# neggles/neurosis

Hardware: AMD Instinct MI355X
Metric: train images/sec (node) SDXL 1024^2 (higher is better)
Workload: dtype bf16

## Files before the change

### include/neurosis_hip.h

```cpp
#ifndef NEUROSIS_HIP_H
#define NEUROSIS_HIP_H

#ifdef __cplusplus
extern "C" {
#endif

const char* nk_last_error(void);
int nk_abi_version(void);

int nk_linear_fwd(const void* x, const void* w, const float* bias, const void* residual, void* y,
                  int M, int N, int K, long ldx, long ldw, long ldr, long ldy, float alpha, void* stream);
int nk_linear_dgrad(const void* dy, const void* w, const void* dx_add, void* dx, int M, int N, int K,
                    long lddy, long ldw, long ldadd, long lddx, void* stream);
long nk_linear_fwd_geglu_ok(int M, int I, int K);
int nk_linear_fwd_geglu(const void* x, const void* w, const float* bias, void* u, void* h, int M, int I, int K, long ldx, long ldw, long ldu,
                        long ldh, void* stream);
int nk_linear_dgrad_geglu(const void* dy, const void* w, const void* u, void* du, int M, int N, int I, long lddy, long ldw, long ldu,
                          long lddu, void* stream);
int nk_linear_fwd_geglu_s(const void* x, const void* w, const float* bias, void* s, void* h, int M, int I, int K, long ldx, long ldw, long lds,
                          long ldh, void* stream);
int nk_linear_dgrad_geglu_s(const void* dy, const void* w, const void* s, void* du, int M, int N, int I, long lddy, long ldw, long lds,
                            long lddu, void* stream);
int nk_linear_wgrad(const void* dy, const void* x, float* dw, int M, int N, int K, long lddy, long ldx,
                    long lddw, int accumulate, void* stream);
int nk_linear_wgrad_bias(const void* dy, const void* x, float* dw, float* dbias, int M, int N, int K, long lddy, long ldx, long lddw,
                         int accumulate, void* stream);

int nk_gemm_sk_status(void);

int nk_health_status(void);
int nk_health_clear(void);
int nk_health_export(int* dst, void* stream);
int nk_health_import(const int* src, void* stream);
int nk_debug_raise_health(void* stream);
int nk_debug_stamp(unsigned long long* dst, void* stream);
int nk_debug_launch_log(int mode);
long nk_debug_launch_names(char* buf, long cap);

int nk_colsum_batched(const void* dy, float* out, float* ws, long M, int N, long ld, int nbatch, int accumulate, void* stream);

int nk_linear_fwd_batched(const void* const* x, const void* const* w, void* const* y, int count, int M, int N, int K,
                          long ldx, long ldw, long ldy, void* stream);

int nk_linear_wgrad_batched(const void* const* dy, const void* const* x, float* const* dw, float* const* dbias, int count, int M, int N,
                            int K, long lddy, long ldx, long lddw, int accumulate, void* stream);

typedef struct NkConvDesc {
  int N, H, W, Cin;
  int Cout, KH, KW;
  int stride;
  int pad_t, pad_l;
  int Ho, Wo;
  int upsample;
} NkConvDesc;
int nk_conv2d_fwd(const NkConvDesc* d, const void* x, const void* w, const float* bias, const void* rowvec,
                  const void* residual, void* y, void* stream);
long nk_conv2d_stats_tiles(const NkConvDesc* d, int stats_groups);
int nk_conv2d_fwd_stats(const NkConvDesc* d, const void* x, const void* w, const float* bias, const void* rowvec, const void* residual,
                        void* y, float* stats_part, int stats_groups, void* stream);
int nk_conv3x3_few_channels_fwd(const void* x, const void* w, const float* bias, void* y, int N, int H, int W, int Cout, int cin_real,
                                void* stream);
int nk_conv_weight_flip(const void* w, void* wt, int Cout, int Cin, int taps, void* stream);
long nk_conv2d_dgrad_flipped_ok(const NkConvDesc* d);
int nk_conv2d_dgrad_flipped(const NkConvDesc* d, const void* dy, const void* wt, void* dx, void* stream);
int nk_conv2d_dgrad(const NkConvDesc* d, const void* dy, const void* w, void* dx, void* stream);
int nk_conv2d_wgrad(const NkConvDesc* d, const void* dy, const void* x, float* dw, int accumulate, void* stream);
int nk_conv2d_wgrad_bias(const NkConvDesc* d, const void* dy, const void* x, float* dw, float* dbias, int accumulate, void* stream);

typedef struct NkAttnDesc {
  int B, H, Lq, Lk, D;
  long sq, sk, sv, so;
  long bq, bk, bv, bo;
  long sdq, sdk, sdv, sdo;
  long bdq, bdk, bdv, bdo;
  float scale;
  int causal;
} NkAttnDesc;
int nk_attention_fwd(const NkAttnDesc* d, const void* q, const void* k, const void* v, void* o, float* lse,
                     void* stream);
long nk_attention_bwd_ws_floats(const NkAttnDesc* d);
int nk_attention_bwd(const NkAttnDesc* d, const void* q, const void* k, const void* v, const void* o,
                     const float* lse, const void* d_o, void* dq, void* dk, void* dv, float* delta_ws, void* stream);
int nk_attention_bwd_causal(const NkAttnDesc* d, const void* q, const void* k, const void* v, const void* o,
                            const float* lse, const void* d_o, void* dq, void* dk, void* dv, void* stream);
int nk_attention_relbias_fwd(const NkAttnDesc* d, const void* q, const void* k, const void* v, void* o, const float* rel, void* stream);
int nk_softmax_rows(void* s, long M, int L, void* stream);

long nk_groupnorm_ws_floats(int N, int HW, int C, int G);
int nk_groupnorm_fwd(const void* x, const float* gamma, const float* beta, void* y, float* mean, float* rstd,
                     float* ws, int N, int HW, int C, int G, float eps, int silu, void* stream);
int nk_groupnorm_sums(const void* x, float* sums, float* ws, int N, int HW, int C, int G, void* stream);
long nk_groupnorm_sums_ws_floats(int N, int nparts, int G);
int nk_groupnorm_sums_from_parts(const float* part, float* sums, float* ws, int N, int nparts, int G, void* stream);
int nk_groupnorm_apply(const void* x, const float* sums, const float* gamma, const float* beta, void* y, float* mean, float* rstd,
                       int N, int HW, int C, int G, float eps, int silu, void* stream);
int nk_groupnorm_bwd(const void* dy, const void* x, const float* gamma, const float* beta, const float* mean,
                     const float* rstd, const void* dx_add, void* dx, float* dgamma, float* dbeta, float* ws,
                     int N, int HW, int C, int G, int silu, int accumulate, void* stream);
int nk_groupnorm_mod_fwd(const void* x, const float* gamma, const float* beta, const void* mod, void* y, float* mean, float* rstd,
                         float* ws, int N, int HW, int C, int G, float eps, int silu, void* stream);
int nk_groupnorm_mod_apply(const void* x, const float* sums, const float* gamma, const float* beta, const void* mod, void* y, float* mean,
                           float* rstd, int N, int HW, int C, int G, float eps, int silu, void* stream);
int nk_groupnorm_mod_bwd(const void* dy, const void* x, const float* gamma, const float* beta, const void* mod, const float* mean,
                         const float* rstd, const void* dx_add, void* dx, float* dgamma, float* dbeta, void* dmod, float* ws,
                         int N, int HW, int C, int G, int silu, int accumulate, void* stream);

int nk_layernorm_fwd(const void* x, const float* gamma, const float* beta, void* y, float* mean, float* rstd,
                     int M, int C, float eps, void* stream);
long nk_layernorm_ws_floats(int M, int C);
int nk_rmsnorm_fwd(const void* x, const float* gamma, void* y, int M, int C, float eps, void* stream);
int nk_layernorm_bwd(const void* dy, const void* x, const float* gamma, const float* mean, const float* rstd,
                     const void* dx_add, void* dx, float* dgamma, float* dbeta, float* ws, int M, int C, int accumulate, void* stream);
#define NK_COLPART_MAX 32
typedef struct NkColpartBatch {
  const float* part[NK_COLPART_MAX];
  float* dgamma[NK_COLPART_MAX];
  float* dbeta[NK_COLPART_MAX];
  int nrows[NK_COLPART_MAX];
  int C[NK_COLPART_MAX];
  int accumulate[NK_COLPART_MAX];
  int n;
} NkColpartBatch;
long nk_layernorm_part_rows(int M);
int nk_layernorm_bwd_rows(const void* dy, const void* x, const float* gamma, const float* mean, const float* rstd,
                          const void* dx_add, void* dx, float* part, int M, int C, void* stream);
int nk_colpart_reduce_batch(const NkColpartBatch* b, void* stream);
int nk_layernorm_bwd_dx(const void* dy, const void* x, const float* gamma, const float* mean, const float* rstd,
                        const void* dx_add, void* dx, int M, int C, void* stream);
int nk_layernorm_bwd_params(const void* dy, const void* x, const float* mean, const float* rstd, float* dgamma,
                            float* dbeta, float* ws, int M, int C, int accumulate, void* stream);

int nk_geglu_fwd(const void* u, void* y, long M, int I, void* stream);
int nk_geglu_bwd(const void* dy, const void* u, void* du, long M, int I, void* stream);
int nk_geglu_fwd_s(const void* u, void* y, void* s, long M, int I, void* stream);
int nk_geglu_bwd_s(const void* dy, const void* s, void* du, long M, int I, void* stream);

int nk_silu_fwd(const void* x, void* y, long n, void* stream);
int nk_silu_bwd(const void* dy, const void* x, void* dx, long n, void* stream);

int nk_dropout(const void* x, const void* residual, void* y, long rows, int cols, long ld_x, long ld_res, long ld_y, const void* token,
               int site, int thr, float scale, void* stream);
int nk_dropout_draw(void* state, void* token, void* stream);

int nk_add(const void* a, const void* b, void* out, long n, void* stream);

int nk_cat_channels(const void* a, const void* b, void* out, long rows, int Ca, int Cb, void* stream);
int nk_split_channels(const void* src, void* a, void* b, long rows, int Ca, int Cb, void* stream);

int nk_upsample2x_bwd(const void* dup, void* dx, int N, int H, int W, int C, void* stream);
int nk_upsample2x_fwd(const void* x, void* up, int N, int H, int W, int C, void* stream);
int nk_avgpool2x_fwd(const void* x, void* y, int N, int H, int W, int C, void* stream);
int nk_avgpool2x_bwd(const void* dy, void* dx, int N, int H, int W, int C, void* stream);

int nk_nchw_to_nhwc(const void* src, int src_is_f32, void* dst, int N, int C, int HW, int Cpad, float scale,
                    void* stream);
int nk_nhwc_to_nchw(const void* src, void* dst, int dst_is_f32, int N, int C, int HW, int Cpad, void* stream);
int nk_cast_f32_to_bf16(const float* src, void* dst, long n, void* stream);
int nk_cast_bf16_to_f32(const void* src, float* dst, long n, void* stream);

long nk_colsum_ws_floats(long M, int N);
int nk_colsum(const void* dy, float* out, float* ws, long M, int N, long ld, int accumulate, void* stream);

int nk_softmax_rows_bwd(const void* p, void* dp, long M, int L, float scale, void* stream);

int nk_leaky_relu_fwd(const void* x, void* y, long n, float slope, void* stream);
int nk_leaky_relu_bwd(const void* dy, const void* y, void* dx, long n, float slope, void* stream);
long nk_batchnorm_ws_floats(long M, int C);
int nk_batchnorm_fwd(const void* x, const float* gamma, const float* beta, void* y, float* mean, float* rstd, float* running_mean,
                     float* running_var, float* ws, long M, int C, float eps, float momentum, float slope, void* stream);
int nk_batchnorm_bwd(const void* dy, const void* x, const void* y, const float* gamma, const float* mean, const float* rstd, void* dx,
                     float* dgamma, float* dbeta, float* ws, long M, int C, float slope, int accumulate, void* stream);
int nk_batchnorm_eval(const void* x, const float* gamma, const float* beta, const float* running_mean, const float* running_var, void* y,
                      float* ws, long M, int C, float eps, float slope, void* stream);

int nk_maxpool2x2_fwd(const void* x, void* y, int N, int H, int W, int C, void* stream);
int nk_maxpool2x2_bwd(const void* dy, const void* x, void* dx, int N, int H, int W, int C, void* stream);
int nk_maxpool_fwd(const void* x, void* y, int N, int H, int W, int C, int k, int s, void* stream);
int nk_maxpool_bwd(const void* dy, const void* x, void* dx, int N, int H, int W, int C, int k, int s, void* stream);
long nk_lpips_layer_ws_floats(int N, int HW);
int nk_lpips_layer_fwd(const void* f0, const void* f1, const float* w, float* out, float* ws, int N, int HW, int C, float eps,
                       int accumulate, void* stream);
int nk_lpips_layer_bwd(const void* f0, const void* f1, const float* w, const float* upstream, void* df1, int N, int HW, int C,
                       float eps, void* stream);

int nk_gelu_fwd(const void* x, void* y, long n, int mode, void* stream);
int nk_gated_gelu_tanh_fwd(const void* u, void* y, long M, int I, void* stream);
int nk_gelu_bwd(const void* dy, const void* x, void* dx, long n, int mode, void* stream);
#define NK_EMBEDDING_BWD_MAX_TOKENS 8192
int nk_embedding_bwd(const long long* ids, const void* dx, long ldx, float* dtable, float* dpos, int B, int L, int V, int P, int C,
                     int accumulate, void* stream);
int nk_gather_rows_bwd(const void* dsel, long ldsel, const long long* idx, void* dx, int B, int L, int C, void* stream);
int nk_wgrad_few_rows(const void* x, long ldx, const void* dy, long lddy, float* dw, long lddw, int M, int K, int N, int accumulate, void* stream);

#define NK_VQ_MAX_D 256
#define NK_VQ_MAX_CODES 65536
long nk_vq_search_ws_floats(long N, int n_e);
int nk_vq_search(const float* z, long ldz, const float* codebook, float* ws, long long* idx, long N, int D, int n_e, void* stream);
int nk_vq_code_stats(const long long* idx, const float* z, long ldz, long long* count, float* sum, long N, int D, int n_e, void* stream);
long nk_vq_quantize_ws_floats(long N);
int nk_vq_quantize(const long long* idx, const float* codebook, const float* z, long ldz, float* zq, float* sumsq, float* ws, long N, int D,
                   int n_e, int HW, void* stream);

int nk_timestep_embedding(const float* t, void* out, int B, int dim, float max_period, void* stream);

int nk_edm_prepare(const float* x, const float* eps, const float* sigma, const float* c_in, float* zt, void* net_in,
                   int B, int C, int HW, int Cpad, void* stream);
int nk_edm_prepare_cat(const float* x, const float* eps, const float* sigma, const float* c_in, const float* extra, float* zt,
                       void* net_in, int B, int C, int Ce, int HW, int Cpad, void* stream);
int nk_edm_loss(const void* net_out, const float* zt, const float* target, const float* c_out, const float* c_skip,
                const float* w, float* loss, void* dnet, int B, int C, int HW, int Cpad, float upstream, void* stream);

int nk_sample_prepare(const float* x, const float* c_in, void* net_in, int B, int C, int HW, int Cpad, int rep, void* stream);
int nk_sample_prepare_cat(const float* x, const float* c_in, const float* extra_u, const float* extra_c, void* net_in, int B, int C,
                          int Ce, int HW, int Cpad, int rep, void* stream);
int nk_sample_denoise(const void* net_out, const float* x, const float* c_skip, const float* c_out, float scale,
                      float* denoised, int B, int C, int HW, int Cpad, int rep, void* stream);
int nk_sample_euler_step(const void* net_out, const float* x, const float* c_skip, const float* c_out, const float* sigma_hat,
                         const float* sigma_next, float scale, float* x_next, float* denoised, int B, int C, int HW, int Cpad,
                         int rep, void* stream);

int nk_adamw_flat(float* p, const float* g, float* m, float* v, void* shadow, long n, float lr, float beta1,
                  float beta2, float eps, float weight_decay, int step, float grad_scale, void* stream);

typedef struct NkAdafactorArgs {
  float* master; const float* grad; void* shadow; float* state; float* ws;
  const void* tensors; const void* items;
  float* u2_part; float* p2_part; float* mean_row; float* scale; float* lr_t;
  int item_lo, item_hi, tensor_lo, tensor_hi;
  float beta2t, eps1, eps2, clip_threshold, rel_step, weight_decay, grad_scale;
  int scale_parameter;
  unsigned* counters;
  int has_matrix;
  int reserved;
} NkAdafactorArgs;
long nk_adafactor_tensor_bytes(void);
int nk_adafactor_init(const NkAdafactorArgs* args, void* stream);
int nk_adafactor_chunk(const NkAdafactorArgs* args, void* stream);

typedef struct NkCameArgs {
  float* master; const float* grad; void* shadow; float* state; float* ws;
  const void* tensors; const void* items;
  float* u2_part;
  float* mean_row;
  float* denom;
  unsigned* counters;
  int item_lo, item_hi, tensor_lo, tensor_hi;
  float beta1, beta2, beta3;
  float one_minus_beta1, one_minus_beta2, one_minus_beta3;
  float eps1, eps2, clip_threshold, lr, decay, grad_scale;
  int has_matrix;
} NkCameArgs;
long nk_came_tensor_bytes(void);
int nk_came_chunk(const NkCameArgs* args, void* stream);

typedef struct NkAdamW8bitArgs {
  float* master; const float* grad; void* shadow;
  unsigned char* code1; unsigned char* code2; float* absmax1; float* absmax2;
  float* m32; float* v32;
  const float* qmap1; const float* qmap2;
  const void* tensors; const int* blk_start;
  int ntensors, nblocks;
  float beta1, beta2, one_minus_beta1, one_minus_beta2, eps, lr, decay, bc1, bc2, grad_scale;
} NkAdamW8bitArgs;
long nk_adamw8bit_tensor_bytes(void);
int nk_adamw8bit_step(const NkAdamW8bitArgs* args, void* stream);

int nk_ema_flat(float* ema, const float* p, long n, float one_minus_decay, void* stream);

#ifdef __cplusplus
}
#endif
#endif
```

### neurosis_amd/csrc/norm.hip

```cpp
#include "../../include/neurosis_hip.h"
#include "nk_common.h"

#define GN_THREADS 256
#define GN_MAXC 4096

__global__ __launch_bounds__(GN_THREADS) void gn_stats_kernel(const bf16_t* __restrict__ x, float* __restrict__ stats,
                                                              int HW, int C, int G, int rows_per) {
  __shared__ float ps[GN_THREADS * 8], pss[GN_THREADS * 8];
  const int n = blockIdx.y;
  const int cpr = (C >> 3) / gridDim.z;
  const int ch0 = blockIdx.z * cpr;
  const int rows_par = GN_THREADS / cpr;
  const int tid = threadIdx.x;
  const int cpg = C / G;
  const int row_lo = blockIdx.x * rows_per;
  const int row_hi = min(HW, row_lo + rows_per);
  float s[8], ss[8];
#pragma unroll
  for (int e = 0; e < 8; ++e) { s[e] = 0.f; ss[e] = 0.f; }
  const int chunk = tid % cpr, rsub = tid / cpr;
  if (rsub < rows_par) {
    const bf16_t* base = x + ((long)n * HW) * C + (ch0 + chunk) * 8;
    int r = row_lo + rsub;
    for (; r + 3 * rows_par < row_hi; r += 4 * rows_par) {
      uint4_t v[4];
#pragma unroll
      for (int u = 0; u < 4; ++u) v[u] = *(const uint4_t*)(base + (long)(r + u * rows_par) * C);
#pragma unroll
      for (int u = 0; u < 4; ++u) {
        float f[8];
        unpack8(v[u], f);
#pragma unroll
        for (int e = 0; e < 8; ++e) { s[e] += f[e]; ss[e] += f[e] * f[e]; }
      }
    }
    for (; r < row_hi; r += rows_par) {
      float f[8];
      unpack8(*(const uint4_t*)(base + (long)r * C), f);
#pragma unroll
      for (int e = 0; e < 8; ++e) { s[e] += f[e]; ss[e] += f[e] * f[e]; }
    }
#pragma unroll
    for (int e = 0; e < 8; ++e) {
      ps[(rsub * cpr + chunk) * 8 + e] = s[e];
      pss[(rsub * cpr + chunk) * 8 + e] = ss[e];
    }
  }
  __syncthreads();
  float* part = stats + (((long)n * gridDim.x + blockIdx.x) * gridDim.z + blockIdx.z) * 2 * G;
  for (int i = tid; i < 2 * G; i += GN_THREADS) {
    const int g = i >> 1;
    const float* src = (i & 1) ? pss : ps;
    const int c_lo = max(g * cpg, ch0 * 8), c_hi = min((g + 1) * cpg, (ch0 + cpr) * 8);
    float a = 0.f;
    for (int c = c_lo; c < c_hi; ++c)
      for (int r = 0; r < rows_par; ++r) a += src[r * cpr * 8 + (c - ch0 * 8)];
    part[i] = a;
  }
}

__global__ __launch_bounds__(1024) void gn_reduce_partials_kernel(const float* __restrict__ part, float* __restrict__ out,
                                                                 int nparts, int G2) {
  __shared__ float sm[8][128];
  const int n = blockIdx.x;
  const int tx = threadIdx.x & 127, ty = threadIdx.x >> 7;
  float a = 0.f;
  if (tx < G2)
    for (int p = ty; p < nparts; p += 8) a += part[((long)n * nparts + p) * G2 + tx];
  sm[ty][tx] = a;
  __syncthreads();
  if (ty == 0 && tx < G2) {
#pragma unroll
    for (int j = 1; j < 8; ++j) a += sm[j][tx];
    out[(long)n * G2 + tx] = a;
  }
}

__device__ __forceinline__ void gn_modulate(const bf16_t* __restrict__ mod, int n, int c, int C, float& ga, float& be) {
  const float s1 = 1.0f + bf2f(mod[(long)n * 2 * C + c]);
  const float t = bf2f(mod[(long)n * 2 * C + C + c]);
  ga = ga * s1;
  be = be * s1 + t;
}

template <bool MOD>
__global__ __launch_bounds__(GN_THREADS) void gn_apply_kernel(const bf16_t* __restrict__ x, const float* __restrict__ stats,
                                                              const float* __restrict__ gamma, const float* __restrict__ beta,
                                                              const bf16_t* __restrict__ mod,
                                                              bf16_t* __restrict__ y, float* __restrict__ mean_out,
                                                              float* __restrict__ rstd_out, int HW, int C, int G,
                                                              float eps, int silu, int rows_per) {
  extern __shared__ __attribute__((aligned(16))) char smem_raw[];
  float* sc = (float*)smem_raw;
  float* sh = sc + C;
  const int n = blockIdx.y;
  const int tid = threadIdx.x;
  const int cpg = C / G;
  const float inv_cnt = 1.0f / ((float)HW * (float)cpg);
  for (int c = tid; c < C; c += GN_THREADS) {
    int g = c / cpg;
    float m = stats[(long)n * 2 * G + 2 * g] * inv_cnt;
    float var = fmaxf(stats[(long)n * 2 * G + 2 * g + 1] * inv_cnt - m * m, 0.f);
    float rs = rsqrtf(var + eps);
    float ga = gamma[c], be = beta[c];
    if constexpr (MOD) gn_modulate(mod, n, c, C, ga, be);
    float a = rs * ga;
    sc[c] = a;
    sh[c] = be - m * a;
    if (blockIdx.x == 0 && (c % cpg) == 0) { mean_out[n * G + g] = m; rstd_out[n * G + g] = rs; }
  }
  __syncthreads();
  const int cpr = C >> 3;
  const int row_lo = blockIdx.x * rows_per;
  const int row_hi = min(HW, row_lo + rows_per);
  const unsigned total = (unsigned)(row_hi - row_lo) * (unsigned)cpr;
  const bf16_t* xb = x + ((long)n * HW + row_lo) * C;
  bf16_t* yb = y + ((long)n * HW + row_lo) * C;
  auto one = [&](unsigned i, const uint4_t& raw) {
    const unsigned chunk = i % (unsigned)cpr;
    float f[8];
    unpack8(raw, f);
    const float4_t a0 = *(const float4_t*)(sc + chunk * 8), a1 = *(const float4_t*)(sc + chunk * 8 + 4);
    const float4_t b0 = *(const float4_t*)(sh + chunk * 8), b1 = *(const float4_t*)(sh + chunk * 8 + 4);
    f[0] = f[0] * a0[0] + b0[0]; f[1] = f[1] * a0[1] + b0[1]; f[2] = f[2] * a0[2] + b0[2]; f[3] = f[3] * a0[3] + b0[3];
    f[4] = f[4] * a1[0] + b1[0]; f[5] = f[5] * a1[1] + b1[1]; f[6] = f[6] * a1[2] + b1[2]; f[7] = f[7] * a1[3] + b1[3];
    if (silu) {
#pragma unroll
      for (int e = 0; e < 8; ++e) f[e] = silu_f(f[e]);
    }
    *(uint4_t*)(yb + (size_t)i * 8) = pack8(f);
  };
  unsigned i = tid;
  for (; i + 3 * GN_THREADS < total; i += 4 * GN_THREADS) {
    uint4_t v[4];
#pragma unroll
    for (int u = 0; u < 4; ++u) v[u] = *(const uint4_t*)(xb + (size_t)(i + u * GN_THREADS) * 8);
#pragma unroll
    for (int u = 0; u < 4; ++u) one(i + u * GN_THREADS, v[u]);
  }
  for (; i < total; i += GN_THREADS) one(i, *(const uint4_t*)(xb + (size_t)i * 8));
}

template <bool MOD>
__global__ __launch_bounds__(GN_THREADS, 4) void gn_bwd_stats_kernel(const bf16_t* __restrict__ dy, const bf16_t* __restrict__ x,
                                                                  const float* __restrict__ gamma, const float* __restrict__ beta,
                                                                  const bf16_t* __restrict__ mod,
                                                                  const float* __restrict__ mean, const float* __restrict__ rstd,
                                                                  float* __restrict__ gsum, float* __restrict__ chan_part,
                                                                  int HW, int C, int G, int silu, int rows_per) {
  __shared__ float pa[GN_THREADS * 8], pb[GN_THREADS * 8];
  extern __shared__ __attribute__((aligned(16))) char smem_raw[];
  float* ca = (float*)smem_raw;
  float* cb = ca + C;
  const int n = blockIdx.y;
  const int tid = threadIdx.x;
  const int cpg = C / G;
  const int cpr = (C >> 3) / gridDim.z;
  const int ch0 = blockIdx.z * cpr;
  const int rows_par = GN_THREADS / cpr;
  const int row_lo = blockIdx.x * rows_per;
  const int row_hi = min(HW, row_lo + rows_per);
  const int chunk = tid % cpr, rsub = tid / cpr;
  if (rsub < rows_par) {
    float a[8], b[8], mu[8], rs[8], ga[8], be[8];
#pragma unroll
    for (int e = 0; e < 8; ++e) {
      int c = (ch0 + chunk) * 8 + e;
      int g = c / cpg;
      a[e] = 0.f; b[e] = 0.f;
      mu[e] = mean[n * G + g]; rs[e] = rstd[n * G + g];
      ga[e] = gamma[c]; be[e] = beta[c];
      if constexpr (MOD) gn_modulate(mod, n, c, C, ga[e], be[e]);
    }
    const long base = ((long)n * HW) * C + (ch0 + chunk) * 8;
    auto one = [&](const uint4_t& rx, const uint4_t& rd) {
      float fx[8], fd[8];
      unpack8(rx, fx);
      unpack8(rd, fd);
#pragma unroll
      for (int e = 0; e < 8; ++e) {
        float xh = (fx[e] - mu[e]) * rs[e];
        float dz = fd[e];
        if (silu) dz *= dsilu_f(xh * ga[e] + be[e]);
        a[e] += dz;
        b[e] += dz * xh;
      }
    };
    int r = row_lo + rsub;
    for (; r + 3 * rows_par < row_hi; r += 4 * rows_par) {
      uint4_t vx[4], vd[4];
#pragma unroll
      for (int u = 0; u < 4; ++u) {
        vx[u] = *(const uint4_t*)(x + base + (long)(r + u * rows_par) * C);
        vd[u] = *(const uint4_t*)(dy + base + (long)(r + u * rows_par) * C);
      }
#pragma unroll
      for (int u = 0; u < 4; ++u) one(vx[u], vd[u]);
    }
    for (; r < row_hi; r += rows_par) one(*(const uint4_t*)(x + base + (long)r * C), *(const uint4_t*)(dy + base + (long)r * C));
#pragma unroll
    for (int e = 0; e < 8; ++e) {
      pa[(rsub * cpr + chunk) * 8 + e] = a[e];
      pb[(rsub * cpr + chunk) * 8 + e] = b[e];
    }
  }
  __syncthreads();
  float* cp = chan_part + ((long)n * gridDim.x + blockIdx.x) * 2 * C;
  for (int cl = tid; cl < cpr * 8; cl += GN_THREADS) {
    float av = 0.f, bv = 0.f;
    for (int r = 0; r < rows_par; ++r) { av += pa[r * cpr * 8 + cl]; bv += pb[r * cpr * 8 + cl]; }
    const int c = ch0 * 8 + cl;
    ca[cl] = av;
    cb[cl] = bv;
    cp[c] = bv;
    cp[C + c] = av;
  }
  __syncthreads();
  float* part = gsum + (((long)n * gridDim.x + blockIdx.x) * gridDim.z + blockIdx.z) * 2 * G;
  for (int i = tid; i < 2 * G; i += GN_THREADS) {
    const int g = i >> 1;
    const float* src = (i & 1) ? cb : ca;
    const int c_lo = max(g * cpg, ch0 * 8), c_hi = min((g + 1) * cpg, (ch0 + cpr) * 8);
    float acc = 0.f;
    for (int c = c_lo; c < c_hi; ++c) {
      float gc = gamma[c];
      if constexpr (MOD) { float bc = 0.f; gn_modulate(mod, n, c, C, gc, bc); }
      acc += gc * src[c - ch0 * 8];
    }
    part[i] = acc;
  }
}

__global__ __launch_bounds__(1024) void colpart_reduce_kernel(const float* __restrict__ part, float* __restrict__ dgamma,
                                                              float* __restrict__ dbeta, int nrows, int C, int accumulate) {
  __shared__ float sa[16][64], sb[16][64];
  const int tx = threadIdx.x & 63, ty = threadIdx.x >> 6;
  const int c = blockIdx.x * 64 + tx;
  float a = 0.f, b = 0.f;
  if (c < C) {
#pragma unroll 4
    for (int r = ty; r < nrows; r += 16) {
      a += part[(long)r * 2 * C + c];
      b += part[(long)r * 2 * C + C + c];
    }
  }
  sa[ty][tx] = a;
  sb[ty][tx] = b;
  __syncthreads();
  if (ty == 0 && c < C) {
#pragma unroll
    for (int j = 1; j < 16; ++j) { a += sa[j][tx]; b += sb[j][tx]; }
    dgamma[c] = accumulate ? dgamma[c] + a : a;
    dbeta[c] = accumulate ? dbeta[c] + b : b;
  }
}

__global__ __launch_bounds__(1024) void colpart_reduce_mod_kernel(const float* __restrict__ part, const bf16_t* __restrict__ mod,
                                                                  float* __restrict__ dgamma, float* __restrict__ dbeta, int nrows, int nsplit,
                                                                  int C, int accumulate) {
  __shared__ float sa[16][64], sb[16][64];
  const int tx = threadIdx.x & 63, ty = threadIdx.x >> 6;
  const int c = blockIdx.x * 64 + tx;
  float a = 0.f, b = 0.f;
  if (c < C) {
#pragma unroll 4
    for (int r = ty; r < nrows; r += 16) {
      const float s1 = 1.0f + bf2f(mod[(long)(r / nsplit) * 2 * C + c]);
      a += s1 * part[(long)r * 2 * C + c];
      b += s1 * part[(long)r * 2 * C + C + c];
    }
  }
  sa[ty][tx] = a;
  sb[ty][tx] = b;
  __syncthreads();
  if (ty == 0 && c < C) {
#pragma unroll
    for (int j = 1; j < 16; ++j) { a += sa[j][tx]; b += sb[j][tx]; }
    dgamma[c] = accumulate ? dgamma[c] + a : a;
    dbeta[c] = accumulate ? dbeta[c] + b : b;
  }
}

__global__ __launch_bounds__(1024) void gn_dmod_kernel(const float* __restrict__ part, const float* __restrict__ gamma,
                                                       const float* __restrict__ beta, bf16_t* __restrict__ dmod, int nsplit, int C) {
  __shared__ float sa[16][64], sb[16][64];
  const int tx = threadIdx.x & 63, ty = threadIdx.x >> 6;
  const int c = blockIdx.x * 64 + tx, n = blockIdx.y;
  float a = 0.f, b = 0.f;
  if (c < C) {
    for (int r = ty; r < nsplit; r += 16) {
      b += part[((long)n * nsplit + r) * 2 * C + c];
      a += part[((long)n * nsplit + r) * 2 * C + C + c];
    }
  }
  sa[ty][tx] = a;
  sb[ty][tx] = b;
  __syncthreads();
  if (ty == 0 && c < C) {
#pragma unroll
    for (int j = 1; j < 16; ++j) { a += sa[j][tx]; b += sb[j][tx]; }
    dmod[(long)n * 2 * C + c] = f2bf(gamma[c] * b + beta[c] * a);
    dmod[(long)n * 2 * C + C + c] = f2bf(a);
  }
}

template <bool MOD>
__global__ __launch_bounds__(GN_THREADS) void gn_bwd_apply_kernel(const bf16_t* __restrict__ dy, const bf16_t* __restrict__ x,
                                                                  const float* __restrict__ gamma, const float* __restrict__ beta,
                                                                  const bf16_t* __restrict__ mod,
                                                                  const float* __restrict__ mean, const float* __restrict__ rstd,
                                                                  const float* __restrict__ gsum, const bf16_t* __restrict__ dx_add,
                                                                  bf16_t* __restrict__ dx, int HW, int C, int G, int silu,
                                                                  int rows_per) {
  extern __shared__ __attribute__((aligned(16))) char smem_raw[];
  float* p_a = (float*)smem_raw;
  float* p_b = p_a + C;
  float* p_c = p_b + C;
  float* p_d = p_c + C;
  const int n = blockIdx.y;
  const int tid = threadIdx.x;
  const int cpg = C / G;
  const float inv_cnt = 1.0f / ((float)HW * (float)cpg);
  for (int c = tid; c < C; c += GN_THREADS) {
    const int g = c / cpg;
    const float mu = mean[n * G + g], rs = rstd[n * G + g];
    const float s1 = gsum[(long)n * 2 * G + 2 * g] * inv_cnt, s2 = gsum[(long)n * 2 * G + 2 * g + 1] * inv_cnt;
    float ga = gamma[c], be = beta[c];
    if constexpr (MOD) gn_modulate(mod, n, c, C, ga, be);
    const float a = rs * ga;
    p_a[c] = a;
    p_b[c] = be - mu * a;
    p_c[c] = -rs * rs * s2;
    p_d[c] = -rs * s1 + mu * rs * rs * s2;
  }
  __syncthreads();
  const int cpr = C >> 3;
  const int row_lo = blockIdx.x * rows_per;
  const int row_hi = min(HW, row_lo + rows_per);
  const unsigned total = (unsigned)(row_hi - row_lo) * (unsigned)cpr;
  const long off0 = ((long)n * HW + row_lo) * C;
  auto one = [&](unsigned i, const uint4_t& rx, const uint4_t& rd, const uint4_t& ra) {
    const int c0 = (int)(i % (unsigned)cpr) * 8;
    float fx[8], fd[8], fa[8], ca[8], cb[8], cc[8], cd[8];
    unpack8(rx, fx);
    unpack8(rd, fd);
    unpack8(ra, fa);
    *(float4_t*)ca = *(const float4_t*)(p_a + c0); *(float4_t*)(ca + 4) = *(const float4_t*)(p_a + c0 + 4);
    *(float4_t*)cc = *(const float4_t*)(p_c + c0); *(float4_t*)(cc + 4) = *(const float4_t*)(p_c + c0 + 4);
    *(float4_t*)cd = *(const float4_t*)(p_d + c0); *(float4_t*)(cd + 4) = *(const float4_t*)(p_d + c0 + 4);
    if (silu) {
      *(float4_t*)cb = *(const float4_t*)(p_b + c0); *(float4_t*)(cb + 4) = *(const float4_t*)(p_b + c0 + 4);
#pragma unroll
      for (int e = 0; e < 8; ++e) fd[e] *= dsilu_f(fx[e] * ca[e] + cb[e]);
    }
#pragma unroll
    for (int e = 0; e < 8; ++e) fx[e] = ca[e] * fd[e] + (fx[e] * cc[e] + cd[e]) + fa[e];
    *(uint4_t*)(dx + off0 + (size_t)i * 8) = pack8(fx);
  };
  const uint4_t zero4 = {0u, 0u, 0u, 0u};
  unsigned i = tid;
  for (; i + GN_THREADS < total; i += 2 * GN_THREADS) {
    uint4_t vx[2], vd[2], va[2];
#pragma unroll
    for (int u = 0; u < 2; ++u) {
      const size_t o = off0 + (size_t)(i + u * GN_THREADS) * 8;
      vx[u] = *(const uint4_t*)(x + o);
      vd[u] = *(const uint4_t*)(dy + o);
      va[u] = dx_add ? *(const uint4_t*)(dx_add + o) : zero4;
    }
#pragma unroll
    for (int u = 0; u < 2; ++u) one(i + u * GN_THREADS, vx[u], vd[u], va[u]);
  }
  for (; i < total; i += GN_THREADS) {
    const size_t o = off0 + (size_t)i * 8;
    one(i, *(const uint4_t*)(x + o), *(const uint4_t*)(dy + o), dx_add ? *(const uint4_t*)(dx_add + o) : zero4);
  }
}

static int gn_nz(int C) {
  int cpr = C >> 3, nz = (cpr + GN_THREADS - 1) / GN_THREADS;
  while (cpr % nz) ++nz;
  return nz;
}

static int gn_rows_per(int N, int HW, int* nsplit) {
  int want = (1024 + N - 1) / N;
  int rows_per = (HW + want - 1) / want;
  if (rows_per < 32) rows_per = 32;
  *nsplit = (HW + rows_per - 1) / rows_per;
  return rows_per;
}

extern "C" long nk_groupnorm_ws_floats(int N, int HW, int C, int G) {
  int nsplit;
  gn_rows_per(N, HW, &nsplit);
  long parts = (long)N * nsplit * gn_nz(C) * 2 * G;
  long chan = (long)N * nsplit * 2 * C;
  return parts + chan + (long)N * 2 * G + 64;
}

extern "C" int nk_groupnorm_fwd(const void* x, const float* gamma, const float* beta, void* y, float* mean,
                                float* rstd, float* ws, int N, int HW, int C, int G, float eps, int silu,
                                void* stream_) {
  hipStream_t stream = (hipStream_t)stream_;
  NK_CHECK_ARG(N > 0 && HW > 0 && C > 0 && G > 0 && G <= 64);
  NK_CHECK_ARG((C & 7) == 0 && C % G == 0 && C <= GN_MAXC);
  NK_CHECK_ARG(x && gamma && beta && y && mean && rstd && ws);
  int nsplit;
  int rows_per = gn_rows_per(N, HW, &nsplit);
  const int nz = gn_nz(C);
  float* part = ws;
  float* stats = ws + (long)N * nsplit * nz * 2 * G;
  hipLaunchKernelGGL(gn_stats_kernel, dim3(nsplit, N, nz), dim3(GN_THREADS), 0, stream, (const bf16_t*)x, part, HW, C,
                     G, rows_per);
  if (int e = nk_check_launch("gn_stats_kernel")) return e;
  hipLaunchKernelGGL(gn_reduce_partials_kernel, dim3(N), dim3(1024), 0, stream, part, stats, nsplit * nz, 2 * G);
  if (int e = nk_check_launch("gn_reduce_partials_kernel")) return e;
  hipLaunchKernelGGL(gn_apply_kernel<false>, dim3(nsplit, N), dim3(GN_THREADS), 2 * C * sizeof(float), stream,
                     (const bf16_t*)x, stats, gamma, beta, (const bf16_t*)nullptr, (bf16_t*)y, mean, rstd, HW, C, G, eps, silu, rows_per);
  return nk_check_launch("gn_apply_kernel");
}

__global__ __launch_bounds__(256) void gn_reduce_partials_l1_kernel(const float* __restrict__ part, float* __restrict__ out, int nparts, int G2, int nchunks) {
  __shared__ float sm[4][64];
  const int n = blockIdx.y, chunk = blockIdx.x;
  const int tx = threadIdx.x & 63, ty = threadIdx.x >> 6;
  float a = 0.f;
  if (tx < G2)
    for (int p = chunk + ty * nchunks; p < nparts; p += 4 * nchunks) a += part[((long)n * nparts + p) * G2 + tx];
  sm[ty][tx] = a;
  __syncthreads();
  if (ty == 0 && tx < G2) out[((long)n * nchunks + chunk) * G2 + tx] = (a + sm[1][tx]) + (sm[2][tx] + sm[3][tx]);
}

extern "C" long nk_groupnorm_sums_ws_floats(int N, int nparts, int G) {
  (void)nparts;
  return (long)N * 64 * 2 * G + 64;
}
extern "C" int nk_groupnorm_sums_from_parts(const float* part, float* sums, float* ws, int N, int nparts, int G, void* stream_) {
  hipStream_t stream = (hipStream_t)stream_;
  NK_CHECK_ARG(part && sums && N > 0 && nparts > 0 && G > 0 && G <= 32);
  if (nparts > 128) {
    NK_CHECK_ARG(ws != nullptr);
    const int nchunks = 64;
    hipLaunchKernelGGL(gn_reduce_partials_l1_kernel, dim3(nchunks, N), dim3(256), 0, stream, part, ws, nparts, 2 * G, nchunks);
    if (int e = nk_check_launch("gn_reduce_partials_l1_kernel")) return e;
    part = ws;
    nparts = nchunks;
  }
  hipLaunchKernelGGL(gn_reduce_partials_kernel, dim3(N), dim3(1024), 0, stream, part, sums, nparts, 2 * G);
  return nk_check_launch("gn_reduce_partials_kernel");
}

extern "C" int nk_groupnorm_sums(const void* x, float* sums, float* ws, int N, int HW, int C, int G, void* stream_) {
  hipStream_t stream = (hipStream_t)stream_;
  NK_CHECK_ARG(N > 0 && HW > 0 && C > 0 && G > 0 && G <= 64);
  NK_CHECK_ARG((C & 7) == 0 && C % G == 0 && C <= GN_MAXC);
  NK_CHECK_ARG(x && sums && ws);
  int nsplit;
  int rows_per = gn_rows_per(N, HW, &nsplit);
  const int nz = gn_nz(C);
  hipLaunchKernelGGL(gn_stats_kernel, dim3(nsplit, N, nz), dim3(GN_THREADS), 0, stream, (const bf16_t*)x, ws, HW, C, G, rows_per);
  if (int e = nk_check_launch("gn_stats_kernel")) return e;
  hipLaunchKernelGGL(gn_reduce_partials_kernel, dim3(N), dim3(1024), 0, stream, ws, sums, nsplit * nz, 2 * G);
  return nk_check_launch("gn_reduce_partials_kernel");
}

extern "C" int nk_groupnorm_apply(const void* x, const float* sums, const float* gamma, const float* beta, void* y, float* mean,
                                  float* rstd, int N, int HW, int C, int G, float eps, int silu, void* stream_) {
  hipStream_t stream = (hipStream_t)stream_;
  NK_CHECK_ARG(N > 0 && HW > 0 && C > 0 && G > 0 && G <= 64);
  NK_CHECK_ARG((C & 7) == 0 && C % G == 0 && C <= GN_MAXC);
  NK_CHECK_ARG(x && sums && gamma && beta && y && mean && rstd);
  int nsplit;
  int rows_per = gn_rows_per(N, HW, &nsplit);
  hipLaunchKernelGGL(gn_apply_kernel<false>, dim3(nsplit, N), dim3(GN_THREADS), 2 * C * sizeof(float), stream, (const bf16_t*)x, sums, gamma, beta,
                     (const bf16_t*)nullptr, (bf16_t*)y, mean, rstd, HW, C, G, eps, silu, rows_per);
  return nk_check_launch("gn_apply_kernel");
}

extern "C" int nk_groupnorm_bwd(const void* dy, const void* x, const float* gamma, const float* beta,
                                const float* mean, const float* rstd, const void* dx_add, void* dx, float* dgamma,
                                float* dbeta, float* ws, int N, int HW, int C, int G, int silu, int accumulate, void* stream_) {
  hipStream_t stream = (hipStream_t)stream_;
  NK_CHECK_ARG(N > 0 && HW > 0 && C > 0 && G > 0 && G <= 64);
  NK_CHECK_ARG((C & 7) == 0 && C % G == 0 && C <= GN_MAXC);
  NK_CHECK_ARG(dy && x && gamma && beta && mean && rstd && dx && dgamma && dbeta && ws);
  int nsplit;
  int rows_per = gn_rows_per(N, HW, &nsplit);
  const int nz = gn_nz(C);
  float* part = ws;
  float* gsum = part + (long)N * nsplit * nz * 2 * G;
  float* chan = gsum + (long)N * 2 * G;
  hipLaunchKernelGGL(gn_bwd_stats_kernel<false>, dim3(nsplit, N, nz), dim3(GN_THREADS), 2 * C * sizeof(float), stream,
                     (const bf16_t*)dy, (const bf16_t*)x, gamma, beta, (const bf16_t*)nullptr, mean, rstd, part, chan, HW, C, G, silu, rows_per);
  if (int e = nk_check_launch("gn_bwd_stats_kernel")) return e;
  hipLaunchKernelGGL(gn_reduce_partials_kernel, dim3(N), dim3(1024), 0, stream, part, gsum, nsplit * nz, 2 * G);
  if (int e = nk_check_launch("gn_reduce_partials_kernel")) return e;
  hipLaunchKernelGGL(colpart_reduce_kernel, dim3((C + 63) / 64), dim3(1024), 0, stream, chan, dgamma, dbeta, N * nsplit, C, accumulate);
  if (int e = nk_check_launch("colpart_reduce_kernel")) return e;
  hipLaunchKernelGGL(gn_bwd_apply_kernel<false>, dim3(nsplit, N), dim3(GN_THREADS), 4 * C * sizeof(float), stream,
                     (const bf16_t*)dy, (const bf16_t*)x, gamma, beta, (const bf16_t*)nullptr, mean, rstd, gsum, (const bf16_t*)dx_add,
                     (bf16_t*)dx, HW, C, G, silu, rows_per);
  return nk_check_launch("gn_bwd_apply_kernel");
}

static int gn_mod_apply_launch(const void* x, const float* sums, const float* gamma, const float* beta, const void* mod, void* y, float* mean,
                               float* rstd, int N, int HW, int C, int G, float eps, int silu, hipStream_t stream) {
  int nsplit;
  int rows_per = gn_rows_per(N, HW, &nsplit);
  hipLaunchKernelGGL(gn_apply_kernel<true>, dim3(nsplit, N), dim3(GN_THREADS), 2 * C * sizeof(float), stream, (const bf16_t*)x, sums, gamma, beta,
                     (const bf16_t*)mod, (bf16_t*)y, mean, rstd, HW, C, G, eps, silu, rows_per);
  return nk_check_launch("gn_apply_kernel<mod>");
}

extern "C" int nk_groupnorm_mod_fwd(const void* x, const float* gamma, const float* beta, const void* mod, void* y, float* mean, float* rstd,
                                    float* ws, int N, int HW, int C, int G, float eps, int silu, void* stream_) {
  hipStream_t stream = (hipStream_t)stream_;
  NK_CHECK_ARG(N > 0 && HW > 0 && C > 0 && G > 0 && G <= 64);
  NK_CHECK_ARG((C & 7) == 0 && C % G == 0 && C <= GN_MAXC);
  NK_CHECK_ARG(x && gamma && beta && mod && y && mean && rstd && ws);
  int nsplit;
  gn_rows_per(N, HW, &nsplit);
  float* stats = ws + (long)N * nsplit * gn_nz(C) * 2 * G;
  if (int e = nk_groupnorm_sums(x, stats, ws, N, HW, C, G, stream_)) return e;
  return gn_mod_apply_launch(x, stats, gamma, beta, mod, y, mean, rstd, N, HW, C, G, eps, silu, stream);
}

extern "C" int nk_groupnorm_mod_apply(const void* x, const float* sums, const float* gamma, const float* beta, const void* mod, void* y,
                                      float* mean, float* rstd, int N, int HW, int C, int G, float eps, int silu, void* stream_) {
  NK_CHECK_ARG(N > 0 && HW > 0 && C > 0 && G > 0 && G <= 64);
  NK_CHECK_ARG((C & 7) == 0 && C % G == 0 && C <= GN_MAXC);
  NK_CHECK_ARG(x && sums && gamma && beta && mod && y && mean && rstd);
  return gn_mod_apply_launch(x, sums, gamma, beta, mod, y, mean, rstd, N, HW, C, G, eps, silu, (hipStream_t)stream_);
}

extern "C" int nk_groupnorm_mod_bwd(const void* dy, const void* x, const float* gamma, const float* beta, const void* mod, const float* mean,
                                    const float* rstd, const void* dx_add, void* dx, float* dgamma, float* dbeta, void* dmod, float* ws,
                                    int N, int HW, int C, int G, int silu, int accumulate, void* stream_) {
  hipStream_t stream = (hipStream_t)stream_;
  NK_CHECK_ARG(N > 0 && HW > 0 && C > 0 && G > 0 && G <= 64);
  NK_CHECK_ARG((C & 7) == 0 && C % G == 0 && C <= GN_MAXC);
  NK_CHECK_ARG(dy && x && gamma && beta && mod && mean && rstd && dx && dgamma && dbeta && dmod && ws);
  int nsplit;
  int rows_per = gn_rows_per(N, HW, &nsplit);
  const int nz = gn_nz(C);
  float* part = ws;
  float* gsum = part + (long)N * nsplit * nz * 2 * G;
  float* chan = gsum + (long)N * 2 * G;
  hipLaunchKernelGGL(gn_bwd_stats_kernel<true>, dim3(nsplit, N, nz), dim3(GN_THREADS), 2 * C * sizeof(float), stream,
                     (const bf16_t*)dy, (const bf16_t*)x, gamma, beta, (const bf16_t*)mod, mean, rstd, part, chan, HW, C, G, silu, rows_per);
  if (int e = nk_check_launch("gn_bwd_stats_kernel<mod>")) return e;
  hipLaunchKernelGGL(gn_reduce_partials_kernel, dim3(N), dim3(1024), 0, stream, part, gsum, nsplit * nz, 2 * G);
  if (int e = nk_check_launch("gn_reduce_partials_kernel")) return e;
  hipLaunchKernelGGL(colpart_reduce_mod_kernel, dim3((C + 63) / 64), dim3(1024), 0, stream, chan, (const bf16_t*)mod, dgamma, dbeta, N * nsplit,
                     nsplit, C, accumulate);
  if (int e = nk_check_launch("colpart_reduce_mod_kernel")) return e;
  hipLaunchKernelGGL(gn_dmod_kernel, dim3((C + 63) / 64, N), dim3(1024), 0, stream, chan, gamma, beta, (bf16_t*)dmod, nsplit, C);
  if (int e = nk_check_launch("gn_dmod_kernel")) return e;
  hipLaunchKernelGGL(gn_bwd_apply_kernel<true>, dim3(nsplit, N), dim3(GN_THREADS), 4 * C * sizeof(float), stream,
                     (const bf16_t*)dy, (const bf16_t*)x, gamma, beta, (const bf16_t*)mod, mean, rstd, gsum, (const bf16_t*)dx_add,
                     (bf16_t*)dx, HW, C, G, silu, rows_per);
  return nk_check_launch("gn_bwd_apply_kernel<mod>");
}

#define LN_MAXCH 4

template <int NCH>
__global__ __launch_bounds__(256) void ln_fwd_kernel(const bf16_t* __restrict__ x, const float* __restrict__ gamma,
                                                     const float* __restrict__ beta, bf16_t* __restrict__ y,
                                                     float* __restrict__ mean, float* __restrict__ rstd, int M, int C,
                                                     float eps) {
  const int lane = threadIdx.x & 63;
  const int wave = (blockIdx.x * blockDim.x + threadIdx.x) >> 6;
  const int nwaves = (gridDim.x * blockDim.x) >> 6;
  const int cpr = C >> 3;
  const float invC = 1.0f / (float)C;
  for (int row = wave; row < M; row += nwaves) {
    float f[NCH][8];
    float s = 0.f;
#pragma unroll
    for (int j = 0; j < NCH; ++j) {
      int ch = lane + 64 * j;
      if (ch < cpr) {
        unpack8(*(const uint4_t*)(x + (long)row * C + ch * 8), f[j]);
#pragma unroll
        for (int e = 0; e < 8; ++e) s += f[j][e];
      }
    }
    const float mu = wave_sum(s) * invC;
    float v = 0.f;
#pragma unroll
    for (int j = 0; j < NCH; ++j) {
      int ch = lane + 64 * j;
      if (ch < cpr) {
#pragma unroll
        for (int e = 0; e < 8; ++e) { float d = f[j][e] - mu; v += d * d; }
      }
    }
    const float rs = rsqrtf(wave_sum(v) * invC + eps);
    if (lane == 0) { mean[row] = mu; rstd[row] = rs; }
#pragma unroll
    for (int j = 0; j < NCH; ++j) {
      int ch = lane + 64 * j;
      if (ch < cpr) {
        const float4_t g0 = *(const float4_t*)(gamma + ch * 8), g1 = *(const float4_t*)(gamma + ch * 8 + 4);
        const float4_t b0 = *(const float4_t*)(beta + ch * 8), b1 = *(const float4_t*)(beta + ch * 8 + 4);
        float o[8];
#pragma unroll
        for (int e = 0; e < 4; ++e) {
          o[e] = (f[j][e] - mu) * rs * g0[e] + b0[e];
          o[4 + e] = (f[j][4 + e] - mu) * rs * g1[e] + b1[e];
        }
        *(uint4_t*)(y + (long)row * C + ch * 8) = pack8(o);
      }
    }
  }
}

template <int NCH>
__global__ __launch_bounds__(256, 4) void ln_bwd_dx_kernel(const bf16_t* __restrict__ dy, const bf16_t* __restrict__ x,
                                                        const float* __restrict__ gamma, const float* __restrict__ mean,
                                                        const float* __restrict__ rstd, const bf16_t* __restrict__ dx_add,
                                                        bf16_t* __restrict__ dx, int M, int C) {
  const int lane = threadIdx.x & 63;
  const int wave = (blockIdx.x * blockDim.x + threadIdx.x) >> 6;
  const int nwaves = (gridDim.x * blockDim.x) >> 6;
  const int cpr = C >> 3;
  const float invC = 1.0f / (float)C;
  float gm[NCH][8];
#pragma unroll
  for (int j = 0; j < NCH; ++j) {
    int ch = lane + 64 * j;
#pragma unroll
    for (int e = 0; e < 8; ++e) gm[j][e] = 0.f;
    if (ch < cpr) {
      const float4_t g0 = *(const float4_t*)(gamma + ch * 8), g1 = *(const float4_t*)(gamma + ch * 8 + 4);
#pragma unroll
      for (int e = 0; e < 4; ++e) { gm[j][e] = g0[e]; gm[j][4 + e] = g1[e]; }
    }
  }
  for (int row = wave; row < M; row += nwaves) {
    const float mu = mean[row], rs = rstd[row];
    uint4_t rx[NCH], rd[NCH], ra[NCH];
#pragma unroll
    for (int j = 0; j < NCH; ++j) {
      int ch = lane + 64 * j;
      rx[j] = rd[j] = ra[j] = (uint4_t){0u, 0u, 0u, 0u};
      if (ch < cpr) {
        rx[j] = *(const uint4_t*)(x + (long)row * C + ch * 8);
        rd[j] = *(const uint4_t*)(dy + (long)row * C + ch * 8);
        if (dx_add) ra[j] = *(const uint4_t*)(dx_add + (long)row * C + ch * 8);
      }
    }
    float s1 = 0.f, s2 = 0.f;
#pragma unroll
    for (int j = 0; j < NCH; ++j) {
      float fx[8], fd[8];
      unpack8(rx[j], fx);
      unpack8(rd[j], fd);
#pragma unroll
      for (int e = 0; e < 8; ++e) {
        float d = fd[e] * gm[j][e];
        s1 += d;
        s2 += d * ((fx[e] - mu) * rs);
      }
    }
    s1 = wave_sum(s1) * invC;
    s2 = wave_sum(s2) * invC;
#pragma unroll
    for (int j = 0; j < NCH; ++j) {
      int ch = lane + 64 * j;
      if (ch < cpr) {
        float fx[8], fd[8], o[8];
        unpack8(rx[j], fx);
        unpack8(rd[j], fd);
        unpack8(ra[j], o);
#pragma unroll
        for (int e = 0; e < 8; ++e) o[e] += rs * (fd[e] * gm[j][e] - s1 - (fx[e] - mu) * rs * s2);
        *(uint4_t*)(dx + (long)row * C + ch * 8) = pack8(o);
      }
    }
  }
}

#define LNP_ROWS 64
__global__ __launch_bounds__(256) void ln_bwd_param_kernel(const bf16_t* __restrict__ dy, const bf16_t* __restrict__ x,
                                                           const float* __restrict__ mean, const float* __restrict__ rstd,
                                                           float* __restrict__ part, int M, int C) {
  __shared__ float pg[16][16 * 8 + 4], pb[16][16 * 8 + 4];
  const int tid = threadIdx.x;
  const int cx = tid & 15, ry = tid >> 4;
  const int chunk = blockIdx.y * 16 + cx;
  const bool cok = chunk < (C >> 3);
  const int row_lo = blockIdx.x * LNP_ROWS;
  float sg[8], sb[8];
#pragma unroll
  for (int e = 0; e < 8; ++e) { sg[e] = 0.f; sb[e] = 0.f; }
  if (cok) {
    uint4_t vx[4], vd[4];
    float mu[4], rs[4];
#pragma unroll
    for (int i = 0; i < 4; ++i) {
      const int r = row_lo + ry + 16 * i;
      const bool ok = r < M;
      vx[i] = ok ? *(const uint4_t*)(x + (long)r * C + chunk * 8) : (uint4_t){0u, 0u, 0u, 0u};
      vd[i] = ok ? *(const uint4_t*)(dy + (long)r * C + chunk * 8) : (uint4_t){0u, 0u, 0u, 0u};
      mu[i] = ok ? mean[r] : 0.f;
      rs[i] = ok ? rstd[r] : 0.f;
    }
#pragma unroll
    for (int i = 0; i < 4; ++i) {
      float fx[8], fd[8];
      unpack8(vx[i], fx);
      unpack8(vd[i], fd);
#pragma unroll
      for (int e = 0; e < 8; ++e) {
        sb[e] += fd[e];
        sg[e] += fd[e] * ((fx[e] - mu[i]) * rs[i]);
      }
    }
  }
#pragma unroll
  for (int e = 0; e < 8; ++e) { pg[ry][cx * 8 + e] = sg[e]; pb[ry][cx * 8 + e] = sb[e]; }
  __syncthreads();
  if (tid < 128) {
    const int c = blockIdx.y * 128 + tid;
    if (c < C) {
      float a = 0.f, b = 0.f;
#pragma unroll
      for (int r = 0; r < 16; ++r) { a += pg[r][tid]; b += pb[r][tid]; }
      float* out = part + (long)blockIdx.x * 2 * C;
      out[c] = a;
      out[C + c] = b;
    }
  }
}

static int ln_param_split(int M) { return (M + LNP_ROWS - 1) / LNP_ROWS; }

#define LNR_WAVES 4
#define LNR_MAX_BLOCKS 512
template <int NCH>
__global__ __launch_bounds__(LNR_WAVES * 64) void ln_bwd_rows_kernel(const bf16_t* __restrict__ dy, const bf16_t* __restrict__ x,
                                                                       const float* __restrict__ gamma, const float* __restrict__ mean,
                                                                       const float* __restrict__ rstd, const bf16_t* __restrict__ dx_add,
                                                                       bf16_t* __restrict__ dx, float* __restrict__ part, int M, int C) {
  extern __shared__ __attribute__((aligned(16))) char ln_smem[];
  float* red = (float*)ln_smem;
  const int lane = threadIdx.x & 63, wv = threadIdx.x >> 6;
  const int wave = blockIdx.x * LNR_WAVES + wv;
  const int nwaves = gridDim.x * LNR_WAVES;
  const int cpr = C >> 3;
  const float invC = 1.0f / (float)C;
  float gm[NCH][8], sg[NCH][8], sb[NCH][8];
#pragma unroll
  for (int j = 0; j < NCH; ++j) {
    int ch = lane + 64 * j;
#pragma unroll
    for (int e = 0; e < 8; ++e) { gm[j][e] = 0.f; sg[j][e] = 0.f; sb[j][e] = 0.f; }
    if (ch < cpr) {
      const float4_t g0 = *(const float4_t*)(gamma + ch * 8), g1 = *(const float4_t*)(gamma + ch * 8 + 4);
#pragma unroll
      for (int e = 0; e < 4; ++e) { gm[j][e] = g0[e]; gm[j][4 + e] = g1[e]; }
    }
  }
  uint4_t rx[NCH], rd[NCH], ra[NCH];
  float mu = 0.f, rs = 0.f;
  auto fetch = [&](int row, uint4_t (&fx)[NCH], uint4_t (&fd)[NCH], uint4_t (&fa)[NCH], float& fmu, float& frs) {
#pragma unroll
    for (int j = 0; j < NCH; ++j) {
      const int ch = lane + 64 * j;
      fx[j] = fd[j] = fa[j] = (uint4_t){0u, 0u, 0u, 0u};
      if (row < M && ch < cpr) {
        fx[j] = *(const uint4_t*)(x + (long)row * C + ch * 8);
        fd[j] = *(const uint4_t*)(dy + (long)row * C + ch * 8);
        if (dx_add) fa[j] = *(const uint4_t*)(dx_add + (long)row * C + ch * 8);
      }
    }
    fmu = row < M ? mean[row] : 0.f;
    frs = row < M ? rstd[row] : 0.f;
  };
  constexpr bool AHEAD = NCH < 4;
  if (AHEAD) fetch(wave, rx, rd, ra, mu, rs);
  for (int row = wave; row < M; row += nwaves) {
    uint4_t nx[NCH], nd[NCH], na[NCH];
    float nmu = 0.f, nrs = 0.f;
    if (AHEAD) fetch(row + nwaves, nx, nd, na, nmu, nrs);
    else fetch(row, rx, rd, ra, mu, rs);
    float s1 = 0.f, s2 = 0.f;
#pragma unroll
    for (int j = 0; j < NCH; ++j) {
      float fx[8], fd[8];
      unpack8(rx[j], fx);
      unpack8(rd[j], fd);
#pragma unroll
      for (int e = 0; e < 8; ++e) {
        const float xh = (fx[e] - mu) * rs;
        const float d = fd[e] * gm[j][e];
        s1 += d;
        s2 += d * xh;
        sb[j][e] += fd[e];
        sg[j][e] += fd[e] * xh;
      }
    }
    s1 = wave_sum(s1) * invC;
    s2 = wave_sum(s2) * invC;
#pragma unroll
    for (int j = 0; j < NCH; ++j) {
      int ch = lane + 64 * j;
      if (ch < cpr) {
        float fx[8], fd[8], o[8];
        unpack8(rx[j], fx);
        unpack8(rd[j], fd);
        unpack8(ra[j], o);
#pragma unroll
        for (int e = 0; e < 8; ++e) o[e] += rs * (fd[e] * gm[j][e] - s1 - (fx[e] - mu) * rs * s2);
        *(uint4_t*)(dx + (long)row * C + ch * 8) = pack8(o);
      }
    }
    if (AHEAD) {
#pragma unroll
      for (int j = 0; j < NCH; ++j) { rx[j] = nx[j]; rd[j] = nd[j]; ra[j] = na[j]; }
      mu = nmu;
      rs = nrs;
    }
  }
#pragma unroll
  for (int round = 0; round < LNR_WAVES / 2; ++round) {
    if ((wv >> 1) == round) {
      float* gbase = red + ((long)(wv & 1) * 2) * C;
#pragma unroll
      for (int j = 0; j < NCH; ++j) {
        int ch = lane + 64 * j;
        if (ch < cpr) {
          float* g = gbase + ch * 8;
          float4_t g0 = {sg[j][0], sg[j][1], sg[j][2], sg[j][3]}, g1 = {sg[j][4], sg[j][5], sg[j][6], sg[j][7]};
          float4_t b0 = {sb[j][0], sb[j][1], sb[j][2], sb[j][3]}, b1 = {sb[j][4], sb[j][5], sb[j][6], sb[j][7]};
          if (round) { g0 += *(const float4_t*)g; g1 += *(const float4_t*)(g + 4); b0 += *(const float4_t*)(g + C); b1 += *(const float4_t*)(g + C + 4); }
          *(float4_t*)g = g0;
          *(float4_t*)(g + 4) = g1;
          *(float4_t*)(g + C) = b0;
          *(float4_t*)(g + C + 4) = b1;
        }
      }
    }
    __syncthreads();
  }
  float* out = part + (long)blockIdx.x * 2 * C;
  for (int c = threadIdx.x; c < 2 * C; c += LNR_WAVES * 64) out[c] = red[c] + red[2 * C + c];
}
static int ln_rows_blocks(int M) {
  int b = (M + 4 * LNR_WAVES - 1) / (4 * LNR_WAVES);
  return b < 1 ? 1 : (b > LNR_MAX_BLOCKS ? LNR_MAX_BLOCKS : b);
}

__global__ __launch_bounds__(1024) void colpart_reduce_batch_kernel(const NkColpartBatch b) {
  __shared__ float sa[32][33], sb[32][33];
  const int z = blockIdx.y;
  const int C = b.C[z], nrows = b.nrows[z];
  if ((int)blockIdx.x * 32 >= C) return;
  const float* __restrict__ part = b.part[z];
  const int tx = threadIdx.x & 31, ty = threadIdx.x >> 5;
  const int c = blockIdx.x * 32 + tx;
  float a = 0.f, v = 0.f;
  if (c < C) {
#pragma unroll 8
    for (int r = ty; r < nrows; r += 32) {
      a += part[(long)r * 2 * C + c];
      v += part[(long)r * 2 * C + C + c];
    }
  }
  sa[ty][tx] = a;
  sb[ty][tx] = v;
  __syncthreads();
  if (ty == 0 && c < C) {
#pragma unroll
    for (int j = 1; j < 32; ++j) { a += sa[j][tx]; v += sb[j][tx]; }
    float* dgamma = b.dgamma[z];
    float* dbeta = b.dbeta[z];
    dgamma[c] = b.accumulate[z] ? dgamma[c] + a : a;
    dbeta[c] = b.accumulate[z] ? dbeta[c] + v : v;
  }
}

extern "C" int nk_colpart_reduce_batch(const NkColpartBatch* b, void* stream_) {
  NK_CHECK_ARG(b && b->n > 0 && b->n <= NK_COLPART_MAX);
  int maxC = 0;
  for (int z = 0; z < b->n; ++z) {
    NK_CHECK_ARG(b->part[z] && b->dgamma[z] && b->dbeta[z] && b->nrows[z] > 0 && b->C[z] > 0);
    maxC = b->C[z] > maxC ? b->C[z] : maxC;
  }
  hipLaunchKernelGGL(colpart_reduce_batch_kernel, dim3((maxC + 31) / 32, b->n), dim3(1024), 0, (hipStream_t)stream_, *b);
  return nk_check_launch("colpart_reduce_batch_kernel");
}

extern "C" int nk_layernorm_fwd(const void* x, const float* gamma, const float* beta, void* y, float* mean,
                                float* rstd, int M, int C, float eps, void* stream) {
  NK_CHECK_ARG(M > 0 && C > 0 && (C & 7) == 0 && (C >> 3) <= 64 * LN_MAXCH);
  NK_CHECK_ARG(x && gamma && beta && y && mean && rstd);
  int blocks = min((M + 3) / 4, 4096);
  const int nch = ((C >> 3) + 63) / 64;
#define NK_LN_FWD(NCH_) hipLaunchKernelGGL(ln_fwd_kernel<NCH_>, dim3(blocks), dim3(256), 0, (hipStream_t)stream, (const bf16_t*)x, gamma, beta, (bf16_t*)y, mean, rstd, M, C, eps)
  if (nch <= 2) NK_LN_FWD(2); else if (nch == 3) NK_LN_FWD(3); else NK_LN_FWD(4);
#undef NK_LN_FWD
  return nk_check_launch("ln_fwd_kernel");
}

#define RMS_MAXCH 8
template <int NCH>
__global__ __launch_bounds__(256) void rms_fwd_kernel(const bf16_t* __restrict__ x, const float* __restrict__ gamma, bf16_t* __restrict__ y, int M, int C,
                                                      float eps) {
  const int lane = threadIdx.x & 63;
  const int wave = (blockIdx.x * blockDim.x + threadIdx.x) >> 6;
  const int nwaves = (gridDim.x * blockDim.x) >> 6;
  const int cpr = C >> 3;
  const float invC = 1.0f / (float)C;
  for (int row = wave; row < M; row += nwaves) {
    uint4_t raw[NCH];
    float s = 0.f;
#pragma unroll
    for (int j = 0; j < NCH; ++j) {
      const int ch = lane + 64 * j;
      if (ch < cpr) {
        float f[8];
        raw[j] = *(const uint4_t*)(x + (long)row * C + ch * 8);
        unpack8(raw[j], f);
#pragma unroll
        for (int e = 0; e < 8; ++e) s = fmaf(f[e], f[e], s);
      }
    }
    const float rs = rsqrtf(wave_sum(s) * invC + eps);
#pragma unroll
    for (int j = 0; j < NCH; ++j) {
      const int ch = lane + 64 * j;
      if (ch < cpr) {
        const float4_t g0 = *(const float4_t*)(gamma + ch * 8), g1 = *(const float4_t*)(gamma + ch * 8 + 4);
        float f[8], o[8];
        unpack8(raw[j], f);
#pragma unroll
        for (int e = 0; e < 4; ++e) {
          o[e] = f[e] * rs * g0[e];
          o[4 + e] = f[4 + e] * rs * g1[e];
        }
        *(uint4_t*)(y + (long)row * C + ch * 8) = pack8(o);
      }
    }
  }
}

extern "C" int nk_rmsnorm_fwd(const void* x, const float* gamma, void* y, int M, int C, float eps, void* stream) {
  NK_CHECK_ARG(M > 0 && C > 0 && (C & 7) == 0 && (C >> 3) <= 64 * RMS_MAXCH);
  NK_CHECK_ARG(x && gamma && y);
  NK_CHECK_ARG(((uintptr_t)x & 15) == 0 && ((uintptr_t)y & 15) == 0 && ((uintptr_t)gamma & 15) == 0);
  int blocks = min((M + 3) / 4, 4096);
  const int nch = ((C >> 3) + 63) / 64;
#define NK_RMS_FWD(NCH_) hipLaunchKernelGGL(rms_fwd_kernel<NCH_>, dim3(blocks), dim3(256), 0, (hipStream_t)stream, (const bf16_t*)x, gamma, (bf16_t*)y, M, C, eps)
  if (nch <= 2) NK_RMS_FWD(2); else if (nch <= 4) NK_RMS_FWD(4); else NK_RMS_FWD(8);
#undef NK_RMS_FWD
  return nk_check_launch("rms_fwd_kernel");
}

extern "C" long nk_layernorm_ws_floats(int M, int C) {
  const long a = (long)ln_param_split(M), b = LNR_MAX_BLOCKS;
  return (a > b ? a : b) * 2 * C + 64;
}

extern "C" long nk_layernorm_part_rows(int M) { return ln_rows_blocks(M); }

extern "C" int nk_layernorm_bwd_dx(const void* dy, const void* x, const float* gamma, const float* mean, const float* rstd,
                                   const void* dx_add, void* dx, int M, int C, void* stream_) {
  hipStream_t stream = (hipStream_t)stream_;
  NK_CHECK_ARG(M > 0 && C > 0 && (C & 7) == 0 && (C >> 3) <= 64 * LN_MAXCH);
  NK_CHECK_ARG(dy && x && gamma && mean && rstd && dx);
  const int blocks = min((M + 3) / 4, 4096);
  const int nch = ((C >> 3) + 63) / 64;
#define NK_LN_DX(NCH_) hipLaunchKernelGGL(ln_bwd_dx_kernel<NCH_>, dim3(blocks), dim3(256), 0, stream, (const bf16_t*)dy, (const bf16_t*)x, gamma, mean, rstd, (const bf16_t*)dx_add, (bf16_t*)dx, M, C)
  if (nch <= 2) NK_LN_DX(2); else if (nch == 3) NK_LN_DX(3); else NK_LN_DX(4);
#undef NK_LN_DX
  return nk_check_launch("ln_bwd_dx_kernel");
}

extern "C" int nk_layernorm_bwd_params(const void* dy, const void* x, const float* mean, const float* rstd, float* dgamma,
                                       float* dbeta, float* ws, int M, int C, int accumulate, void* stream_) {
  hipStream_t stream = (hipStream_t)stream_;
  NK_CHECK_ARG(M > 0 && C > 0 && (C & 7) == 0);
  NK_CHECK_ARG(dy && x && mean && rstd && dgamma && dbeta && ws);
  const int nsplit = ln_param_split(M);
  hipLaunchKernelGGL(ln_bwd_param_kernel, dim3(nsplit, (C + 127) / 128), dim3(256), 0, stream, (const bf16_t*)dy, (const bf16_t*)x,
                     mean, rstd, ws, M, C);
  if (int e = nk_check_launch("ln_bwd_param_kernel")) return e;
  hipLaunchKernelGGL(colpart_reduce_kernel, dim3((C + 63) / 64), dim3(1024), 0, stream, ws, dgamma, dbeta, nsplit, C, accumulate);
  return nk_check_launch("colpart_reduce_kernel");
}

static int launch_ln_rows(const void* dy, const void* x, const float* gamma, const float* mean, const float* rstd, const void* dx_add,
                          void* dx, float* part, int M, int C, hipStream_t stream) {
  const int blocks = ln_rows_blocks(M);
  const int nch = ((C >> 3) + 63) / 64;
  const int smem = 2 * 2 * C * (int)sizeof(float);
#define NK_LN_ROWS(NCH_)                                                                                                       \
  do {                                                                                                                          \
    nk_optin_lds((const void*)ln_bwd_rows_kernel<NCH_>, 2 * 2 * 2048 * 4);                                                      \
    hipLaunchKernelGGL(ln_bwd_rows_kernel<NCH_>, dim3(blocks), dim3(LNR_WAVES * 64), smem, stream, (const bf16_t*)dy, (const bf16_t*)x, gamma, mean, rstd,   \
                       (const bf16_t*)dx_add, (bf16_t*)dx, part, M, C);                                                        \
  } while (0)
  if (nch <= 2) NK_LN_ROWS(2); else if (nch == 3) NK_LN_ROWS(3); else NK_LN_ROWS(4);
#undef NK_LN_ROWS
  return nk_check_launch("ln_bwd_rows_kernel");
}

extern "C" int nk_layernorm_bwd_rows(const void* dy, const void* x, const float* gamma, const float* mean, const float* rstd,
                                     const void* dx_add, void* dx, float* part, int M, int C, void* stream_) {
  NK_CHECK_ARG(M > 0 && C > 0 && (C & 7) == 0 && (C >> 3) <= 64 * LN_MAXCH);
  NK_CHECK_ARG(dy && x && gamma && mean && rstd && dx && part);
  return launch_ln_rows(dy, x, gamma, mean, rstd, dx_add, dx, part, M, C, (hipStream_t)stream_);
}

extern "C" int nk_layernorm_bwd(const void* dy, const void* x, const float* gamma, const float* mean,
                                const float* rstd, const void* dx_add, void* dx, float* dgamma, float* dbeta, float* ws,
                                int M, int C, int accumulate, void* stream_) {
  hipStream_t stream = (hipStream_t)stream_;
  NK_CHECK_ARG(M > 0 && C > 0 && (C & 7) == 0 && (C >> 3) <= 64 * LN_MAXCH);
  NK_CHECK_ARG(dy && x && gamma && mean && rstd && dx && dgamma && dbeta && ws);
  if (int e = launch_ln_rows(dy, x, gamma, mean, rstd, dx_add, dx, ws, M, C, stream)) return e;
  hipLaunchKernelGGL(colpart_reduce_kernel, dim3((C + 63) / 64), dim3(1024), 0, stream, ws, dgamma, dbeta, ln_rows_blocks(M), C, accumulate);
  return nk_check_launch("colpart_reduce_kernel");
}
```

### neurosis_amd/lib.py

```python
from __future__ import annotations

import ctypes as C
import os
from pathlib import Path

import torch

CSRC = Path(__file__).resolve().parent / "csrc"
LIB_PATH = CSRC / "libneurosis_hip.so"

vp, i32, i64, f32 = C.c_void_p, C.c_int, C.c_long, C.c_float


class NkConvDesc(C.Structure):
    _fields_ = [(n, i32) for n in ("N", "H", "W", "Cin", "Cout", "KH", "KW", "stride", "pad_t", "pad_l", "Ho", "Wo", "upsample")]


class NkAttnDesc(C.Structure):
    _fields_ = (
        [(n, i32) for n in ("B", "H", "Lq", "Lk", "D")]
        + [(n, i64) for n in ("sq", "sk", "sv", "so", "bq", "bk", "bv", "bo", "sdq", "sdk", "sdv", "sdo", "bdq", "bdk", "bdv", "bdo")]
        + [("scale", f32), ("causal", i32)]
    )


NK_COLPART_MAX = 32


class NkColpartBatch(C.Structure):
    _fields_ = [("part", vp * NK_COLPART_MAX), ("dgamma", vp * NK_COLPART_MAX), ("dbeta", vp * NK_COLPART_MAX), ("nrows", i32 * NK_COLPART_MAX),
                ("C", i32 * NK_COLPART_MAX), ("accumulate", i32 * NK_COLPART_MAX), ("n", i32)]


cdp, adp = C.POINTER(NkConvDesc), C.POINTER(NkAttnDesc)

SIGNATURES: dict[str, list] = {
    "nk_linear_fwd": [vp, vp, vp, vp, vp, i32, i32, i32, i64, i64, i64, i64, f32, vp],
    "nk_linear_dgrad": [vp, vp, vp, vp, i32, i32, i32, i64, i64, i64, i64, vp],
    "nk_linear_dgrad_geglu": [vp, vp, vp, vp, i32, i32, i32, i64, i64, i64, i64, vp],
    "nk_linear_fwd_geglu": [vp, vp, vp, vp, vp, i32, i32, i32, i64, i64, i64, i64, vp],
    "nk_linear_fwd_geglu_s": [vp, vp, vp, vp, vp, i32, i32, i32, i64, i64, i64, i64, vp],
    "nk_linear_dgrad_geglu_s": [vp, vp, vp, vp, i32, i32, i32, i64, i64, i64, i64, vp],
    "nk_linear_wgrad": [vp, vp, vp, i32, i32, i32, i64, i64, i64, i32, vp],
    "nk_linear_fwd_batched": [C.POINTER(vp), C.POINTER(vp), C.POINTER(vp), i32, i32, i32, i32, i64, i64, i64, vp],
    "nk_linear_wgrad_batched": [C.POINTER(vp), C.POINTER(vp), C.POINTER(vp), C.POINTER(vp), i32, i32, i32, i32, i64, i64, i64, i32, vp],
    "nk_linear_wgrad_bias": [vp, vp, vp, vp, i32, i32, i32, i64, i64, i64, i32, vp],
    "nk_conv2d_wgrad_bias": [cdp, vp, vp, vp, vp, i32, vp],
    "nk_conv2d_fwd": [cdp, vp, vp, vp, vp, vp, vp, vp],
    "nk_conv2d_fwd_stats": [cdp, vp, vp, vp, vp, vp, vp, vp, i32, vp],
    "nk_conv_weight_flip": [vp, vp, i32, i32, i32, vp],
    "nk_conv3x3_few_channels_fwd": [vp, vp, vp, vp, i32, i32, i32, i32, i32, vp],
    "nk_conv2d_dgrad": [cdp, vp, vp, vp, vp],
    "nk_conv2d_dgrad_flipped": [cdp, vp, vp, vp, vp],
    "nk_conv2d_wgrad": [cdp, vp, vp, vp, i32, vp],
    "nk_attention_fwd": [adp, vp, vp, vp, vp, vp, vp],
    "nk_attention_bwd": [adp, vp, vp, vp, vp, vp, vp, vp, vp, vp, vp, vp],
    "nk_attention_bwd_causal": [adp, vp, vp, vp, vp, vp, vp, vp, vp, vp, vp],
    "nk_attention_relbias_fwd": [adp, vp, vp, vp, vp, vp, vp],
    "nk_softmax_rows": [vp, i64, i32, vp],
    "nk_softmax_rows_bwd": [vp, vp, i64, i32, f32, vp],
    "nk_groupnorm_fwd": [vp, vp, vp, vp, vp, vp, vp, i32, i32, i32, i32, f32, i32, vp],
    "nk_groupnorm_sums": [vp, vp, vp, i32, i32, i32, i32, vp],
    "nk_groupnorm_sums_from_parts": [vp, vp, vp, i32, i32, i32, vp],
    "nk_groupnorm_apply": [vp, vp, vp, vp, vp, vp, vp, i32, i32, i32, i32, f32, i32, vp],
    "nk_groupnorm_bwd": [vp, vp, vp, vp, vp, vp, vp, vp, vp, vp, vp, i32, i32, i32, i32, i32, i32, vp],
    "nk_groupnorm_mod_fwd": [vp, vp, vp, vp, vp, vp, vp, vp, i32, i32, i32, i32, f32, i32, vp],
    "nk_groupnorm_mod_apply": [vp, vp, vp, vp, vp, vp, vp, vp, i32, i32, i32, i32, f32, i32, vp],
    "nk_groupnorm_mod_bwd": [vp, vp, vp, vp, vp, vp, vp, vp, vp, vp, vp, vp, vp, i32, i32, i32, i32, i32, i32, vp],
    "nk_layernorm_fwd": [vp, vp, vp, vp, vp, vp, i32, i32, f32, vp],
    "nk_rmsnorm_fwd": [vp, vp, vp, i32, i32, f32, vp],
    "nk_layernorm_bwd": [vp, vp, vp, vp, vp, vp, vp, vp, vp, vp, i32, i32, i32, vp],
    "nk_layernorm_bwd_dx": [vp, vp, vp, vp, vp, vp, vp, i32, i32, vp],
    "nk_layernorm_bwd_rows": [vp, vp, vp, vp, vp, vp, vp, vp, i32, i32, vp],
    "nk_colpart_reduce_batch": [C.POINTER(NkColpartBatch), vp],
    "nk_layernorm_bwd_params": [vp, vp, vp, vp, vp, vp, vp, i32, i32, i32, vp],
    "nk_geglu_fwd": [vp, vp, i64, i32, vp],
    "nk_geglu_bwd": [vp, vp, vp, i64, i32, vp],
    "nk_geglu_fwd_s": [vp, vp, vp, i64, i32, vp],
    "nk_geglu_bwd_s": [vp, vp, vp, i64, i32, vp],
    "nk_silu_fwd": [vp, vp, i64, vp],
    "nk_gelu_fwd": [vp, vp, i64, i32, vp],
    "nk_gated_gelu_tanh_fwd": [vp, vp, i64, i32, vp],
    "nk_gelu_bwd": [vp, vp, vp, i64, i32, vp],
    "nk_embedding_bwd": [vp, vp, i64, vp, vp, i32, i32, i32, i32, i32, i32, vp],
    "nk_gather_rows_bwd": [vp, i64, vp, vp, i32, i32, i32, vp],
    "nk_wgrad_few_rows": [vp, i64, vp, i64, vp, i64, i32, i32, i32, i32, vp],
    "nk_vq_search": [vp, i64, vp, vp, vp, i64, i32, i32, vp],
    "nk_vq_code_stats": [vp, vp, i64, vp, vp, i64, i32, i32, vp],
    "nk_vq_quantize": [vp, vp, vp, i64, vp, vp, vp, i64, i32, i32, i32, vp],
    "nk_leaky_relu_fwd": [vp, vp, i64, f32, vp],
    "nk_leaky_relu_bwd": [vp, vp, vp, i64, f32, vp],
    "nk_maxpool2x2_fwd": [vp, vp, i32, i32, i32, i32, vp],
    "nk_maxpool2x2_bwd": [vp, vp, vp, i32, i32, i32, i32, vp],
    "nk_maxpool_fwd": [vp, vp, i32, i32, i32, i32, i32, i32, vp],
    "nk_maxpool_bwd": [vp, vp, vp, i32, i32, i32, i32, i32, i32, vp],
    "nk_lpips_layer_fwd": [vp, vp, vp, vp, vp, i32, i32, i32, f32, i32, vp],
    "nk_lpips_layer_bwd": [vp, vp, vp, vp, vp, i32, i32, i32, f32, vp],
    "nk_batchnorm_fwd": [vp, vp, vp, vp, vp, vp, vp, vp, vp, i64, i32, f32, f32, f32, vp],
    "nk_batchnorm_bwd": [vp, vp, vp, vp, vp, vp, vp, vp, vp, vp, i64, i32, f32, i32, vp],
    "nk_batchnorm_eval": [vp, vp, vp, vp, vp, vp, vp, i64, i32, f32, f32, vp],
    "nk_silu_bwd": [vp, vp, vp, i64, vp],
    "nk_add": [vp, vp, vp, i64, vp],
    "nk_dropout": [vp, vp, vp, i64, i32, i64, i64, i64, vp, i32, i32, f32, vp],
    "nk_dropout_draw": [vp, vp, vp],
    "nk_cat_channels": [vp, vp, vp, i64, i32, i32, vp],
    "nk_split_channels": [vp, vp, vp, i64, i32, i32, vp],
    "nk_upsample2x_bwd": [vp, vp, i32, i32, i32, i32, vp],
    "nk_upsample2x_fwd": [vp, vp, i32, i32, i32, i32, vp],
    "nk_avgpool2x_fwd": [vp, vp, i32, i32, i32, i32, vp],
    "nk_avgpool2x_bwd": [vp, vp, i32, i32, i32, i32, vp],
    "nk_nchw_to_nhwc": [vp, i32, vp, i32, i32, i32, i32, f32, vp],
    "nk_nhwc_to_nchw": [vp, vp, i32, i32, i32, i32, i32, vp],
    "nk_cast_f32_to_bf16": [vp, vp, i64, vp],
    "nk_cast_bf16_to_f32": [vp, vp, i64, vp],
    "nk_colsum": [vp, vp, vp, i64, i32, i64, i32, vp],
    "nk_colsum_batched": [vp, vp, vp, i64, i32, i64, i32, i32, vp],
    "nk_timestep_embedding": [vp, vp, i32, i32, f32, vp],
    "nk_edm_prepare": [vp, vp, vp, vp, vp, vp, i32, i32, i32, i32, vp],
    "nk_edm_prepare_cat": [vp, vp, vp, vp, vp, vp, vp, i32, i32, i32, i32, i32, vp],
    "nk_edm_loss": [vp, vp, vp, vp, vp, vp, vp, vp, i32, i32, i32, i32, f32, vp],
    "nk_sample_prepare": [vp, vp, vp, i32, i32, i32, i32, i32, vp],
    "nk_sample_prepare_cat": [vp, vp, vp, vp, vp, i32, i32, i32, i32, i32, i32, vp],
    "nk_sample_denoise": [vp, vp, vp, vp, f32, vp, i32, i32, i32, i32, i32, vp],
    "nk_sample_euler_step": [vp, vp, vp, vp, vp, vp, f32, vp, vp, i32, i32, i32, i32, i32, vp],
    "nk_adamw_flat": [vp, vp, vp, vp, vp, i64, f32, f32, f32, f32, f32, i32, f32, vp],
    "nk_ema_flat": [vp, vp, i64, f32, vp],
    "nk_debug_raise_health": [vp],
    "nk_debug_stamp": [vp, vp],
    "nk_debug_launch_log": [i32],
    "nk_health_clear": [],
    "nk_health_export": [vp, vp],
    "nk_health_import": [vp, vp],
    "nk_adafactor_init": [vp, vp],
    "nk_adafactor_chunk": [vp, vp],
    "nk_came_chunk": [vp, vp],
    "nk_adamw8bit_step": [vp, vp],
}

SIZE_QUERIES: dict[str, list] = {
    "nk_groupnorm_ws_floats": [i32, i32, i32, i32],
    "nk_groupnorm_sums_ws_floats": [i32, i32, i32],
    "nk_conv2d_stats_tiles": [cdp, i32],
    "nk_conv2d_dgrad_flipped_ok": [cdp],
    "nk_linear_fwd_geglu_ok": [i32, i32, i32],
    "nk_layernorm_ws_floats": [i32, i32],
    "nk_layernorm_part_rows": [i32],
    "nk_colsum_ws_floats": [i64, i32],
    "nk_batchnorm_ws_floats": [i64, i32],
    "nk_lpips_layer_ws_floats": [i32, i32],
    "nk_attention_bwd_ws_floats": [adp],
    "nk_vq_search_ws_floats": [i64, i32],
    "nk_vq_quantize_ws_floats": [i64],
    "nk_adafactor_tensor_bytes": [],
    "nk_came_tensor_bytes": [],
    "nk_adamw8bit_tensor_bytes": [],
    "nk_gemm_sk_status": [],
    "nk_health_status": [],
    "nk_debug_launch_names": [C.c_char_p, i64],
}

_lib = None


class NkError(RuntimeError):
    pass


def load() -> C.CDLL:
    global _lib
    if _lib is not None:
        return _lib
    path = Path(os.environ.get("NEUROSIS_HIP_LIB", LIB_PATH))
    if not path.exists():
        raise NkError(
            f"{path} not found: the HIP extension is not built. Run `python -c 'import __graft_entry__ as g; g.build()'` "
            "(or `make -C neurosis_amd/csrc`). There is no CPU fallback for the product path."
        )
    lib = C.CDLL(str(path))
    lib.nk_last_error.restype = C.c_char_p
    lib.nk_last_error.argtypes = []
    lib.nk_abi_version.restype = i32
    lib.nk_abi_version.argtypes = []
    for name, argtypes in SIGNATURES.items():
        fn = getattr(lib, name)
        fn.argtypes = argtypes
        fn.restype = i32
    for name, argtypes in SIZE_QUERIES.items():
        fn = getattr(lib, name)
        fn.argtypes = argtypes
        fn.restype = i64
    _lib = lib
    return lib


def launch_log(mode: int) -> None:
    call("nk_debug_launch_log", int(mode))


def launched() -> list[str]:
    buf = C.create_string_buffer(8192)
    n = query("nk_debug_launch_names", buf, len(buf))
    if n < 0:
        raise NkError("nk_debug_launch_names failed")
    return buf.value.decode().split("\n")[:-1]


def query(name: str, *args) -> int:
    return int(getattr(load(), name)(*args))


def call(name: str, *args) -> None:
    lib = load()
    rc = getattr(lib, name)(*args)
    if rc != 0:
        raise NkError(f"{name} failed (rc={rc}): {lib.nk_last_error().decode()}")
```

### neurosis_amd/modules/diffusion/openaimodel.py

```python
from __future__ import annotations

import os

from typing import Callable, List, Optional, Union

import torch
from torch import Tensor, nn

from ... import ops
from ...nn import Conv2d, FlatParamStore, apply_module, as_tokens, linear_module_fwd
from ...ops import BF16, Img
from ..attention import SpatialTransformer, zero_module


def conv_nd(dims: int, *args, **kwargs) -> nn.Module:
    if dims != 2:
        raise ValueError(f"unsupported dimensions: {dims} (the MI355X path implements 2-D convolutions)")
    return Conv2d(*args, **kwargs)


class TimestepBlock(nn.Module):

    def forward(self, x: Tensor, emb: Tensor):
        raise NotImplementedError("TimestepBlock is an interface: subclasses implement forward(x, emb)")


class TimestepEmbedSequential(nn.Sequential, TimestepBlock):

    def fwd(self, x: Img, emb: Tensor, context: Optional[Tensor], dctx_sink: Optional[Callable[[Tensor], None]] = None):
        bwds = []
        first = True
        for layer in self:
            if isinstance(layer, TimestepBlock):
                x, b = layer.fwd(x, emb)
                bwds.append(("emb", b))
            elif isinstance(layer, SpatialTransformer):
                x, b = layer.fwd(x, context, need_dctx=dctx_sink is not None)
                bwds.append(("ctx", b))
            elif isinstance(layer, (Conv2d, Upsample, Downsample)):
                x, b = layer.fwd(x, need_dx=not (first and getattr(self, "_nk_input_block", False)))
                bwds.append(("plain", b))
            elif isinstance(layer, nn.Identity):
                continue
            else:
                raise NotImplementedError(f"TimestepEmbedSequential: unsupported layer {type(layer).__name__}")
            first = False

        def bwd(dy: Tensor):
            demb = None
            for kind, b in reversed(bwds):
                if dy is None:
                    break
                if kind == "emb":
                    dy, de = b(dy)
                    demb = de if demb is None else ops.add(demb, de)
                elif kind == "ctx":
                    dy, dc = b(dy)
                    if dctx_sink is not None and dc is not None:
                        dctx_sink(dc)
                else:
                    dyi, _ = b(dy)
                    dy = None if dyi is None else dyi.t
            bwds.clear()
            return dy, demb

        return x, bwd

    def forward(self, x: Tensor, emb: Tensor, context: Optional[Tensor] = None, image_only_indicator=None, time_context=None, num_video_frames=None):
        ins = [x, emb] if context is None else [x, emb, context]
        ops.dropout_open(self)

        def run(x, emb, context=None):
            img = Img.from_nchw(x)
            out, bwd = self.fwd(img, as_tokens(emb), None if context is None else as_tokens(context))

            def bwd2(g):
                dx, demb = bwd(Img.from_nchw(g).t)
                res = (Img(dx, img.N, img.H, img.W).to_nchw(), None if demb is None else demb.view(emb.shape))
                return res if context is None else (*res, None)

            return out.to_nchw(), bwd2

        return apply_module(run, ins, self)


class Upsample(nn.Module):

    def __init__(self, channels: int, use_conv: bool, dims: int = 2, out_channels: Optional[int] = None, padding: int = 1,
                 third_up: bool = False, kernel_size: int = 3, scale_factor: int = 2):
        super().__init__()
        self.channels = channels
        self.out_channels = out_channels or channels
        self.use_conv = use_conv
        self.dims = dims
        self.third_up = third_up
        self.scale_factor = scale_factor
        if dims != 2 or scale_factor != 2:
            raise NotImplementedError("Upsample: the MI355X path implements dims=2, scale_factor=2 (dims=3 / third_up are the video options)")
        if use_conv:
            self.conv = conv_nd(dims, self.channels, self.out_channels, kernel_size, padding=padding)

    def fwd(self, x: Img, need_dx: bool = True):
        assert x.C == self.channels
        if self.use_conv:
            return self.conv.fwd(x, upsample=True, need_dx=need_dx)
        y, b = ops.upsample2x_fwd(x)
        return y, (lambda dy: (Img(b(dy), x.N, x.H, x.W) if need_dx else None, None))

    def forward(self, x: Tensor) -> Tensor:
        return _plain_forward(self, x)


class Downsample(nn.Module):

    def __init__(self, channels: int, use_conv: bool, dims: int = 2, out_channels: Optional[int] = None, padding: int = 1, third_down: bool = False):
        super().__init__()
        self.channels = channels
        self.out_channels = out_channels or channels
        self.use_conv = use_conv
        self.dims = dims
        if dims != 2:
            raise NotImplementedError("Downsample: the MI355X path implements dims=2 (dims=3 / third_down are the video options)")
        if use_conv:
            self.op = conv_nd(dims, self.channels, self.out_channels, 3, stride=2, padding=padding)
        else:
            assert self.channels == self.out_channels, "Downsample(use_conv=False) cannot change the channel count"
            self.op = nn.AvgPool2d(kernel_size=2, stride=2)

    def fwd(self, x: Img, need_dx: bool = True):
        assert x.C == self.channels
        if self.use_conv:
            return self.op.fwd(x, need_dx=need_dx)
        y, b = ops.avgpool2x_fwd(x)
        return y, (lambda dy: (Img(b(dy), x.N, x.H, x.W) if need_dx else None, None))

    def forward(self, x: Tensor) -> Tensor:
        return _plain_forward(self, x)


def _plain_forward(mod: nn.Module, x: Tensor) -> Tensor:
    def run(x):
        img = Img.from_nchw(x)
        out, bwd = mod.fwd(img)
        return out.to_nchw(), lambda g: bwd(Img.from_nchw(g).t)[0].to_nchw()

    return apply_module(run, [x], mod)


class ResBlock(TimestepBlock):

    def __init__(self, channels: int, emb_channels: int, dropout: float, out_channels: Optional[int] = None, use_conv: bool = False,
                 use_scale_shift_norm: bool = False, dims: int = 2, use_checkpoint: bool = False, up: bool = False, down: bool = False,
                 kernel_size: int = 3, exchange_temb_dims: bool = False, skip_t_emb: bool = False):
        super().__init__()
        if exchange_temb_dims or skip_t_emb:
            raise NotImplementedError("ResBlock: exchange_temb_dims / skip_t_emb are options of the video UNet, which is not on the MI355X path")
        self.channels = channels
        self.emb_channels = emb_channels
        self.dropout = self.dropout_p = ops.check_dropout_rate(dropout, "ResBlock")
        self.out_channels = out_channels if out_channels is not None else channels
        self.use_conv = use_conv
        self.use_checkpoint = use_checkpoint
        self.use_scale_shift_norm = use_scale_shift_norm
        self.exchange_temb_dims = exchange_temb_dims
        padding = kernel_size // 2
        self.in_layers = nn.Sequential(nn.GroupNorm(32, channels), nn.SiLU(), conv_nd(dims, channels, self.out_channels, kernel_size, padding=padding))
        self.updown = up or down
        self._up, self._down = bool(up), bool(down) and not up
        if up:
            self.h_upd = Upsample(channels, False, dims)
            self.x_upd = Upsample(channels, False, dims)
        elif down:
            self.h_upd = Downsample(channels, False, dims)
            self.x_upd = Downsample(channels, False, dims)
        else:
            self.h_upd = self.x_upd = nn.Identity()
        self.skip_t_emb = skip_t_emb
        self.emb_out_channels = 2 * self.out_channels if use_scale_shift_norm else self.out_channels
        self.emb_layers = nn.Sequential(nn.SiLU(), nn.Linear(emb_channels, self.emb_out_channels))
        self.out_layers = nn.Sequential(
            nn.GroupNorm(32, self.out_channels), nn.SiLU(), nn.Dropout(p=dropout),
            zero_module(conv_nd(dims, self.out_channels, self.out_channels, kernel_size, padding=padding)),
        )
        if self.out_channels == channels:
            self.skip_connection = nn.Identity()
        elif use_conv:
            self.skip_connection = conv_nd(dims, channels, self.out_channels, kernel_size, padding=padding)
        else:
            self.skip_connection = conv_nd(dims, channels, self.out_channels, 1)

    def _skip_fwd(self, x: Img):
        skip = self.skip_connection
        b_res = None
        if self._down:
            x, b_res = ops.avgpool2x_fwd(x)
        if isinstance(skip, nn.Identity):
            s, b_skip = x.t, None
        elif skip.kernel_size == 1:
            s, b_skip = ops.linear_fwd(x.t, skip.weight, skip.bias)
        else:
            si, b_skip3 = skip.fwd(x, upsample=self._up)
            s, b_skip = si.t, (lambda g: b_skip3(g)[0].t)
        b_up = None
        if self._up and (b_skip is None or skip.kernel_size == 1):
            sup, b_up = ops.upsample2x_fwd(Img(s, x.N, x.H, x.W))
            s = sup.t
        if b_skip is None and b_res is None and b_up is None:
            return s, None

        def bwd(dy: Tensor) -> Tensor:
            if b_up is not None:
                dy = b_up(dy)
            if b_skip is not None:
                dy = b_skip(dy)
            return dy if b_res is None else b_res(dy)

        return s, bwd

    def _fwd(self, x: Img, emb: Tensor):
        gn1, gn2 = self.in_layers[0], self.out_layers[0]
        ssn = self.use_scale_shift_norm
        h1, b_gn1 = ops.groupnorm_fwd(x, gn1.weight, gn1.bias, 32, gn1.eps, silu=True)
        b_pool = None
        if self._down:
            h1, b_pool = ops.avgpool2x_fwd(h1)
        es, b_es = ops.silu_fwd(emb)
        eo, b_eo = linear_module_fwd(self.emb_layers[1], es)
        h2, b_c1 = self.in_layers[2].fwd(h1, rowvec=None if ssn else eo, upsample=self._up, stats_groups=32)
        if ssn:
            h3, b_gn2 = ops.groupnorm_mod_fwd(h2, gn2.weight, gn2.bias, eo, 32, gn2.eps, silu=True)
        else:
            h3, b_gn2 = ops.groupnorm_fwd(h2, gn2.weight, gn2.bias, 32, gn2.eps, silu=True)
        b_drop = None
        if self.training and self.dropout_p > 0.0:
            _, b_drop = ops.dropout_fwd(h3.t, self.dropout_p, ops.dropout_site(self), inplace=True)
        s, b_skip = self._skip_fwd(x)
        out, b_c2 = self.out_layers[3].fwd(h3, residual=s, stats_groups=32)

        def bwd(dy: Tensor):
            dh3, _ = b_c2(dy)
            dh2 = b_gn2(dh3.t if b_drop is None else b_drop(dh3.t, inplace=True))
            if ssn:
                dh2, deo = dh2
                dh1, _ = b_c1(dh2)
            else:
                dh1, deo = b_c1(dh2)
            dh1 = dh1.t if b_pool is None else b_pool(dh1.t)
            dxs = dy if b_skip is None else b_skip(dy)
            dx = b_gn1(dh1, dxs)
            demb = b_es(b_eo(deo))
            return dx, demb

        return out, bwd

    def fwd(self, x: Img, emb: Tensor):
        if not (self.use_checkpoint and ops.recording()):
            return self._fwd(x, emb)
        out, _ = self._fwd(x, emb)
        tok = ops.dropout_token(required=False)

        def bwd(dy: Tensor):
            with ops.dropout_token_scope(tok):
                _, b = self._fwd(x, emb)
            return b(dy)

        return out, bwd

    def forward(self, x: Tensor, emb: Tensor) -> Tensor:
        ops.dropout_open(self)

        def run(x, emb):
            img = Img.from_nchw(x)
            out, bwd = self.fwd(img, as_tokens(emb))

            def bwd2(g):
                dx, demb = bwd(Img.from_nchw(g).t)
                return Img(dx, img.N, img.H, img.W).to_nchw(), demb.view(emb.shape)

            return out.to_nchw(), bwd2

        return apply_module(run, [x, emb], self)


class Timestep(nn.Module):

    def __init__(self, dim: int):
        super().__init__()
        self.dim = dim

    def forward(self, t: Tensor) -> Tensor:
        return ops.timestep_embedding(t, self.dim)


class UNetModel(nn.Module):

    def __init__(
        self,
        in_channels: int,
        model_channels: int,
        out_channels: int,
        num_res_blocks: int,
        attention_resolutions,
        dropout: float = 0.0,
        channel_mult=(1, 2, 4, 8),
        conv_resample: bool = True,
        dims: int = 2,
        num_classes=None,
        use_checkpoint: bool = False,
        num_heads: int = -1,
        num_head_channels: int = -1,
        num_heads_upsample: int = -1,
        use_scale_shift_norm: bool = False,
        resblock_updown: bool = False,
        transformer_depth=1,
        context_dim: Optional[int] = None,
        disable_self_attentions: Optional[List[bool]] = None,
        num_attention_blocks: Optional[List[int]] = None,
        disable_middle_self_attn: bool = False,
        disable_middle_transformer: bool = False,
        use_linear_in_transformer: bool = False,
        spatial_transformer_attn_type: str = "softmax",
        adm_in_channels: Optional[int] = None,
    ):
        super().__init__()
        if num_heads_upsample == -1:
            num_heads_upsample = num_heads
        if num_heads == -1:
            assert num_head_channels != -1, "UNetModel: num_heads = -1 needs num_head_channels"
        if num_head_channels == -1:
            assert num_heads != -1, "UNetModel: num_head_channels = -1 needs num_heads"
        self.in_channels = in_channels
        self.model_channels = model_channels
        self.out_channels = out_channels
        if isinstance(transformer_depth, int):
            transformer_depth = len(channel_mult) * [transformer_depth]
        transformer_depth_middle = transformer_depth[-1]
        if isinstance(num_res_blocks, int):
            self.num_res_blocks = len(channel_mult) * [num_res_blocks]
        else:
            if len(num_res_blocks) != len(channel_mult):
                raise ValueError(f"UNetModel: num_res_blocks is an int or one entry per level ({len(channel_mult)}), got {num_res_blocks!r}")
            self.num_res_blocks = num_res_blocks
        if disable_self_attentions is not None and len(disable_self_attentions) != len(channel_mult):
            raise ValueError(f"UNetModel: disable_self_attentions needs one entry per level ({len(channel_mult)})")
        if num_attention_blocks is not None and len(num_attention_blocks) != len(self.num_res_blocks):
            raise ValueError("UNetModel: num_attention_blocks needs one entry per level, like num_res_blocks")

        self.attention_resolutions = attention_resolutions
        self.dropout = ops.check_dropout_rate(dropout, "UNetModel")
        self.channel_mult = channel_mult
        self.conv_resample = conv_resample
        self.num_classes = num_classes
        self.use_checkpoint = use_checkpoint
        self.num_heads = num_heads
        self.num_head_channels = num_head_channels
        self.num_heads_upsample = num_heads_upsample

        time_embed_dim = model_channels * 4
        self.time_embed = nn.Sequential(nn.Linear(model_channels, time_embed_dim), nn.SiLU(), nn.Linear(time_embed_dim, time_embed_dim))

        if self.num_classes is not None:
            if self.num_classes == "sequential":
                if adm_in_channels is None:
                    raise ValueError("UNetModel: num_classes='sequential' needs adm_in_channels (the width of the vector conditioning)")
                self.label_emb = nn.Sequential(nn.Sequential(nn.Linear(adm_in_channels, time_embed_dim), nn.SiLU(), nn.Linear(time_embed_dim, time_embed_dim)))
            else:
                raise NotImplementedError(f"num_classes={self.num_classes!r}: only 'sequential' (SDXL) and None (SD1.5) are on the path")

        def make_st(ch, level_depth, disabled_sa):
            if num_head_channels == -1:
                heads, dim_head = num_heads, ch // num_heads
            else:
                heads, dim_head = ch // num_head_channels, num_head_channels
            return SpatialTransformer(ch, heads, dim_head, depth=level_depth, dropout=dropout, context_dim=context_dim, disable_self_attn=disabled_sa,
                                      use_linear=use_linear_in_transformer, attn_type=spatial_transformer_attn_type, use_checkpoint=use_checkpoint)

        def res(cin, cout, **updown):
            return ResBlock(cin, time_embed_dim, dropout, out_channels=cout, dims=dims, use_checkpoint=use_checkpoint, use_scale_shift_norm=use_scale_shift_norm,
                            **updown)

        self.input_blocks = nn.ModuleList([TimestepEmbedSequential(conv_nd(dims, in_channels, model_channels, 3, padding=1))])
        input_block_chans = [model_channels]
        ch = model_channels
        ds = 1
        for level, mult in enumerate(channel_mult):
            for nr in range(self.num_res_blocks[level]):
                layers = [res(ch, mult * model_channels)]
                ch = mult * model_channels
                if ds in attention_resolutions:
                    disabled_sa = disable_self_attentions[level] if (context_dim is not None and disable_self_attentions is not None) else False
                    if num_attention_blocks is None or nr < num_attention_blocks[level]:
                        layers.append(make_st(ch, transformer_depth[level], disabled_sa))
                self.input_blocks.append(TimestepEmbedSequential(*layers))
                input_block_chans.append(ch)
            if level != len(channel_mult) - 1:
                out_ch = ch
                self.input_blocks.append(TimestepEmbedSequential(
                    res(ch, out_ch, down=True) if resblock_updown else Downsample(ch, conv_resample, dims=dims, out_channels=out_ch)))
                ch = out_ch
                input_block_chans.append(ch)
                ds *= 2

        self.middle_block = TimestepEmbedSequential(
            res(ch, ch),
            make_st(ch, transformer_depth_middle, disable_middle_self_attn) if not disable_middle_transformer else nn.Identity(),
            res(ch, ch),
        )

        self.output_blocks = nn.ModuleList([])
        for level, mult in list(enumerate(channel_mult))[::-1]:
            for i in range(self.num_res_blocks[level] + 1):
                ich = input_block_chans.pop()
                layers = [res(ch + ich, model_channels * mult)]
                ch = model_channels * mult
                if ds in attention_resolutions:
                    disabled_sa = disable_self_attentions[level] if disable_self_attentions is not None else False
                    if num_attention_blocks is None or i < num_attention_blocks[level]:
                        layers.append(make_st(ch, transformer_depth[level], disabled_sa))
                if level and i == self.num_res_blocks[level]:
                    out_ch = ch
                    layers.append(res(ch, out_ch, up=True) if resblock_updown else Upsample(ch, conv_resample, dims=dims, out_channels=out_ch))
                    ds //= 2
                self.output_blocks.append(TimestepEmbedSequential(*layers))

        self.out = nn.Sequential(nn.GroupNorm(32, ch), nn.SiLU(), zero_module(conv_nd(dims, model_channels, out_channels, 3, padding=1)))
        self.input_blocks[0]._nk_input_block = True
        self.grad_ready_hook: Optional[Callable[[nn.Module], None]] = None
        self._nk_graphs = None

    def _mlp_fwd(self, seq: nn.Sequential, x: Tensor, need_dx: bool):
        a, b0 = linear_module_fwd(seq[0], x, need_dx=need_dx)
        s, b1 = ops.silu_fwd(a)
        o, b2 = linear_module_fwd(seq[2], s)
        return o, (lambda g: b0(b1(b2(g))))

    def set_recompute(self, policy: Optional[str]) -> "UNetModel":
        from ..attention import BasicTransformerBlock

        if policy not in (None, "norms"):
            raise ValueError(f"recompute policy must be None or 'norms', got {policy!r}")
        for m in self.modules():
            if isinstance(m, BasicTransformerBlock):
                m.recompute = policy
        self._nk_graphs = None
        return self

    def _project_context(self, context: Tensor) -> None:
        from ..attention import BasicTransformerBlock
        from ...nn import adjacent

        if getattr(self, "_nk_cross", None) is None:
            self._nk_cross = [blk.attn2 for blk in self.modules() if isinstance(blk, BasicTransformerBlock)]
        groups = {}
        for att in self._nk_cross:
            wk, wv = att.to_k.weight, att.to_v.weight
            if wk.shape[1] != context.shape[1] or not adjacent(wk, wv):
                continue
            groups.setdefault((wk.shape[0], wk.shape[1]), []).append(att)
        for (inner, cdim), atts in groups.items():
            if len(atts) < 2:
                continue
            ws = [torch.as_strided(ops.shadow(a.to_k.weight), (2 * inner, cdim), (cdim, 1)) for a in atts]
            outs = ops.gemm_nt_batched([context] * len(atts), ws)
            for a, kv in zip(atts, outs):
                a._nk_kv = (kv, context)

    def fwd_graphed(self, x: Img, timesteps: Tensor, context: Optional[Tensor], y: Optional[Tensor], need_dctx: bool = False, need_dy: bool = False):
        from ...graphs import ChainGraphs, frozen_stamp, graphs_enabled

        if not x.t.is_cuda or not graphs_enabled():
            return self.fwd(x, timesteps, context, y, need_dctx, need_dy)
        if self._nk_graphs is None:
            self._nk_graphs = ChainGraphs(self.out[2].weight, hook=lambda: self.grad_ready_hook)
        N, H, W = x.N, x.H, x.W
        return self._nk_graphs.run(lambda t, ts, c, yy: self.fwd(Img(t, N, H, W), ts, c, yy, need_dctx, need_dy), [x.t, timesteps, context, y],
                                   extra_key=(N, H, W, frozen_stamp(self), self.training, need_dctx, need_dy))

    def fwd(self, x: Img, timesteps: Tensor, context: Optional[Tensor], y: Optional[Tensor], need_dctx: bool = False, need_dy: bool = False):
        hook_raw = self.grad_ready_hook
        need_dctx = bool(need_dctx) and context is not None
        need_dy = bool(need_dy) and y is not None and self.num_classes is not None
        if self.training and self.dropout > 0.0:
            ops.dropout_open(self)
        t_emb = ops.timestep_embedding(timesteps, self.model_channels)
        emb, b_time = self._mlp_fwd(self.time_embed, t_emb, need_dx=False)
        b_label = None
        if self.num_classes is not None:
            lab, b_label = self._mlp_fwd(self.label_emb[0], y, need_dx=need_dy)
            emb = ops.add(emb, lab)
        if context is not None:
            self._project_context(context)
        dctx = [None]

        def sink(dc: Tensor) -> None:
            dctx[0] = dc if dctx[0] is None else ops.add(dctx[0], dc)

        sink_ = sink if need_dctx else None
        hs: List[Img] = []
        tape = []
        h = x
        for module in self.input_blocks:
            h, b = module.fwd(h, emb, context, sink_)
            hs.append(h)
            tape.append((module, b))
        h, b_mid = self.middle_block.fwd(h, emb, context, sink_)
        out_tape = []
        for module in self.output_blocks:
            h, b_cat = ops.cat_fwd(h, hs.pop())
            h, b = module.fwd(h, emb, context, sink_)
            out_tape.append((module, b, b_cat))
        gn = self.out[0]
        hn, b_gn = ops.groupnorm_fwd(h, gn.weight, gn.bias, 32, gn.eps, silu=True)
        out, b_conv = self.out[2].fwd(hn)

        def bwd(dout: Tensor):
            est = ops.state_of(self.out[2].weight)
            if est.segment_hook is not None:
                hook = est.segment_hook
            elif hook_raw is not None:
                def hook(m):
                    hook_raw(m)
            else:
                hook = None
            dh, _ = b_conv(dout)
            dh = b_gn(dh.t)
            if hook:
                hook(self.out)
            demb = None

            def acc_emb(de):
                nonlocal demb
                if de is not None:
                    demb = de if demb is None else ops.add(demb, de)

            skips = []
            for module, b, b_cat in reversed(out_tape):
                dh, de = b(dh)
                acc_emb(de)
                dh, dskip = b_cat(dh)
                skips.append(dskip)
                if hook:
                    hook(module)
            out_tape.clear()
            dh, de = b_mid(dh)
            acc_emb(de)
            if hook:
                hook(self.middle_block)
            for module, b in reversed(tape):
                dh = ops.add(dh, skips.pop())
                dh, de = b(dh)
                acc_emb(de)
                if hook:
                    hook(module)
            tape.clear()
            dy = None
            if b_label is not None:
                dy = b_label(demb)
                if hook:
                    hook(self.label_emb)
            b_time(demb)
            if hook:
                hook(self.time_embed)
            ops.join_wgrad_stream(self.out[2].weight)
            if need_dctx or need_dy:
                return dh, dctx[0], dy
            return dh

        return out, bwd

    def forward(self, x: Tensor, timesteps: Optional[Tensor] = None, context: Optional[Tensor] = None, y: Optional[Tensor] = None, **kwargs) -> Tensor:
        if (y is not None) != (self.num_classes is not None):
            raise ValueError(f"UNetModel.forward: this network has no label embedding (num_classes=None) but was given y of shape {tuple(y.shape)}")
        if y is not None:
            assert y.shape[0] == x.shape[0]
        N, Cin, H, W = x.shape
        ins = [x, timesteps, context, y]

        def run(x, timesteps, context, y):
            cpad = (Cin + 7) // 8 * 8
            if cpad == Cin:
                img = Img.from_nchw(x)
            else:
                img = Img(ops.nchw_to_tokens(x, cpad), N, H, W)
            need_dctx = context is not None and context.requires_grad
            need_dy = y is not None and y.requires_grad
            out, bwd = self.fwd(img, timesteps, None if context is None else as_tokens(context), None if y is None else as_tokens(y), need_dctx, need_dy)
            o = ops.tokens_to_nchw(out.t, N, self.out_channels, out.H, out.W, dtype=x.dtype if x.dtype in (torch.float32, BF16) else torch.float32)

            def bwd2(g):
                gt = ops.nchw_to_tokens(g, out.C)
                res = bwd(gt)
                dx, dctx, dy = res if (need_dctx or need_dy) else (res, None, None)
                gx = None
                if dx is not None and x.requires_grad:
                    gx = ops.tokens_to_nchw(dx, N, Cin, H, W, dtype=x.dtype)
                return gx, None, None if dctx is None else dctx.view(context.shape), None if dy is None else dy.view(y.shape)

            return o, bwd2

        return apply_module(run, ins, self)
```

### neurosis_amd/ops.py

```python
from __future__ import annotations

import ctypes as C
import os
import threading
import weakref
from dataclasses import dataclass
from typing import Callable, Optional

import torch
from torch import Tensor

from . import lib
from .lib import NkAttnDesc, NkConvDesc, call, query

BF16 = torch.bfloat16


class EngineState:

    _live = weakref.WeakSet()

    def __init__(self, wgrad_stream=None):
        self.grad_accumulate = False
        self.assume_zeroed = False
        self.wgrad_stream = wgrad_stream
        self.batch_wgrads = os.environ.get("NK_BATCH_WGRADS", "1") != "0"
        self.norm_params_on_side_stream: Optional[bool] = None
        self.deferred: Optional[list] = None
        self.segment_hook: Optional[Callable] = None
        EngineState._live.add(self)

    def derived(self) -> "EngineState":
        return EngineState(self.wgrad_stream)


_capture_depth = 0


def capturing() -> bool:
    return _capture_depth > 0


class capture_scope:
    def __enter__(self):
        global _capture_depth
        _capture_depth += 1

    def __exit__(self, *exc):
        global _capture_depth
        _capture_depth -= 1


state = EngineState()
state.param_epoch = 0


def state_of(p) -> EngineState:
    if p is not None:
        st = getattr(p, "_nk_state", None)
        if st is not None:
            return st
        store = getattr(p, "_nk_store", None)
        if store is not None:
            return store.state
    return state


def wgrad_mode(p=None) -> int:
    st = state_of(p)
    if st.grad_accumulate:
        return 1
    return 2 if st.assume_zeroed else 0


_recording = threading.local()


class recording_backward:

    def __enter__(self):
        _recording.depth = getattr(_recording, "depth", 0) + 1

    def __exit__(self, *exc):
        _recording.depth -= 1


def recording() -> bool:
    return getattr(_recording, "depth", 0) > 0


def on_wgrad_stream(fn: Callable[[], None], *reads: Tensor, owner=None) -> None:
    st = state_of(owner)
    side = st.wgrad_stream
    if side is None:
        fn()
        return
    if st.deferred is not None:
        st.deferred.append((fn, reads))
        return
    side.wait_stream(torch.cuda.current_stream())
    with torch.cuda.stream(side):
        fn()
    for t in reads:
        if t is not None:
            t.record_stream(side)


class WgradQueue:

    def __init__(self, owner=None):
        self.items = []
        self.colparts = []
        self.owner = owner

    MAX_ELEMS = 2 << 20

    @classmethod
    def takes(cls, weight: Tensor) -> bool:
        return weight.numel() <= cls.MAX_ELEMS

    def add(self, dy: Tensor, x: Tensor, dw: Tensor, db: Optional[Tensor] = None) -> None:
        self.items.append((dy, x, dw, db))

    def add_colpart(self, part: Tensor, dgamma: Tensor, dbeta: Tensor, nrows: int, Cc: int, accumulate: bool) -> None:
        self.colparts.append((part, dgamma, dbeta, nrows, Cc, accumulate))

    def flush(self) -> None:
        colparts, self.colparts = self.colparts, []
        if colparts:
            on_wgrad_stream(lambda: colpart_reduce(colparts), *[c[0] for c in colparts], owner=self.owner)
        items, self.items = self.items, []
        if not items:
            return
        groups = {}
        for it in items:
            dy, x, dw, _db = it
            key = (dy.shape[0], dy.shape[1], x.shape[1], dy.stride(0), x.stride(0), dw.stride(0))
            groups.setdefault(key, []).append(it)
        mode = wgrad_mode(self.owner)

        def run():
            for (M, N, K, lddy, ldx, lddw), its in groups.items():
                for i in range(0, len(its), 8):
                    chunk = its[i:i + 8]
                    if len(chunk) == 1:
                        gemm_tn_f32(chunk[0][0], chunk[0][1], chunk[0][2], mode, dbias=chunk[0][3])
                        continue
                    n = len(chunk)
                    arr = C.c_void_p * n
                    call("nk_linear_wgrad_batched", arr(*[c[0].data_ptr() for c in chunk]), arr(*[c[1].data_ptr() for c in chunk]),
                         arr(*[c[2].data_ptr() for c in chunk]), arr(*[None if c[3] is None else c[3].data_ptr() for c in chunk]), n, M, N, K,
                         lddy, ldx, lddw, mode, _stream())

        on_wgrad_stream(run, *[t for it in items for t in it[:2]], owner=self.owner)


def colpart_reduce(entries) -> None:
    for i in range(0, len(entries), lib.NK_COLPART_MAX):
        chunk = entries[i:i + lib.NK_COLPART_MAX]
        b = lib.NkColpartBatch()
        for z, (part, dgamma, dbeta, nrows, Cc, acc) in enumerate(chunk):
            b.part[z], b.dgamma[z], b.dbeta[z] = part.data_ptr(), dgamma.data_ptr(), dbeta.data_ptr()
            b.nrows[z], b.C[z], b.accumulate[z] = nrows, Cc, int(acc)
        b.n = len(chunk)
        call("nk_colpart_reduce_batch", C.byref(b), _stream())


_wgrad_queue: Optional[WgradQueue] = None


class batched_wgrads:

    def __init__(self, owner=None):
        self.owner = owner

    def __enter__(self):
        global _wgrad_queue
        self.prev = _wgrad_queue
        _wgrad_queue = WgradQueue(self.owner) if state_of(self.owner).batch_wgrads else None
        return _wgrad_queue

    def __exit__(self, *exc):
        global _wgrad_queue
        q, _wgrad_queue = _wgrad_queue, self.prev
        if exc[0] is None and q is not None:
            q.flush()
        return False


def join_wgrad_stream(owner=None) -> None:
    if owner is not None:
        st = state_of(owner)
        side = st.wgrad_stream
        if side is not None and st.deferred is None:
            torch.cuda.current_stream().wait_stream(side)
        return
    seen = set()
    for st in list(EngineState._live):
        side = st.wgrad_stream
        if side is not None and st.deferred is None and id(side) not in seen:
            seen.add(id(side))
            torch.cuda.current_stream().wait_stream(side)


def _ws(n_floats: int, device) -> Tensor:
    return torch.empty(n_floats, dtype=torch.float32, device=device)


def _p(t: Optional[Tensor]):
    return None if t is None else t.data_ptr()


def _stream():
    return torch.cuda.current_stream().cuda_stream


def _check2d(t: Tensor, name: str):
    if t.dim() != 2 or t.stride(1) != 1 or t.dtype != BF16 or not t.is_cuda:
        raise ValueError(f"{name}: expected a 2-D bf16 CUDA tensor with unit inner stride, got {tuple(t.shape)} {t.dtype} {t.stride()} {t.device}")


@dataclass
class Img:

    t: Tensor
    N: int
    H: int
    W: int
    sums: Optional[Tensor] = None

    @property
    def C(self) -> int:
        return self.t.shape[1]

    @staticmethod
    def from_nchw(x: Tensor) -> "Img":
        N, Cc, H, W = x.shape
        if x.dtype == BF16 and x.permute(0, 2, 3, 1).is_contiguous():
            return Img(x.permute(0, 2, 3, 1).reshape(N * H * W, Cc), N, H, W)
        return Img(nchw_to_tokens(x, Cc), N, H, W)

    def to_nchw(self) -> Tensor:
        return self.t.view(self.N, self.H, self.W, self.C).permute(0, 3, 1, 2)


def _param_stamp(p: Tensor):
    st = getattr(p, "_nk_store", None)
    if st is not None:
        return ("epoch", id(st), st.epoch)
    return ("version", p._version, p.data_ptr())


def shadow(p: Tensor) -> Tensor:
    if getattr(p, "_nk_store", None) is not None:
        return p._nk_shadow
    s = getattr(p, "_nk_shadow", None)
    stamp = _param_stamp(p)
    if s is not None and getattr(p, "_nk_shadow_stamp", None) == stamp:
        return s
    flat = _phys_flat(p)
    n = flat.numel()
    if s is not None and n % 8 == 0 and s.numel() == n and s.device == p.device:
        call("nk_cast_f32_to_bf16", flat.data_ptr(), s.data_ptr(), n, _stream())
        p._nk_shadow_stamp = stamp
        return s
    s = torch.empty(flat.numel(), dtype=BF16, device=p.device)
    if n % 8 == 0:
        call("nk_cast_f32_to_bf16", flat.data_ptr(), s.data_ptr(), n, _stream())
    else:
        pad = torch.zeros((n + 7) // 8 * 8, dtype=torch.float32, device=p.device)
        pad[:n] = flat
        s8 = torch.empty(pad.numel(), dtype=BF16, device=p.device)
        call("nk_cast_f32_to_bf16", pad.data_ptr(), s8.data_ptr(), pad.numel(), _stream())
        s = s8[:n]
    p._nk_shadow = s
    p._nk_shadow_stamp = stamp
    return s


def _phys_flat(p: Tensor) -> Tensor:
    d = p.detach()
    if d.dim() == 4:
        d = d.permute(0, 2, 3, 1)
    if not d.is_contiguous():
        raise ValueError("parameter storage must be dense (conv weights in channels_last memory format)")
    return d.reshape(-1)


def grad_flat(p: Tensor) -> Tensor:
    if p.grad is None:
        g = torch.zeros_like(p, memory_format=torch.preserve_format)
        p.grad = g
    g = p.grad
    if g.dim() == 4:
        g = g.permute(0, 2, 3, 1)
    if not g.is_contiguous():
        raise ValueError("parameter .grad must share the parameter's physical layout")
    return g.reshape(-1)


def w2d(p: Tensor) -> Tensor:
    return shadow(p).view(p.shape[0], -1)


def g2d(p: Tensor) -> Tensor:
    return grad_flat(p).view(p.shape[0], -1)


def conv_weight_param(out_ch: int, in_ch: int, kh: int, kw: int) -> torch.nn.Parameter:
    base = torch.empty(out_ch, kh, kw, in_ch)
    return torch.nn.Parameter(base.permute(0, 3, 1, 2))


def nchw_to_tokens(x: Tensor, cpad: int, scale: float = 1.0) -> Tensor:
    N, Cc, H, W = x.shape
    x = x.contiguous()
    if x.dtype not in (torch.float32, BF16):
        raise ValueError(f"unsupported dtype {x.dtype}")
    out = torch.empty(N * H * W, cpad, dtype=BF16, device=x.device)
    call("nk_nchw_to_nhwc", x.data_ptr(), int(x.dtype == torch.float32), out.data_ptr(), N, Cc, H * W, cpad, scale, _stream())
    return out


def tokens_to_nchw(t: Tensor, N: int, Cc: int, H: int, W: int, dtype=torch.float32) -> Tensor:
    _check2d(t, "t")
    out = torch.empty(N, Cc, H, W, dtype=dtype, device=t.device)
    call("nk_nhwc_to_nchw", t.data_ptr(), out.data_ptr(), int(dtype == torch.float32), N, Cc, H * W, t.shape[1], _stream())
    return out


def cast_bf16(x: Tensor) -> Tensor:
    if x.dtype == BF16:
        return x
    x = x.contiguous()
    out = torch.empty(x.shape, dtype=BF16, device=x.device)
    n = x.numel()
    if n % 8:
        raise ValueError("cast_bf16 needs numel % 8 == 0")
    call("nk_cast_f32_to_bf16", x.data_ptr(), out.data_ptr(), n, _stream())
    return out


def add(a: Tensor, b: Tensor) -> Tensor:
    if a.shape != b.shape or not a.is_contiguous() or not b.is_contiguous():
        raise ValueError("add: contiguous tensors of equal shape expected")
    out = torch.empty_like(a)
    call("nk_add", a.data_ptr(), b.data_ptr(), out.data_ptr(), a.numel(), _stream())
    return out


def gemm_nt(x: Tensor, w: Tensor, bias: Optional[Tensor] = None, residual: Optional[Tensor] = None, alpha: float = 1.0, out: Optional[Tensor] = None) -> Tensor:
    _check2d(x, "x")
    _check2d(w, "w")
    M, K = x.shape
    N = w.shape[0]
    if w.shape[1] != K:
        raise ValueError(f"gemm_nt: K mismatch {x.shape} vs {w.shape}")
    if out is None:
        out = torch.empty(M, N, dtype=BF16, device=x.device)
    if residual is not None:
        _check2d(residual, "residual")
    call("nk_linear_fwd", x.data_ptr(), w.data_ptr(), _p(bias), _p(residual), out.data_ptr(), M, N, K, x.stride(0), w.stride(0),
         residual.stride(0) if residual is not None else 0, out.stride(0), float(alpha), _stream())
    return out


def gemm_nt_batched(xs, ws, outs=None):
    M, K = xs[0].shape
    N = ws[0].shape[0]
    for x, w in zip(xs, ws):
        _check2d(x, "x")
        _check2d(w, "w")
        if x.shape != (M, K) or w.shape != (N, K) or x.stride(0) != xs[0].stride(0) or w.stride(0) != ws[0].stride(0):
            raise ValueError("gemm_nt_batched: every problem must have the same shape and strides")
    if outs is None:
        outs = [torch.empty(M, N, dtype=BF16, device=xs[0].device) for _ in xs]
    for i in range(0, len(xs), 8):
        n = min(8, len(xs) - i)
        arr = C.c_void_p * n
        call("nk_linear_fwd_batched", arr(*[t.data_ptr() for t in xs[i:i + n]]), arr(*[t.data_ptr() for t in ws[i:i + n]]),
             arr(*[t.data_ptr() for t in outs[i:i + n]]), n, M, N, K, xs[0].stride(0), ws[0].stride(0), outs[0].stride(0), _stream())
    return outs


def gemm_nn(dy: Tensor, w: Tensor, dx_add: Optional[Tensor] = None, out: Optional[Tensor] = None) -> Tensor:
    _check2d(dy, "dy")
    _check2d(w, "w")
    M, N = dy.shape
    K = w.shape[1]
    if w.shape[0] != N:
        raise ValueError(f"gemm_nn: N mismatch {dy.shape} vs {w.shape}")
    if out is None:
        out = torch.empty(M, K, dtype=BF16, device=dy.device)
    if dx_add is not None:
        _check2d(dx_add, "dx_add")
    call("nk_linear_dgrad", dy.data_ptr(), w.data_ptr(), _p(dx_add), out.data_ptr(), M, N, K, dy.stride(0), w.stride(0),
         dx_add.stride(0) if dx_add is not None else 0, out.stride(0), _stream())
    return out


def gemm_tn_f32(dy: Tensor, x: Tensor, dw: Tensor, accumulate, dbias: Optional[Tensor] = None) -> None:
    _check2d(dy, "dy")
    _check2d(x, "x")
    M, N = dy.shape
    K = x.shape[1]
    if x.shape[0] != M or dw.shape != (N, K) or dw.dtype != torch.float32 or dw.stride(1) != 1:
        raise ValueError(f"gemm_tn_f32: bad shapes {dy.shape} {x.shape} {dw.shape}")
    if dbias is None:
        call("nk_linear_wgrad", dy.data_ptr(), x.data_ptr(), dw.data_ptr(), M, N, K, dy.stride(0), x.stride(0), dw.stride(0), int(accumulate), _stream())
        return
    if dbias.shape != (N,) or dbias.dtype != torch.float32 or not dbias.is_contiguous():
        raise ValueError(f"gemm_tn_f32: dbias must be a dense fp32 [{N}] tensor")
    call("nk_linear_wgrad_bias", dy.data_ptr(), x.data_ptr(), dw.data_ptr(), dbias.data_ptr(), M, N, K, dy.stride(0), x.stride(0), dw.stride(0),
         int(accumulate), _stream())


def colsum(dy: Tensor, out: Tensor, accumulate: bool) -> None:
    _check2d(dy, "dy")
    M, N = dy.shape
    ws = _ws(query("nk_colsum_ws_floats", M, N), dy.device)
    call("nk_colsum", dy.data_ptr(), out.data_ptr(), ws.data_ptr(), M, N, dy.stride(0), int(accumulate), _stream())


def linear_fwd(x: Tensor, weight: Tensor, bias: Optional[Tensor], residual: Optional[Tensor] = None, need_dx: bool = True, x_saved=None):
    y = gemm_nt(x, w2d(weight), bias, residual)
    return y, _linear_bwd(x if x_saved is None else x_saved, weight, bias, need_dx)


def geglu_save_enabled() -> bool:
    return os.environ.get("NK_GEGLU_SAVE", "1") != "0"


def linear_geglu_fwd(x: Tensor, weight: Tensor, bias: Optional[Tensor], x_saved=None, save_derivative: bool = False):
    _check2d(x, "x")
    M, K = x.shape
    I2 = weight.shape[0]
    I = I2 // 2
    wq = w2d(weight)
    if I2 % 2 == 0 and x.is_contiguous() and query("nk_linear_fwd_geglu_ok", M, I, K):
        u = torch.empty(M, I2, dtype=BF16, device=x.device)
        h = torch.empty(M, I, dtype=BF16, device=x.device)
        call("nk_linear_fwd_geglu_s" if save_derivative else "nk_linear_fwd_geglu", x.data_ptr(), wq.data_ptr(), _p(bias), u.data_ptr(), h.data_ptr(), M, I, K,
             x.stride(0), wq.stride(0), u.stride(0), h.stride(0), _stream())
    else:
        u = gemm_nt(x, wq, bias, None)
        if save_derivative:
            h = torch.empty(M, I, dtype=BF16, device=x.device)
            call("nk_geglu_fwd_s", u.data_ptr(), h.data_ptr(), u.data_ptr(), M, I, _stream())
        else:
            h = geglu_fwd(u)[0]
    return u, h, _linear_bwd(x if x_saved is None else x_saved, weight, bias, True)


def _linear_bwd(x_in, weight: Tensor, bias: Optional[Tensor], need_dx: bool):
    def bwd(dy: Tensor, dx_add: Optional[Tensor] = None, geglu_u: Optional[Tensor] = None, geglu_s: Optional[Tensor] = None):
        entry = "nk_linear_dgrad_geglu"
        if geglu_s is not None:
            if geglu_u is not None:
                raise ValueError("linear bwd: geglu_u and geglu_s are exclusive")
            geglu_u, entry = geglu_s, "nk_linear_dgrad_geglu_s"
        x = x_in() if callable(x_in) else x_in
        queued = _wgrad_queue is not None and _wgrad_queue.takes(weight) and dy.is_contiguous() and x.is_contiguous()
        db = grad_flat(bias) if bias is not None else None
        if queued:
            _wgrad_queue.add(dy, x, g2d(weight), db)
        else:
            on_wgrad_stream(lambda: gemm_tn_f32(dy, x, g2d(weight), wgrad_mode(weight), dbias=db), dy, x, owner=weight)
        if not need_dx:
            return None
        if geglu_u is not None:
            if dx_add is not None:
                raise ValueError("linear bwd: geglu_u and dx_add are exclusive")
            M, N = dy.shape
            K = weight.shape[1]
            _check2d(geglu_u, "geglu_u")
            if geglu_u.shape != (M, 2 * K):
                raise ValueError(f"linear bwd: geglu_u must be [{M}, {2 * K}], got {tuple(geglu_u.shape)}")
            du = torch.empty(M, 2 * K, dtype=BF16, device=dy.device)
            wq = w2d(weight)
            call(entry, dy.data_ptr(), wq.data_ptr(), geglu_u.data_ptr(), du.data_ptr(), M, N, K, dy.stride(0), wq.stride(0),
                 geglu_u.stride(0), du.stride(0), _stream())
            return du
        return gemm_nn(dy, w2d(weight), dx_add)

    return bwd


def _conv_desc(N, H, W, Cin, Cout, KH, KW, stride, pad_t, pad_l, Ho, Wo, upsample) -> NkConvDesc:
    return NkConvDesc(N, H, W, Cin, Cout, KH, KW, stride, pad_t, pad_l, Ho, Wo, int(upsample))


def groupnorm_sums(x: Img, groups: int) -> Tensor:
    if x.sums is not None and x.sums.shape == (x.N, 2 * groups):
        return x.sums
    sums = torch.empty(x.N, 2 * groups, dtype=torch.float32, device=x.t.device)
    ws = _ws(query("nk_groupnorm_ws_floats", x.N, x.H * x.W, x.C, groups), x.t.device)
    call("nk_groupnorm_sums", x.t.data_ptr(), sums.data_ptr(), ws.data_ptr(), x.N, x.H * x.W, x.C, groups, _stream())
    return sums


def conv2d_fwd(x: Img, weight: Tensor, bias: Optional[Tensor], stride: int = 1, padding=1, upsample: bool = False,
               rowvec: Optional[Tensor] = None, residual: Optional[Tensor] = None, need_dx: bool = True,
               asym_pad: bool = False, stats_groups: Optional[int] = None, cin_real: Optional[int] = None):
    Cout, Cin, KH, KW = weight.shape
    if x.C != Cin:
        raise ValueError(f"conv2d: input has {x.C} channels, weight expects {Cin}")
    Hin, Win = (2 * x.H, 2 * x.W) if upsample else (x.H, x.W)
    if asym_pad:
        pad_t = pad_l = 0
        Ho = (Hin + 1 - KH) // stride + 1
        Wo = (Win + 1 - KW) // stride + 1
    else:
        pad_t = pad_l = int(padding)
        Ho = (Hin + 2 * pad_t - KH) // stride + 1
        Wo = (Win + 2 * pad_l - KW) // stride + 1
    d = _conv_desc(x.N, x.H, x.W, Cin, Cout, KH, KW, stride, pad_t, pad_l, Ho, Wo, upsample)
    y = torch.empty(x.N * Ho * Wo, Cout, dtype=BF16, device=x.t.device)
    _check2d(x.t, "x")
    if not x.t.is_contiguous():
        raise ValueError("conv2d: x must be dense channels-last")
    tiles = query("nk_conv2d_stats_tiles", C.byref(d), stats_groups) if stats_groups else 0
    sums_out = None
    if tiles:
        dev = x.t.device
        part = torch.empty(x.N, tiles, 2 * stats_groups, dtype=torch.float32, device=dev)
        call("nk_conv2d_fwd_stats", C.byref(d), x.t.data_ptr(), w2d(weight).data_ptr(), _p(bias), _p(rowvec), _p(residual), y.data_ptr(),
             part.data_ptr(), stats_groups, _stream())
        sums_out = torch.empty(x.N, 2 * stats_groups, dtype=torch.float32, device=dev)
        ws = _ws(query("nk_groupnorm_sums_ws_floats", x.N, tiles, stats_groups), dev)
        call("nk_groupnorm_sums_from_parts", part.data_ptr(), sums_out.data_ptr(), ws.data_ptr(), x.N, tiles, stats_groups, _stream())
    elif (cin_real in (3, 4) and Cin == 8 and KH == 3 and KW == 3 and stride == 1 and pad_t == 1 and not asym_pad and not upsample and rowvec is None
          and residual is None and Cout % 8 == 0):
        call("nk_conv3x3_few_channels_fwd", x.t.data_ptr(), w2d(weight).data_ptr(), _p(bias), y.data_ptr(), x.N, x.H, x.W, Cout, cin_real, _stream())
    else:
        call("nk_conv2d_fwd", C.byref(d), x.t.data_ptr(), w2d(weight).data_ptr(), _p(bias), _p(rowvec), _p(residual), y.data_ptr(), _stream())
    out = Img(y, x.N, Ho, Wo, sums_out)

    def bwd(dy: Tensor):
        _check2d(dy, "dy")
        if not dy.is_contiguous():
            raise ValueError("conv2d bwd: dy must be dense")
        acc = state_of(weight).grad_accumulate

        if weight.requires_grad:
            if bias is not None:
                on_wgrad_stream(lambda: call("nk_conv2d_wgrad_bias", C.byref(d), dy.data_ptr(), x.t.data_ptr(), g2d(weight).data_ptr(), grad_flat(bias).data_ptr(),
                                             wgrad_mode(weight), _stream()), dy, x.t, owner=weight)
            else:
                on_wgrad_stream(lambda: call("nk_conv2d_wgrad", C.byref(d), dy.data_ptr(), x.t.data_ptr(), g2d(weight).data_ptr(), wgrad_mode(weight), _stream()),
                                dy, x.t, owner=weight)
        drow = None
        if rowvec is not None:
            drow32 = torch.empty(x.N, Cout, dtype=torch.float32, device=dy.device)
            ws = _ws(x.N * query("nk_colsum_ws_floats", Ho * Wo, Cout), dy.device)
            call("nk_colsum_batched", dy.data_ptr(), drow32.data_ptr(), ws.data_ptr(), Ho * Wo, Cout, dy.stride(0), x.N, 0, _stream())
            drow = cast_bf16(drow32)
        dx = None
        if need_dx:
            dxt = torch.empty(x.N * Hin * Win, Cin, dtype=BF16, device=dy.device)
            if query("nk_conv2d_dgrad_flipped_ok", C.byref(d)):
                wt = torch.empty(Cin * 9 * Cout, dtype=BF16, device=dy.device)
                call("nk_conv_weight_flip", w2d(weight).data_ptr(), wt.data_ptr(), Cout, Cin, 9, _stream())
                call("nk_conv2d_dgrad_flipped", C.byref(d), dy.data_ptr(), wt.data_ptr(), dxt.data_ptr(), _stream())
            else:
                call("nk_conv2d_dgrad", C.byref(d), dy.data_ptr(), w2d(weight).data_ptr(), dxt.data_ptr(), _stream())
            if upsample:
                dsm = torch.empty(x.N * x.H * x.W, Cin, dtype=BF16, device=dy.device)
                call("nk_upsample2x_bwd", dxt.data_ptr(), dsm.data_ptr(), x.N, x.H, x.W, Cin, _stream())
                dxt = dsm
            dx = Img(dxt, x.N, x.H, x.W)
        return dx, drow

    return out, bwd


def groupnorm_fwd(x: Img, weight: Tensor, bias: Tensor, groups: int, eps: float, silu: bool):
    if not x.t.is_contiguous():
        raise ValueError("groupnorm: x must be dense channels-last")
    N, HW, Cc = x.N, x.H * x.W, x.C
    y = torch.empty_like(x.t)
    mean = torch.empty(N, groups, dtype=torch.float32, device=x.t.device)
    rstd = torch.empty_like(mean)
    nws = query("nk_groupnorm_ws_floats", N, HW, Cc, groups)
    if x.sums is not None and x.sums.shape == (N, 2 * groups):
        call("nk_groupnorm_apply", x.t.data_ptr(), x.sums.data_ptr(), weight.data_ptr(), bias.data_ptr(), y.data_ptr(), mean.data_ptr(),
             rstd.data_ptr(), N, HW, Cc, groups, float(eps), int(silu), _stream())
    else:
        ws = _ws(nws, x.t.device)
        call("nk_groupnorm_fwd", x.t.data_ptr(), weight.data_ptr(), bias.data_ptr(), y.data_ptr(), mean.data_ptr(), rstd.data_ptr(),
             ws.data_ptr(), N, HW, Cc, groups, float(eps), int(silu), _stream())

    def bwd(dy: Tensor, dx_add: Optional[Tensor] = None):
        dx = torch.empty_like(x.t)
        ws2 = _ws(nws, dy.device)
        call("nk_groupnorm_bwd", dy.data_ptr(), x.t.data_ptr(), weight.data_ptr(), bias.data_ptr(), mean.data_ptr(), rstd.data_ptr(),
             _p(dx_add), dx.data_ptr(), grad_flat(weight).data_ptr(), grad_flat(bias).data_ptr(), ws2.data_ptr(), N, HW, Cc, groups,
             int(silu), int(state_of(weight).grad_accumulate), _stream())
        return dx

    return Img(y, x.N, x.H, x.W), bwd


def groupnorm_mod_fwd(x: Img, weight: Tensor, bias: Tensor, mod: Tensor, groups: int, eps: float, silu: bool):
    if not x.t.is_contiguous():
        raise ValueError("groupnorm_mod: x must be dense channels-last")
    N, HW, Cc = x.N, x.H * x.W, x.C
    _check2d(mod, "mod")
    if tuple(mod.shape) != (N, 2 * Cc) or not mod.is_contiguous():
        raise ValueError(f"groupnorm_mod: mod must be a dense [{N}, {2 * Cc}] (scale | shift) matrix, got {tuple(mod.shape)}")
    y = torch.empty_like(x.t)
    mean = torch.empty(N, groups, dtype=torch.float32, device=x.t.device)
    rstd = torch.empty_like(mean)
    nws = query("nk_groupnorm_ws_floats", N, HW, Cc, groups)
    if x.sums is not None and x.sums.shape == (N, 2 * groups):
        call("nk_groupnorm_mod_apply", x.t.data_ptr(), x.sums.data_ptr(), weight.data_ptr(), bias.data_ptr(), mod.data_ptr(), y.data_ptr(),
             mean.data_ptr(), rstd.data_ptr(), N, HW, Cc, groups, float(eps), int(silu), _stream())
    else:
        ws = _ws(nws, x.t.device)
        call("nk_groupnorm_mod_fwd", x.t.data_ptr(), weight.data_ptr(), bias.data_ptr(), mod.data_ptr(), y.data_ptr(), mean.data_ptr(),
             rstd.data_ptr(), ws.data_ptr(), N, HW, Cc, groups, float(eps), int(silu), _stream())

    def bwd(dy: Tensor, dx_add: Optional[Tensor] = None):
        dx = torch.empty_like(x.t)
        dmod = torch.empty_like(mod)
        ws2 = _ws(nws, dy.device)
        call("nk_groupnorm_mod_bwd", dy.data_ptr(), x.t.data_ptr(), weight.data_ptr(), bias.data_ptr(), mod.data_ptr(), mean.data_ptr(),
             rstd.data_ptr(), _p(dx_add), dx.data_ptr(), grad_flat(weight).data_ptr(), grad_flat(bias).data_ptr(), dmod.data_ptr(),
             ws2.data_ptr(), N, HW, Cc, groups, int(silu), int(state_of(weight).grad_accumulate), _stream())
        return dx, dmod

    return Img(y, x.N, x.H, x.W), bwd


def layernorm_fwd(x: Tensor, weight: Tensor, bias: Tensor, eps: float = 1e-5):
    _check2d(x, "x")
    if not x.is_contiguous():
        raise ValueError("layernorm: x must be dense")
    M, Cc = x.shape
    y = torch.empty_like(x)
    mean = torch.empty(M, dtype=torch.float32, device=x.device)
    rstd = torch.empty_like(mean)
    call("nk_layernorm_fwd", x.data_ptr(), weight.data_ptr(), bias.data_ptr(), y.data_ptr(), mean.data_ptr(), rstd.data_ptr(), M, Cc, float(eps), _stream())

    def bwd(dy: Tensor, dx_add: Optional[Tensor] = None):
        dx = torch.empty_like(x)
        acc = state_of(weight).grad_accumulate
        if os.environ.get("NK_LN_FUSED", "1") != "0":
            rows = query("nk_layernorm_part_rows", M)
            part = torch.empty(rows * 2 * Cc, dtype=torch.float32, device=dy.device)
            call("nk_layernorm_bwd_rows", dy.data_ptr(), x.data_ptr(), weight.data_ptr(), mean.data_ptr(), rstd.data_ptr(), _p(dx_add),
                 dx.data_ptr(), part.data_ptr(), M, Cc, _stream())
            entry = (part, grad_flat(weight), grad_flat(bias), rows, Cc, bool(acc))
            if _wgrad_queue is not None:
                _wgrad_queue.add_colpart(*entry)
            else:
                on_wgrad_stream(lambda: colpart_reduce([entry]), part, owner=weight)
            return dx
        ws = _ws(query("nk_layernorm_ws_floats", M, Cc), dy.device)
        call("nk_layernorm_bwd_dx", dy.data_ptr(), x.data_ptr(), weight.data_ptr(), mean.data_ptr(), rstd.data_ptr(), _p(dx_add),
             dx.data_ptr(), M, Cc, _stream())

        def params():
            call("nk_layernorm_bwd_params", dy.data_ptr(), x.data_ptr(), mean.data_ptr(), rstd.data_ptr(),
                 grad_flat(weight).data_ptr(), grad_flat(bias).data_ptr(), ws.data_ptr(), M, Cc, int(acc), _stream())

        st_ = state_of(weight)
        if st_.norm_params_on_side_stream if st_.norm_params_on_side_stream is not None else st_.deferred is not None:
            on_wgrad_stream(params, dy, x, mean, rstd, ws, owner=weight)
        else:
            params()
        return dx

    return y, bwd


def rmsnorm(x: Tensor, weight: Tensor, eps: float = 1e-6) -> Tensor:
    _check2d(x, "x")
    if not x.is_contiguous():
        raise ValueError("rmsnorm: x must be dense")
    M, Cc = x.shape
    if weight.dtype != torch.float32 or weight.numel() != Cc or not weight.is_contiguous():
        raise ValueError(f"rmsnorm: weight must be a dense fp32 vector of {Cc} elements, got {weight.dtype} {tuple(weight.shape)}")
    y = torch.empty_like(x)
    call("nk_rmsnorm_fwd", x.data_ptr(), weight.data_ptr(), y.data_ptr(), M, Cc, float(eps), _stream())
    return y


GATED_ACT_KINDS = ("gated-gelu", "gelu_new", "relu")


def gated_act(u: Tensor, kind: str) -> Tensor:
    _check2d(u, "u")
    if not u.is_contiguous():
        raise ValueError("gated_act: u must be dense")
    if kind == "gated-gelu":
        M, I2 = u.shape
        if I2 % 16:
            raise ValueError(f"gated_act: u must be [M, 2 I] with I % 8 == 0, got {tuple(u.shape)}")
        y = torch.empty(M, I2 // 2, dtype=BF16, device=u.device)
        call("nk_gated_gelu_tanh_fwd", u.data_ptr(), y.data_ptr(), M, I2 // 2, _stream())
        return y
    if kind in ("gelu_new", "relu"):
        y = torch.empty_like(u)
        call("nk_gelu_fwd", u.data_ptr(), y.data_ptr(), u.numel(), 2 if kind == "gelu_new" else 3, _stream())
        return y
    raise ValueError(f"gated_act: kind must be one of {GATED_ACT_KINDS}, got {kind!r}")


def geglu_fwd(u: Tensor):
    _check2d(u, "u")
    M, I2 = u.shape
    inner = I2 // 2
    y = torch.empty(M, inner, dtype=BF16, device=u.device)
    call("nk_geglu_fwd", u.data_ptr(), y.data_ptr(), M, inner, _stream())

    def bwd(dy: Tensor):
        du = torch.empty_like(u)
        call("nk_geglu_bwd", dy.data_ptr(), u.data_ptr(), du.data_ptr(), M, inner, _stream())
        return du

    return y, bwd


def gelu(x: Tensor, quick: bool = False) -> Tensor:
    y = torch.empty_like(x)
    call("nk_gelu_fwd", x.data_ptr(), y.data_ptr(), x.numel(), int(quick), _stream())
    return y


def gelu_fwd(x: Tensor, quick: bool = False):
    if not x.is_contiguous():
        raise ValueError("gelu_fwd: x must be dense")
    y = gelu(x, quick)

    def bwd(dy: Tensor) -> Tensor:
        if dy.shape != x.shape or dy.dtype != BF16 or not dy.is_contiguous():
            raise ValueError("gelu bwd: dy must be a dense bf16 tensor of x's shape")
        dx = torch.empty_like(x)
        call("nk_gelu_bwd", dy.data_ptr(), x.data_ptr(), dx.data_ptr(), x.numel(), int(quick), _stream())
        return dx

    return y, bwd


def embedding_bwd(ids: Tensor, dx: Tensor, table: Tensor, positions: Tensor) -> None:
    _check2d(dx, "dx")
    B, L = ids.shape
    V, Cc = table.shape
    P = positions.shape[0]
    if ids.dtype != torch.int64 or not ids.is_contiguous() or dx.shape != (B * L, Cc) or positions.shape[1] != Cc:
        raise ValueError(f"embedding_bwd: ids [B, L] int64 and dx [B * L, {Cc}] expected, got {tuple(ids.shape)} {ids.dtype}, {tuple(dx.shape)}")
    call("nk_embedding_bwd", ids.data_ptr(), dx.data_ptr(), dx.stride(0), grad_flat(table).data_ptr(), grad_flat(positions).data_ptr(), B, L, V, P,
         Cc, wgrad_mode(table), _stream())


def gather_rows_bwd(dsel: Tensor, idx: Tensor, L: int) -> Tensor:
    _check2d(dsel, "dsel")
    B, Cc = dsel.shape
    if idx.shape != (B,) or idx.dtype != torch.int64 or not idx.is_contiguous():
        raise ValueError("gather_rows_bwd: idx must be a dense int64 [B] tensor")
    dx = torch.empty(B * L, Cc, dtype=BF16, device=dsel.device)
    call("nk_gather_rows_bwd", dsel.data_ptr(), dsel.stride(0), idx.data_ptr(), dx.data_ptr(), B, L, Cc, _stream())
    return dx


def wgrad_few_rows(x: Tensor, dy: Tensor, dw: Tensor, accumulate: bool) -> None:
    _check2d(x, "x")
    _check2d(dy, "dy")
    M, K = x.shape
    N = dy.shape[1]
    if dy.shape[0] != M or dw.shape != (K, N) or dw.dtype != torch.float32 or dw.stride(1) != 1:
        raise ValueError(f"wgrad_few_rows: bad shapes {tuple(x.shape)} {tuple(dy.shape)} {tuple(dw.shape)}")
    call("nk_wgrad_few_rows", x.data_ptr(), x.stride(0), dy.data_ptr(), dy.stride(0), dw.data_ptr(), dw.stride(0), M, K, N, int(accumulate), _stream())


def leaky_relu_fwd(x: Tensor, slope: float = 0.2):
    y = torch.empty_like(x)
    call("nk_leaky_relu_fwd", x.data_ptr(), y.data_ptr(), x.numel(), float(slope), _stream())

    def bwd(dy: Tensor) -> Tensor:
        dx = torch.empty_like(dy)
        call("nk_leaky_relu_bwd", dy.data_ptr(), y.data_ptr(), dx.data_ptr(), dy.numel(), float(slope), _stream())
        return dx

    return y, bwd


def maxpool2x2_fwd(x: Img):
    y = torch.empty(x.N * (x.H // 2) * (x.W // 2), x.C, dtype=BF16, device=x.t.device)
    call("nk_maxpool2x2_fwd", x.t.data_ptr(), y.data_ptr(), x.N, x.H, x.W, x.C, _stream())

    def bwd(dy: Tensor) -> Tensor:
        dx = torch.empty_like(x.t)
        call("nk_maxpool2x2_bwd", dy.data_ptr(), x.t.data_ptr(), dx.data_ptr(), x.N, x.H, x.W, x.C, _stream())
        return dx

    return Img(y, x.N, x.H // 2, x.W // 2), bwd


def avgpool2x_fwd(x: Img):
    if not x.t.is_contiguous():
        raise ValueError("avgpool2x: x must be dense channels-last")
    if x.H < 2 or x.W < 2:
        raise ValueError(f"avgpool2x: a {x.H} x {x.W} image has no 2 x 2 window")
    y = torch.empty(x.N * (x.H // 2) * (x.W // 2), x.C, dtype=BF16, device=x.t.device)
    call("nk_avgpool2x_fwd", x.t.data_ptr(), y.data_ptr(), x.N, x.H, x.W, x.C, _stream())
    N, H, W, Cc = x.N, x.H, x.W, x.C

    def bwd(dy: Tensor) -> Tensor:
        dx = torch.empty(N * H * W, Cc, dtype=BF16, device=dy.device)
        call("nk_avgpool2x_bwd", dy.data_ptr(), dx.data_ptr(), N, H, W, Cc, _stream())
        return dx

    return Img(y, N, H // 2, W // 2), bwd


def upsample2x_fwd(x: Img):
    if not x.t.is_contiguous():
        raise ValueError("upsample2x: x must be dense channels-last")
    N, H, W, Cc = x.N, x.H, x.W, x.C
    y = torch.empty(N * 4 * H * W, Cc, dtype=BF16, device=x.t.device)
    call("nk_upsample2x_fwd", x.t.data_ptr(), y.data_ptr(), N, H, W, Cc, _stream())

    def bwd(dy: Tensor) -> Tensor:
        dx = torch.empty(N * H * W, Cc, dtype=BF16, device=dy.device)
        call("nk_upsample2x_bwd", dy.data_ptr(), dx.data_ptr(), N, H, W, Cc, _stream())
        return dx

    return Img(y, N, 2 * H, 2 * W), bwd


def maxpool_fwd(x: Img, kernel_size: int, stride: int):
    if kernel_size == 2 and stride == 2 and x.H % 2 == 0 and x.W % 2 == 0:
        return maxpool2x2_fwd(x)
    Ho, Wo = (x.H - kernel_size) // stride + 1, (x.W - kernel_size) // stride + 1
    y = torch.empty(x.N * Ho * Wo, x.C, dtype=BF16, device=x.t.device)
    call("nk_maxpool_fwd", x.t.data_ptr(), y.data_ptr(), x.N, x.H, x.W, x.C, kernel_size, stride, _stream())

    def bwd(dy: Tensor) -> Tensor:
        dx = torch.empty_like(x.t)
        call("nk_maxpool_bwd", dy.data_ptr(), x.t.data_ptr(), dx.data_ptr(), x.N, x.H, x.W, x.C, kernel_size, stride, _stream())
        return dx

    return Img(y, x.N, Ho, Wo), bwd


def lpips_layer(f0: Img, f1: Img, w: Tensor, out: Tensor, accumulate: bool, eps: float = 1e-10):
    N, HW, Cc = f0.N, f0.H * f0.W, f0.C
    ws = _ws(query("nk_lpips_layer_ws_floats", N, HW), f0.t.device)
    call("nk_lpips_layer_fwd", f0.t.data_ptr(), f1.t.data_ptr(), w.data_ptr(), out.data_ptr(), ws.data_ptr(), N, HW, Cc, float(eps), int(accumulate), _stream())

    def bwd(upstream: Tensor) -> Tensor:
        d = torch.empty_like(f1.t)
        call("nk_lpips_layer_bwd", f0.t.data_ptr(), f1.t.data_ptr(), w.data_ptr(), upstream.data_ptr(), d.data_ptr(), N, HW, Cc, float(eps), _stream())
        return d

    return bwd


def batchnorm_fwd(x: Tensor, weight: Tensor, bias: Tensor, running_mean: Optional[Tensor], running_var: Optional[Tensor], eps: float = 1e-5,
                  momentum: float = 0.1, slope: float = 1.0):
    _check2d(x, "x")
    if not x.is_contiguous():
        raise ValueError("batchnorm: x must be dense")
    M, Cc = x.shape
    y = torch.empty_like(x)
    mean = torch.empty(Cc, dtype=torch.float32, device=x.device)
    rstd = torch.empty_like(mean)
    nws = query("nk_batchnorm_ws_floats", M, Cc)
    call("nk_batchnorm_fwd", x.data_ptr(), weight.data_ptr(), bias.data_ptr(), y.data_ptr(), mean.data_ptr(), rstd.data_ptr(), _p(running_mean),
         _p(running_var), _ws(nws, x.device).data_ptr(), M, Cc, float(eps), float(momentum), float(slope), _stream())

    def bwd(dy: Tensor) -> Tensor:
        dx = torch.empty_like(x)
        call("nk_batchnorm_bwd", dy.data_ptr(), x.data_ptr(), y.data_ptr(), weight.data_ptr(), mean.data_ptr(), rstd.data_ptr(), dx.data_ptr(),
             grad_flat(weight).data_ptr(), grad_flat(bias).data_ptr(), _ws(nws, x.device).data_ptr(), M, Cc, float(slope), int(state_of(weight).grad_accumulate),
             _stream())
        return dx

    return y, bwd


def batchnorm_eval(x: Tensor, weight: Tensor, bias: Tensor, running_mean: Tensor, running_var: Tensor, eps: float = 1e-5, slope: float = 1.0) -> Tensor:
    _check2d(x, "x")
    if not x.is_contiguous():
        raise ValueError("batchnorm: x must be dense")
    M, Cc = x.shape
    y = torch.empty_like(x)
    call("nk_batchnorm_eval", x.data_ptr(), weight.data_ptr(), bias.data_ptr(), running_mean.data_ptr(), running_var.data_ptr(), y.data_ptr(),
         _ws(Cc + 64, x.device).data_ptr(), M, Cc, float(eps), float(slope), _stream())
    return y


def silu_fwd(x: Tensor):
    y = torch.empty_like(x)
    call("nk_silu_fwd", x.data_ptr(), y.data_ptr(), x.numel(), _stream())

    def bwd(dy: Tensor):
        dx = torch.empty_like(x)
        call("nk_silu_bwd", dy.data_ptr(), x.data_ptr(), dx.data_ptr(), x.numel(), _stream())
        return dx

    return y, bwd


_dropout = threading.local()
_dropout_states: dict = {}


def _as_i64(v: int) -> int:
    v &= (1 << 64) - 1
    return v - (1 << 64) if v >= (1 << 63) else v


def _dropout_state_tensor(device=None) -> Tensor:
    dev = torch.device("cuda", torch.cuda.current_device()) if device is None else torch.device(device)
    if dev.type != "cuda":
        raise ValueError(f"dropout: the counter lives on a GPU, got device {dev}")
    idx = torch.cuda.current_device() if dev.index is None else dev.index
    st = _dropout_states.get(idx)
    if st is None:
        if capturing():
            raise RuntimeError("dropout: the first draw on a device cannot happen inside a hipGraph capture (it allocates the counter)")
        st = _dropout_states[idx] = torch.tensor([_as_i64(torch.initial_seed()), 0], dtype=torch.int64, device=torch.device("cuda", idx))
    return st


def dropout_seed(seed: int, step: int = 0, device=None) -> None:
    st = _dropout_state_tensor(device)
    st.copy_(torch.tensor([_as_i64(int(seed)), _as_i64(int(step))], dtype=torch.int64))


def dropout_state(device=None) -> tuple:
    seed, step = _dropout_state_tensor(device).tolist()
    return seed & ((1 << 64) - 1), step & ((1 << 64) - 1)


def dropout_consts(p: float) -> tuple:
    return int(round(p * 65536)), 1.0 / (1.0 - p)


def check_dropout_rate(p, owner: str) -> float:
    try:
        ok = 0.0 <= float(p) < 1.0
    except (TypeError, ValueError):
        ok = False
    if not ok:
        raise ValueError(f"{owner}: dropout must be a rate in [0, 1), got {p!r}")
    return float(p)


def dropout_draw(device=None) -> Tensor:
    st = _dropout_state_tensor(device)
    tok = torch.empty(2, dtype=torch.int64, device=st.device)
    call("nk_dropout_draw", st.data_ptr(), tok.data_ptr(), _stream())
    _dropout.token = tok
    return tok


def dropout_open(top) -> bool:
    sites = [(i, m) for i, m in enumerate(top.modules()) if m.training and getattr(m, "dropout_p", 0.0) > 0.0]
    if not sites:
        return False
    for i, m in sites:
        m.__dict__["_nk_site"] = i
    p = next(top.parameters(), None)
    dropout_draw(p.device if p is not None and p.is_cuda else None)
    return True


def dropout_site(module) -> int:
    return module.__dict__.get("_nk_site", 0)


def dropout_token(required: bool = True) -> Optional[Tensor]:
    tok = getattr(_dropout, "token", None)
    if tok is None and required:
        raise RuntimeError("dropout: no draw is open on this thread (ops.dropout_draw() / ops.dropout_open(module) at the entry of the forward)")
    return tok


class dropout_token_scope:

    def __init__(self, token: Optional[Tensor]):
        self.token = token

    def __enter__(self):
        self.prev = getattr(_dropout, "token", None)
        _dropout.token = self.token

    def __exit__(self, *exc):
        _dropout.token = self.prev


def dropout_mask_like(x: Tensor, p: float, site: int, token: Tensor, residual: Optional[Tensor] = None, inplace: bool = True) -> Tensor:
    _check2d(x, "x")
    rows, cols = x.shape
    y = x if inplace else torch.empty(rows, cols, dtype=BF16, device=x.device)
    if residual is not None:
        _check2d(residual, "residual")
        if residual.shape != x.shape:
            raise ValueError(f"dropout: residual {tuple(residual.shape)} does not match x {tuple(x.shape)}")
    for name, t in (("x", x), ("residual", residual)):
        if t is not None and (cols % 8 or t.stride(0) % 8 or t.data_ptr() % 16):
            raise ValueError(f"dropout: {name} needs cols % 8 == 0 and 16-byte-aligned rows, got shape {tuple(t.shape)} stride {t.stride()}")
    if token.dtype != torch.int64 or token.numel() != 2 or token.device != x.device:
        raise ValueError("dropout: token must be the int64 [2] tensor of ops.dropout_draw() on x's device")
    if rows == 0:
        return y
    thr, scale = dropout_consts(check_dropout_rate(p, "dropout"))
    call("nk_dropout", x.data_ptr(), _p(residual), y.data_ptr(), rows, cols, x.stride(0), residual.stride(0) if residual is not None else 0, y.stride(0),
         token.data_ptr(), int(site), thr, scale, _stream())
    return y


def dropout_fwd(x: Tensor, p: float, site: int, residual: Optional[Tensor] = None, inplace: bool = False):
    tok = dropout_token()
    y = dropout_mask_like(x, p, site, tok, residual, inplace)

    def bwd(dy: Tensor, inplace: bool = False) -> Tensor:
        return dropout_mask_like(dy, p, site, tok, None, inplace)

    return y, bwd


def cat_fwd(a: Img, b: Img):
    if (a.N, a.H, a.W) != (b.N, b.H, b.W):
        raise ValueError("cat: spatial shapes differ")
    rows = a.t.shape[0]
    out = torch.empty(rows, a.C + b.C, dtype=BF16, device=a.t.device)
    call("nk_cat_channels", a.t.data_ptr(), b.t.data_ptr(), out.data_ptr(), rows, a.C, b.C, _stream())
    Ca, Cb = a.C, b.C

    def bwd(dout: Tensor):
        da = torch.empty(rows, Ca, dtype=BF16, device=dout.device)
        db = torch.empty(rows, Cb, dtype=BF16, device=dout.device)
        call("nk_split_channels", dout.data_ptr(), da.data_ptr(), db.data_ptr(), rows, Ca, Cb, _stream())
        return da, db

    return Img(out, a.N, a.H, a.W), bwd


def attention_fwd(q: Tensor, k: Tensor, v: Tensor, B: int, heads: int, dim_head: int, causal: bool = False, need_lse: bool = True,
                  return_lse: bool = False):
    for n, t in (("q", q), ("k", k), ("v", v)):
        _check2d(t, n)
    Lq, Lk = q.shape[0] // B, k.shape[0] // B
    HD = heads * dim_head
    o = torch.empty(B * Lq, HD, dtype=BF16, device=q.device)
    lse = torch.empty(B, heads, Lq, dtype=torch.float32, device=q.device) if (need_lse or dim_head != 512) else None
    d = NkAttnDesc()
    d.B, d.H, d.Lq, d.Lk, d.D = B, heads, Lq, Lk, dim_head
    d.sq, d.sk, d.sv, d.so = q.stride(0), k.stride(0), v.stride(0), o.stride(0)
    d.bq, d.bk, d.bv, d.bo = Lq * q.stride(0), Lk * k.stride(0), Lk * v.stride(0), Lq * o.stride(0)
    d.scale = float(dim_head) ** -0.5
    d.causal = int(causal)
    call("nk_attention_fwd", C.byref(d), q.data_ptr(), k.data_ptr(), v.data_ptr(), o.data_ptr(), lse.data_ptr() if lse is not None else None,
         _stream())

    def bwd(do: Tensor, dq: Optional[Tensor] = None, dk: Optional[Tensor] = None, dv: Optional[Tensor] = None):
        _check2d(do, "do")
        if dim_head > 160 and dim_head != 512:
            raise NotImplementedError("attention backward: head dim <= 160, or 512 (csrc/attn512_bwd.h)")
        if lse is None:
            raise ValueError("attention backward needs the forward's log-sum-exp: call attention_fwd(..., need_lse=True)")
        dq = torch.empty(B * Lq, HD, dtype=BF16, device=do.device) if dq is None else dq
        dk = torch.empty(B * Lk, HD, dtype=BF16, device=do.device) if dk is None else dk
        dv = torch.empty(B * Lk, HD, dtype=BF16, device=do.device) if dv is None else dv
        d.sdq, d.sdk, d.sdv, d.sdo = dq.stride(0), dk.stride(0), dv.stride(0), do.stride(0)
        d.bdq, d.bdk, d.bdv, d.bdo = Lq * dq.stride(0), Lk * dk.stride(0), Lk * dv.stride(0), Lq * do.stride(0)
        delta = _ws(query("nk_attention_bwd_ws_floats", C.byref(d)), do.device)
        call("nk_attention_bwd", C.byref(d), q.data_ptr(), k.data_ptr(), v.data_ptr(), o.data_ptr(), lse.data_ptr(), do.data_ptr(),
             dq.data_ptr(), dk.data_ptr(), dv.data_ptr(), delta.data_ptr(), _stream())
        return dq, dk, dv

    if return_lse:
        return o, bwd, lse
    return o, bwd


ATTN_RELBIAS_MAX_L = 1024


def attention_relbias_fwd(q: Tensor, k: Tensor, v: Tensor, B: int, heads: int, dim_head: int, rel: Tensor, scale: float = 1.0) -> Tensor:
    for n, t in (("q", q), ("k", k), ("v", v)):
        _check2d(t, n)
    L = q.shape[0] // B
    if k.shape[0] != q.shape[0] or v.shape[0] != q.shape[0]:
        raise ValueError("attention_relbias_fwd: self-attention (q, k and v over the same tokens)")
    if L > ATTN_RELBIAS_MAX_L:
        raise NotImplementedError(f"attention_relbias_fwd: at most {ATTN_RELBIAS_MAX_L} tokens per sequence (the head's bias table lives in LDS), got L = {L}")
    if rel.dtype != torch.float32 or tuple(rel.shape) != (heads, 2 * L - 1) or not rel.is_contiguous() or rel.device != q.device:
        raise ValueError(f"attention_relbias_fwd: rel must be a dense fp32 [{heads}, {2 * L - 1}] tensor on {q.device}, got {rel.dtype} {tuple(rel.shape)}")
    o = torch.empty(B * L, heads * dim_head, dtype=BF16, device=q.device)
    d = NkAttnDesc()
    d.B, d.H, d.Lq, d.Lk, d.D = B, heads, L, L, dim_head
    d.sq, d.sk, d.sv, d.so = q.stride(0), k.stride(0), v.stride(0), o.stride(0)
    d.bq, d.bk, d.bv, d.bo = L * q.stride(0), L * k.stride(0), L * v.stride(0), L * o.stride(0)
    d.scale = float(scale)
    d.causal = 0
    call("nk_attention_relbias_fwd", C.byref(d), q.data_ptr(), k.data_ptr(), v.data_ptr(), o.data_ptr(), rel.data_ptr(), _stream())
    return o


def attention_causal_fwd(q: Tensor, k: Tensor, v: Tensor, B: int, heads: int, dim_head: int = 64):
    L = q.shape[0] // B
    if dim_head != 64 or L > 96 or k.shape[0] != q.shape[0] or v.shape[0] != q.shape[0]:
        raise NotImplementedError(f"attention_causal_fwd: the backward takes head dim 64 and at most 96 tokens (self-attention), got D = {dim_head}, L = {L}")
    o, _, lse = attention_fwd(q, k, v, B, heads, dim_head, causal=True, return_lse=True)
    HD = heads * dim_head

    def bwd(do: Tensor, dq: Optional[Tensor] = None, dk: Optional[Tensor] = None, dv: Optional[Tensor] = None):
        _check2d(do, "do")
        dq = torch.empty(B * L, HD, dtype=BF16, device=do.device) if dq is None else dq
        dk = torch.empty(B * L, HD, dtype=BF16, device=do.device) if dk is None else dk
        dv = torch.empty(B * L, HD, dtype=BF16, device=do.device) if dv is None else dv
        for n, t in (("dq", dq), ("dk", dk), ("dv", dv)):
            _check2d(t, n)
            if t.shape != (B * L, HD):
                raise ValueError(f"attention_causal_fwd bwd: {n} must be [{B * L}, {HD}], got {tuple(t.shape)}")
        d = NkAttnDesc()
        d.B, d.H, d.Lq, d.Lk, d.D = B, heads, L, L, dim_head
        d.sq, d.sk, d.sv, d.so = q.stride(0), k.stride(0), v.stride(0), o.stride(0)
        d.bq, d.bk, d.bv, d.bo = L * q.stride(0), L * k.stride(0), L * v.stride(0), L * o.stride(0)
        d.sdq, d.sdk, d.sdv, d.sdo = dq.stride(0), dk.stride(0), dv.stride(0), do.stride(0)
        d.bdq, d.bdk, d.bdv, d.bdo = L * dq.stride(0), L * dk.stride(0), L * dv.stride(0), L * do.stride(0)
        d.scale = float(dim_head) ** -0.5
        d.causal = 1
        call("nk_attention_bwd_causal", C.byref(d), q.data_ptr(), k.data_ptr(), v.data_ptr(), o.data_ptr(), lse.data_ptr(), do.data_ptr(),
             dq.data_ptr(), dk.data_ptr(), dv.data_ptr(), _stream())
        return dq, dk, dv

    return o, bwd


def attention_unfused(q: Tensor, k: Tensor, v: Tensor, B: int) -> Tensor:
    L = q.shape[0] // B
    D = q.shape[1]
    out = torch.empty_like(q)
    s = torch.empty(L, L, dtype=BF16, device=q.device)
    for b in range(B):
        sl = slice(b * L, (b + 1) * L)
        gemm_nt(q[sl], k[sl], alpha=float(D) ** -0.5, out=s)
        call("nk_softmax_rows", s.data_ptr(), L, L, _stream())
        gemm_nn(s, v[sl], out=out[sl])
    return out


ATTN512_FLASH_MAX_L = 2048
ATTN512_BWD_CHUNK = 2048


def attention512_fwd(q: Tensor, k: Tensor, v: Tensor, B: int):
    L, D = q.shape[0] // B, q.shape[1]
    if D != 512:
        raise ValueError(f"attention512_fwd: head dim 512 only, got {D} (head dims <= 160: attention_fwd)")
    scale = float(D) ** -0.5
    mode = os.environ.get("NK_ATTN512_BWD", "auto")
    if mode == "1" or (mode == "auto" and L <= ATTN512_FLASH_MAX_L):
        out, b_att = attention_fwd(q, k, v, B, 1, D, need_lse=True)
        return out, (lambda do: b_att(do))
    if L % 8:
        raise ValueError(f"attention512_fwd: the chunked recompute backward (L = {L} > {ATTN512_FLASH_MAX_L} tokens per sample, or NK_ATTN512_BWD=0) "
                         f"needs L % 8 == 0; NK_ATTN512_BWD=1 selects the flash backward, which takes any length")
    out, _, lse = attention_fwd(q, k, v, B, 1, D, need_lse=True, return_lse=True)
    return out, _attention_recompute_bwd(q, k, v, B, lse=lse.reshape(B * L))


def attention_anydim_fwd(q: Tensor, k: Tensor, v: Tensor, B: int):
    L, D = q.shape[0] // B, q.shape[1]
    if D % 8 or L % 8:
        raise ValueError(f"attention_anydim_fwd: head dim and tokens per sample must be multiples of 8, got D = {D}, L = {L}")
    return attention_unfused(q, k, v, B), _attention_recompute_bwd(q, k, v, B)


def _attention_recompute_bwd(q: Tensor, k: Tensor, v: Tensor, B: int, lse: Optional[Tensor] = None):
    L, D = q.shape[0] // B, q.shape[1]
    scale = float(D) ** -0.5
    if lse is not None:
        neg = -lse.to(torch.float32) / scale
        p1 = neg.to(BF16)
        r1 = neg - p1.float()
        p2 = r1.to(BF16)
        p3 = (r1 - p2.float()).to(BF16)
        q_aug = torch.cat([q, torch.stack([p1, p2, p3], dim=1), torch.zeros(q.shape[0], 5, dtype=BF16, device=q.device)], dim=1)
        ones = torch.zeros(k.shape[0], 8, dtype=BF16, device=k.device)
        ones[:, :3] = 1.0
        k_aug = torch.cat([k, ones], dim=1)
    else:
        q_aug, k_aug = q, k

    def bwd(do: Tensor):
        _check2d(do, "do")
        dq, dk, dv = torch.empty_like(q), torch.empty_like(k), torch.empty_like(v)
        dk32 = torch.empty(L, D, dtype=torch.float32, device=q.device)
        dv32 = torch.empty(L, D, dtype=torch.float32, device=q.device)
        for b in range(B):
            for c0 in range(0, L, ATTN512_BWD_CHUNK):
                rows = slice(b * L + c0, b * L + min(c0 + ATTN512_BWD_CHUNK, L))
                keys = slice(b * L, (b + 1) * L)
                n = rows.stop - rows.start
                p = gemm_nt(q_aug[rows], k_aug[keys], alpha=scale)
                call("nk_softmax_rows", p.data_ptr(), n, L, _stream())
                dp = gemm_nt(do[rows], v[keys])
                gemm_tn_f32(p, do[rows], dv32, c0 > 0)
                call("nk_softmax_rows_bwd", p.data_ptr(), dp.data_ptr(), n, L, scale, _stream())
                gemm_nn(dp, k[keys], out=dq[rows])
                gemm_tn_f32(dp, q[rows], dk32, c0 > 0)
            dv[b * L:(b + 1) * L].copy_(cast_bf16(dv32))
            dk[b * L:(b + 1) * L].copy_(cast_bf16(dk32))
        return dq, dk, dv

    return bwd


VQ_MAX_D, VQ_MAX_CODES = 256, 65536


def _vq_rows(t: Tensor, name: str, op: str) -> Tensor:
    if not t.is_cuda:
        raise NotImplementedError(f"{op}: {name} is a CPU tensor; the HIP kernels run on the GPU only, there is no CPU path")
    if t.dim() != 2 or t.dtype != torch.float32:
        raise ValueError(f"{op}: {name} must be a 2-D fp32 tensor, got {tuple(t.shape)} {t.dtype}")
    return t if t.stride(1) == 1 and t.stride(0) >= t.shape[1] else t.contiguous()


def _vq_idx(idx: Tensor, N: int, op: str) -> Tensor:
    if not idx.is_cuda:
        raise NotImplementedError(f"{op}: idx is a CPU tensor; the HIP kernels run on the GPU only, there is no CPU path")
    if idx.dtype != torch.int64 or idx.numel() != N:
        raise ValueError(f"{op}: idx must hold {N} int64 indices, got {tuple(idx.shape)} {idx.dtype}")
    return idx.reshape(-1).contiguous()


def vq_search(z: Tensor, codebook: Tensor) -> Tensor:
    z, codebook = _vq_rows(z, "z", "vq_search"), _vq_rows(codebook, "codebook", "vq_search").contiguous()
    N, D = z.shape
    n_e = codebook.shape[0]
    if codebook.shape[1] != D:
        raise ValueError(f"vq_search: z [N, {D}] against a codebook of width {codebook.shape[1]}")
    idx = torch.empty(N, dtype=torch.int64, device=z.device)
    ws = _ws(max(query("nk_vq_search_ws_floats", N, n_e), 1), z.device)
    call("nk_vq_search", z.data_ptr(), z.stride(0), codebook.data_ptr(), ws.data_ptr(), idx.data_ptr(), N, D, n_e, _stream())
    return idx


def vq_code_stats(idx: Tensor, z: Tensor, n_e: int):
    z = _vq_rows(z, "z", "vq_code_stats")
    N, D = z.shape
    idx = _vq_idx(idx, N, "vq_code_stats")
    count = torch.zeros(n_e, dtype=torch.int64, device=z.device)
    total = torch.zeros(n_e, D, dtype=torch.float32, device=z.device)
    call("nk_vq_code_stats", idx.data_ptr(), z.data_ptr(), z.stride(0), count.data_ptr(), total.data_ptr(), N, D, int(n_e), _stream())
    return count, total


def vq_quantize(idx: Tensor, codebook: Tensor, z: Tensor, hw: int = 1, out: Optional[Tensor] = None):
    z, codebook = _vq_rows(z, "z", "vq_quantize"), _vq_rows(codebook, "codebook", "vq_quantize").contiguous()
    N, D = z.shape
    idx = _vq_idx(idx, N, "vq_quantize")
    if codebook.shape[1] != D or hw < 1 or N % hw:
        raise ValueError(f"vq_quantize: z {tuple(z.shape)}, codebook {tuple(codebook.shape)}, hw = {hw}")
    if out is None:
        out = torch.empty((N, D) if hw == 1 else (N // hw, D, hw), dtype=torch.float32, device=z.device)
    elif out.numel() != N * D or out.dtype != torch.float32 or not out.is_contiguous() or not out.is_cuda:
        raise ValueError("vq_quantize: out must be a dense fp32 device tensor of N * D elements")
    sumsq = torch.empty((), dtype=torch.float32, device=z.device)
    ws = _ws(query("nk_vq_quantize_ws_floats", N), z.device)
    call("nk_vq_quantize", idx.data_ptr(), codebook.data_ptr(), z.data_ptr(), z.stride(0), out.data_ptr(), sumsq.data_ptr(), ws.data_ptr(), N, D,
         codebook.shape[0], int(hw), _stream())
    return out, sumsq


def timestep_embedding(t: Tensor, dim: int, max_period: float = 10000.0) -> Tensor:
    tf = t.to(torch.float32).contiguous()
    out = torch.empty(tf.shape[0], dim, dtype=BF16, device=t.device)
    call("nk_timestep_embedding", tf.data_ptr(), out.data_ptr(), tf.shape[0], dim, float(max_period), _stream())
    return out
```

Before: 26.41.

## Fuse groupnorm partial-sum reduction into apply kernels and cat, defer colpart reduce

Groupnorm apply and backward-apply kernels can now finish the per-tile partial sums themselves in shared memory, so the separate sums-from-parts and reduce-partials launches are dropped. Conv and channel-cat producers emit per-tile stats parts instead of reduced sums. A batched column-partial reduce lets dgamma/dbeta reductions be deferred onto the weight-grad stream. This removes several small launches and intermediate buffers, at the cost of every apply block redundantly re-reducing the partials.

```diff
diff --git a/include/neurosis_hip.h b/include/neurosis_hip.h
--- a/include/neurosis_hip.h
+++ b/include/neurosis_hip.h
@@ -104,6 +104,18 @@
 int nk_groupnorm_mod_bwd(const void* dy, const void* x, const float* gamma, const float* beta, const void* mod, const float* mean,
                          const float* rstd, const void* dx_add, void* dx, float* dgamma, float* dbeta, void* dmod, float* ws,
                          int N, int HW, int C, int G, int silu, int accumulate, void* stream);
+struct NkColpartBatch;
+long nk_groupnorm_parts_max(void);
+long nk_groupnorm_bwd_parts_max(void);
+long nk_groupnorm_chan_rows(int N, int HW);
+int nk_groupnorm_apply_parts(const void* x, const float* part, int nparts, const float* gamma, const float* beta, const void* mod, void* y,
+                             float* mean, float* rstd, int N, int HW, int C, int G, float eps, int silu, void* stream);
+int nk_groupnorm_bwd_parts(const void* dy, const void* x, const float* gamma, const float* beta, const void* mod, const float* mean,
+                           const float* rstd, const void* dx_add, void* dx, float* dgamma, float* dbeta, void* dmod, float* ws, float* chan,
+                           int N, int HW, int C, int G, int silu, int accumulate, void* stream);
+int nk_groupnorm_colpart_reduce_batch(const struct NkColpartBatch* b, void* stream);
+long nk_groupnorm_stats_parts(int N, int HW, int C);
+int nk_cat_channels_stats(const void* a, const void* b, void* out, float* part, int N, int HW, int Ca, int Cb, int G, void* stream);
 
 int nk_layernorm_fwd(const void* x, const float* gamma, const float* beta, void* y, float* mean, float* rstd,
                      int M, int C, float eps, void* stream);
diff --git a/neurosis_amd/csrc/norm.hip b/neurosis_amd/csrc/norm.hip
--- a/neurosis_amd/csrc/norm.hip
+++ b/neurosis_amd/csrc/norm.hip
@@ -76,6 +76,36 @@
   }
 }
 
+#ifndef GN_PARTS_MAX
+#define GN_PARTS_MAX 128
+#endif
+#ifndef GN_BWD_PARTS_MAX
+#define GN_BWD_PARTS_MAX 256
+#endif
+__device__ __forceinline__ void gn_finish_sums(const float* __restrict__ part, int nparts, int G2, float (*sm)[128], float* out) {
+  for (int it = threadIdx.x; it < 8 * G2; it += GN_THREADS) {
+    const int tx = it % G2, ty = it / G2;
+    float a = 0.f;
+    for (int p0 = ty; p0 < nparts; p0 += 64) {
+      float v[8];
+#pragma unroll
+      for (int u = 0; u < 8; ++u) v[u] = p0 + 8 * u < nparts ? part[(long)(p0 + 8 * u) * G2 + tx] : 0.f;
+#pragma unroll
+      for (int u = 0; u < 8; ++u)
+        if (p0 + 8 * u < nparts) a += v[u];
+    }
+    sm[ty][tx] = a;
+  }
+  __syncthreads();
+  if ((int)threadIdx.x < G2) {
+    float a = sm[0][threadIdx.x];
+#pragma unroll
+    for (int j = 1; j < 8; ++j) a += sm[j][threadIdx.x];
+    out[threadIdx.x] = a;
+  }
+  __syncthreads();
+}
+
 __device__ __forceinline__ void gn_modulate(const bf16_t* __restrict__ mod, int n, int c, int C, float& ga, float& be) {
   const float s1 = 1.0f + bf2f(mod[(long)n * 2 * C + c]);
   const float t = bf2f(mod[(long)n * 2 * C + C + c]);
@@ -83,13 +113,13 @@
   be = be * s1 + t;
 }
 
-template <bool MOD>
+template <bool MOD, bool PARTS = false>
 __global__ __launch_bounds__(GN_THREADS) void gn_apply_kernel(const bf16_t* __restrict__ x, const float* __restrict__ stats,
                                                               const float* __restrict__ gamma, const float* __restrict__ beta,
                                                               const bf16_t* __restrict__ mod,
                                                               bf16_t* __restrict__ y, float* __restrict__ mean_out,
                                                               float* __restrict__ rstd_out, int HW, int C, int G,
-                                                              float eps, int silu, int rows_per) {
+                                                              float eps, int silu, int rows_per, int nparts) {
   extern __shared__ __attribute__((aligned(16))) char smem_raw[];
   float* sc = (float*)smem_raw;
   float* sh = sc + C;
@@ -97,10 +127,16 @@
   const int tid = threadIdx.x;
   const int cpg = C / G;
   const float inv_cnt = 1.0f / ((float)HW * (float)cpg);
+  const float* st = stats + (long)n * 2 * G;
+  if constexpr (PARTS) {
+    __shared__ float psm[8][128], psum[128];
+    gn_finish_sums(stats + (long)n * nparts * 2 * G, nparts, 2 * G, psm, psum);
+    st = psum;
+  }
   for (int c = tid; c < C; c += GN_THREADS) {
     int g = c / cpg;
-    float m = stats[(long)n * 2 * G + 2 * g] * inv_cnt;
-    float var = fmaxf(stats[(long)n * 2 * G + 2 * g + 1] * inv_cnt - m * m, 0.f);
+    float m = st[2 * g] * inv_cnt;
+    float var = fmaxf(st[2 * g + 1] * inv_cnt - m * m, 0.f);
     float rs = rsqrtf(var + eps);
     float ga = gamma[c], be = beta[c];
     if constexpr (MOD) gn_modulate(mod, n, c, C, ga, be);
@@ -304,14 +340,14 @@
   }
 }
 
-template <bool MOD>
+template <bool MOD, bool PARTS = false>
 __global__ __launch_bounds__(GN_THREADS) void gn_bwd_apply_kernel(const bf16_t* __restrict__ dy, const bf16_t* __restrict__ x,
                                                                   const float* __restrict__ gamma, const float* __restrict__ beta,
                                                                   const bf16_t* __restrict__ mod,
                                                                   const float* __restrict__ mean, const float* __restrict__ rstd,
                                                                   const float* __restrict__ gsum, const bf16_t* __restrict__ dx_add,
                                                                   bf16_t* __restrict__ dx, int HW, int C, int G, int silu,
-                                                                  int rows_per) {
+                                                                  int rows_per, int nparts) {
   extern __shared__ __attribute__((aligned(16))) char smem_raw[];
   float* p_a = (float*)smem_raw;
   float* p_b = p_a + C;
@@ -321,10 +357,16 @@
   const int tid = threadIdx.x;
   const int cpg = C / G;
   const float inv_cnt = 1.0f / ((float)HW * (float)cpg);
+  const float* gs = gsum + (long)n * 2 * G;
+  if constexpr (PARTS) {
+    __shared__ float psm[8][128], psum[128];
+    gn_finish_sums(gsum + (long)n * nparts * 2 * G, nparts, 2 * G, psm, psum);
+    gs = psum;
+  }
   for (int c = tid; c < C; c += GN_THREADS) {
     const int g = c / cpg;
     const float mu = mean[n * G + g], rs = rstd[n * G + g];
-    const float s1 = gsum[(long)n * 2 * G + 2 * g] * inv_cnt, s2 = gsum[(long)n * 2 * G + 2 * g + 1] * inv_cnt;
+    const float s1 = gs[2 * g] * inv_cnt, s2 = gs[2 * g + 1] * inv_cnt;
     float ga = gamma[c], be = beta[c];
     if constexpr (MOD) gn_modulate(mod, n, c, C, ga, be);
     const float a = rs * ga;
@@ -417,7 +459,7 @@
   hipLaunchKernelGGL(gn_reduce_partials_kernel, dim3(N), dim3(1024), 0, stream, part, stats, nsplit * nz, 2 * G);
   if (int e = nk_check_launch("gn_reduce_partials_kernel")) return e;
   hipLaunchKernelGGL(gn_apply_kernel<false>, dim3(nsplit, N), dim3(GN_THREADS), 2 * C * sizeof(float), stream,
-                     (const bf16_t*)x, stats, gamma, beta, (const bf16_t*)nullptr, (bf16_t*)y, mean, rstd, HW, C, G, eps, silu, rows_per);
+                     (const bf16_t*)x, stats, gamma, beta, (const bf16_t*)nullptr, (bf16_t*)y, mean, rstd, HW, C, G, eps, silu, rows_per, 0);
   return nk_check_launch("gn_apply_kernel");
 }
 
@@ -475,7 +517,7 @@
   int nsplit;
   int rows_per = gn_rows_per(N, HW, &nsplit);
   hipLaunchKernelGGL(gn_apply_kernel<false>, dim3(nsplit, N), dim3(GN_THREADS), 2 * C * sizeof(float), stream, (const bf16_t*)x, sums, gamma, beta,
-                     (const bf16_t*)nullptr, (bf16_t*)y, mean, rstd, HW, C, G, eps, silu, rows_per);
+                     (const bf16_t*)nullptr, (bf16_t*)y, mean, rstd, HW, C, G, eps, silu, rows_per, 0);
   return nk_check_launch("gn_apply_kernel");
 }
 
@@ -501,7 +543,7 @@
   if (int e = nk_check_launch("colpart_reduce_kernel")) return e;
   hipLaunchKernelGGL(gn_bwd_apply_kernel<false>, dim3(nsplit, N), dim3(GN_THREADS), 4 * C * sizeof(float), stream,
                      (const bf16_t*)dy, (const bf16_t*)x, gamma, beta, (const bf16_t*)nullptr, mean, rstd, gsum, (const bf16_t*)dx_add,
-                     (bf16_t*)dx, HW, C, G, silu, rows_per);
+                     (bf16_t*)dx, HW, C, G, silu, rows_per, 0);
   return nk_check_launch("gn_bwd_apply_kernel");
 }
 
@@ -510,7 +552,7 @@
   int nsplit;
   int rows_per = gn_rows_per(N, HW, &nsplit);
   hipLaunchKernelGGL(gn_apply_kernel<true>, dim3(nsplit, N), dim3(GN_THREADS), 2 * C * sizeof(float), stream, (const bf16_t*)x, sums, gamma, beta,
-                     (const bf16_t*)mod, (bf16_t*)y, mean, rstd, HW, C, G, eps, silu, rows_per);
+                     (const bf16_t*)mod, (bf16_t*)y, mean, rstd, HW, C, G, eps, silu, rows_per, 0);
   return nk_check_launch("gn_apply_kernel<mod>");
 }
 
@@ -560,8 +602,207 @@
   if (int e = nk_check_launch("gn_dmod_kernel")) return e;
   hipLaunchKernelGGL(gn_bwd_apply_kernel<true>, dim3(nsplit, N), dim3(GN_THREADS), 4 * C * sizeof(float), stream,
                      (const bf16_t*)dy, (const bf16_t*)x, gamma, beta, (const bf16_t*)mod, mean, rstd, gsum, (const bf16_t*)dx_add,
-                     (bf16_t*)dx, HW, C, G, silu, rows_per);
+                     (bf16_t*)dx, HW, C, G, silu, rows_per, 0);
   return nk_check_launch("gn_bwd_apply_kernel<mod>");
+}
+
+extern "C" long nk_groupnorm_parts_max(void) { return GN_PARTS_MAX; }
+extern "C" long nk_groupnorm_bwd_parts_max(void) { return GN_BWD_PARTS_MAX; }
+
+extern "C" long nk_groupnorm_chan_rows(int N, int HW) {
+  int nsplit;
+  gn_rows_per(N, HW, &nsplit);
+  return (long)N * nsplit;
+}
+
+extern "C" int nk_groupnorm_apply_parts(const void* x, const float* part, int nparts, const float* gamma, const float* beta, const void* mod,
+                                        void* y, float* mean, float* rstd, int N, int HW, int C, int G, float eps, int silu, void* stream_) {
+  hipStream_t stream = (hipStream_t)stream_;
+  NK_CHECK_ARG(N > 0 && HW > 0 && C > 0 && G > 0 && G <= 64);
+  NK_CHECK_ARG((C & 7) == 0 && C % G == 0 && C <= GN_MAXC);
+  NK_CHECK_ARG(x && part && gamma && beta && y && mean && rstd);
+  NK_CHECK_ARG(nparts > 0 && nparts <= GN_BWD_PARTS_MAX);
+  int nsplit;
+  int rows_per = gn_rows_per(N, HW, &nsplit);
+  if (mod) {
+    hipLaunchKernelGGL(HIP_KERNEL_NAME(gn_apply_kernel<true, true>), dim3(nsplit, N), dim3(GN_THREADS), 2 * C * sizeof(float), stream,
+                       (const bf16_t*)x, part, gamma, beta, (const bf16_t*)mod, (bf16_t*)y, mean, rstd, HW, C, G, eps, silu, rows_per, nparts);
+    return nk_check_launch("gn_apply_kernel<mod,parts>");
+  }
+  hipLaunchKernelGGL(HIP_KERNEL_NAME(gn_apply_kernel<false, true>), dim3(nsplit, N), dim3(GN_THREADS), 2 * C * sizeof(float), stream,
+                     (const bf16_t*)x, part, gamma, beta, (const bf16_t*)nullptr, (bf16_t*)y, mean, rstd, HW, C, G, eps, silu, rows_per, nparts);
+  return nk_check_launch("gn_apply_kernel<parts>");
+}
+
+template <bool MOD>
+static int gn_bwd_parts_launch(const void* dy, const void* x, const float* gamma, const float* beta, const void* mod, const float* mean,
+                               const float* rstd, const void* dx_add, void* dx, float* dgamma, float* dbeta, void* dmod, float* ws, float* chan,
+                               int N, int HW, int C, int G, int silu, int accumulate, hipStream_t stream) {
+  int nsplit;
+  int rows_per = gn_rows_per(N, HW, &nsplit);
+  const int nz = gn_nz(C), nparts = nsplit * nz;
+  float* part = ws;
+  float* gsum = part + (long)N * nparts * 2 * G;
+  hipLaunchKernelGGL(gn_bwd_stats_kernel<MOD>, dim3(nsplit, N, nz), dim3(GN_THREADS), 2 * C * sizeof(float), stream, (const bf16_t*)dy,
+                     (const bf16_t*)x, gamma, beta, (const bf16_t*)mod, mean, rstd, part, chan, HW, C, G, silu, rows_per);
+  if (int e = nk_check_launch(MOD ? "gn_bwd_stats_kernel<mod>" : "gn_bwd_stats_kernel")) return e;
+  if constexpr (MOD) {
+    hipLaunchKernelGGL(colpart_reduce_mod_kernel, dim3((C + 63) / 64), dim3(1024), 0, stream, chan, (const bf16_t*)mod, dgamma, dbeta, N * nsplit,
+                       nsplit, C, accumulate);
+    if (int e = nk_check_launch("colpart_reduce_mod_kernel")) return e;
+    hipLaunchKernelGGL(gn_dmod_kernel, dim3((C + 63) / 64, N), dim3(1024), 0, stream, chan, gamma, beta, (bf16_t*)dmod, nsplit, C);
+    if (int e = nk_check_launch("gn_dmod_kernel")) return e;
+  } else if (dgamma) {
+    hipLaunchKernelGGL(colpart_reduce_kernel, dim3((C + 63) / 64), dim3(1024), 0, stream, chan, dgamma, dbeta, N * nsplit, C, accumulate);
+    if (int e = nk_check_launch("colpart_reduce_kernel")) return e;
+  }
+  if (nparts <= GN_BWD_PARTS_MAX) {
+    hipLaunchKernelGGL(HIP_KERNEL_NAME(gn_bwd_apply_kernel<MOD, true>), dim3(nsplit, N), dim3(GN_THREADS), 4 * C * sizeof(float), stream,
+                       (const bf16_t*)dy, (const bf16_t*)x, gamma, beta, (const bf16_t*)mod, mean, rstd, part, (const bf16_t*)dx_add, (bf16_t*)dx,
+                       HW, C, G, silu, rows_per, nparts);
+    return nk_check_launch(MOD ? "gn_bwd_apply_kernel<mod,parts>" : "gn_bwd_apply_kernel<parts>");
+  }
+  hipLaunchKernelGGL(gn_reduce_partials_kernel, dim3(N), dim3(1024), 0, stream, part, gsum, nparts, 2 * G);
+  if (int e = nk_check_launch("gn_reduce_partials_kernel")) return e;
+  hipLaunchKernelGGL(HIP_KERNEL_NAME(gn_bwd_apply_kernel<MOD, false>), dim3(nsplit, N), dim3(GN_THREADS), 4 * C * sizeof(float), stream,
+                     (const bf16_t*)dy, (const bf16_t*)x, gamma, beta, (const bf16_t*)mod, mean, rstd, gsum, (const bf16_t*)dx_add, (bf16_t*)dx,
+                     HW, C, G, silu, rows_per, 0);
+  return nk_check_launch(MOD ? "gn_bwd_apply_kernel<mod>" : "gn_bwd_apply_kernel");
+}
+
+extern "C" int nk_groupnorm_bwd_parts(const void* dy, const void* x, const float* gamma, const float* beta, const void* mod, const float* mean,
+                                      const float* rstd, const void* dx_add, void* dx, float* dgamma, float* dbeta, void* dmod, float* ws,
+                                      float* chan, int N, int HW, int C, int G, int silu, int accumulate, void* stream_) {
+  hipStream_t stream = (hipStream_t)stream_;
+  NK_CHECK_ARG(N > 0 && HW > 0 && C > 0 && G > 0 && G <= 64);
+  NK_CHECK_ARG((C & 7) == 0 && C % G == 0 && C <= GN_MAXC);
+  NK_CHECK_ARG(dy && x && gamma && beta && mean && rstd && dx && ws && chan);
+  NK_CHECK_ARG((mod != nullptr) == (dmod != nullptr) && (dgamma != nullptr) == (dbeta != nullptr));
+  NK_CHECK_ARG(dgamma || !mod);
+  if (mod)
+    return gn_bwd_parts_launch<true>(dy, x, gamma, beta, mod, mean, rstd, dx_add, dx, dgamma, dbeta, dmod, ws, chan, N, HW, C, G, silu, accumulate, stream);
+  return gn_bwd_parts_launch<false>(dy, x, gamma, beta, mod, mean, rstd, dx_add, dx, dgamma, dbeta, dmod, ws, chan, N, HW, C, G, silu, accumulate, stream);
+}
+
+__global__ __launch_bounds__(512) void gn_colpart_reduce_batch_kernel(const NkColpartBatch b) {
+  __shared__ float sa[16][33], sb[16][33];
+  const int z = blockIdx.y;
+  const int C = b.C[z], nrows = b.nrows[z];
+  if ((int)blockIdx.x * 32 >= C) return;
+  const float* __restrict__ part = b.part[z];
+  const int tx = threadIdx.x & 31, ty = threadIdx.x >> 5;
+  const int c = blockIdx.x * 32 + tx;
+  float a = 0.f, v = 0.f;
+  if (c < C) {
+#pragma unroll 4
+    for (int r = ty; r < nrows; r += 16) {
+      a += part[(long)r * 2 * C + c];
+      v += part[(long)r * 2 * C + C + c];
+    }
+  }
+  sa[ty][tx] = a;
+  sb[ty][tx] = v;
+  __syncthreads();
+  if (ty == 0 && c < C) {
+#pragma unroll
+    for (int j = 1; j < 16; ++j) { a += sa[j][tx]; v += sb[j][tx]; }
+    float* dgamma = b.dgamma[z];
+    float* dbeta = b.dbeta[z];
+    dgamma[c] = b.accumulate[z] ? dgamma[c] + a : a;
+    dbeta[c] = b.accumulate[z] ? dbeta[c] + v : v;
+  }
+}
+
+extern "C" int nk_groupnorm_colpart_reduce_batch(const NkColpartBatch* b, void* stream_) {
+  NK_CHECK_ARG(b && b->n > 0 && b->n <= NK_COLPART_MAX);
+  int maxC = 0;
+  for (int z = 0; z < b->n; ++z) {
+    NK_CHECK_ARG(b->part[z] && b->dgamma[z] && b->dbeta[z] && b->nrows[z] > 0 && b->C[z] > 0);
+    maxC = b->C[z] > maxC ? b->C[z] : maxC;
+  }
+  hipLaunchKernelGGL(gn_colpart_reduce_batch_kernel, dim3((maxC + 31) / 32, b->n), dim3(512), 0, (hipStream_t)stream_, *b);
+  return nk_check_launch("gn_colpart_reduce_batch_kernel");
+}
+
+__global__ __launch_bounds__(GN_THREADS) void gn_cat_stats_kernel(const bf16_t* __restrict__ a, const bf16_t* __restrict__ b,
+                                                                  bf16_t* __restrict__ o, float* __restrict__ stats, int HW, int Ca, int Cb,
+                                                                  int G, int rows_per) {
+  __shared__ float ps[GN_THREADS * 8], pss[GN_THREADS * 8];
+  const int C = Ca + Cb;
+  const int n = blockIdx.y;
+  const int cpr = (C >> 3) / gridDim.z;
+  const int ch0 = blockIdx.z * cpr;
+  const int rows_par = GN_THREADS / cpr;
+  const int tid = threadIdx.x;
+  const int cpg = C / G;
+  const int row_lo = blockIdx.x * rows_per;
+  const int row_hi = min(HW, row_lo + rows_per);
+  float s[8], ss[8];
+#pragma unroll
+  for (int e = 0; e < 8; ++e) { s[e] = 0.f; ss[e] = 0.f; }
+  const int chunk = tid % cpr, rsub = tid / cpr;
+  if (rsub < rows_par) {
+    const int cg = ch0 + chunk, ca8 = Ca >> 3;
+    const bool from_a = cg < ca8;
+    const int Cs = from_a ? Ca : Cb;
+    const bf16_t* base = from_a ? a + ((long)n * HW) * Ca + cg * 8 : b + ((long)n * HW) * Cb + (cg - ca8) * 8;
+    bf16_t* obase = o + ((long)n * HW) * C + cg * 8;
+    int r = row_lo + rsub;
+    for (; r + 3 * rows_par < row_hi; r += 4 * rows_par) {
+      uint4_t v[4];
+#pragma unroll
+      for (int u = 0; u < 4; ++u) v[u] = *(const uint4_t*)(base + (long)(r + u * rows_par) * Cs);
+#pragma unroll
+      for (int u = 0; u < 4; ++u) {
+        *(uint4_t*)(obase + (long)(r + u * rows_par) * C) = v[u];
+        float f[8];
+        unpack8(v[u], f);
+#pragma unroll
+        for (int e = 0; e < 8; ++e) { s[e] += f[e]; ss[e] += f[e] * f[e]; }
+      }
+    }
+    for (; r < row_hi; r += rows_par) {
+      const uint4_t v = *(const uint4_t*)(base + (long)r * Cs);
+      *(uint4_t*)(obase + (long)r * C) = v;
+      float f[8];
+      unpack8(v, f);
+#pragma unroll
+      for (int e = 0; e < 8; ++e) { s[e] += f[e]; ss[e] += f[e] * f[e]; }
+    }
+#pragma unroll
+    for (int e = 0; e < 8; ++e) {
+      ps[(rsub * cpr + chunk) * 8 + e] = s[e];
+      pss[(rsub * cpr + chunk) * 8 + e] = ss[e];
+    }
+  }
+  __syncthreads();
+  float* part = stats + (((long)n * gridDim.x + blockIdx.x) * gridDim.z + blockIdx.z) * 2 * G;
+  for (int i = tid; i < 2 * G; i += GN_THREADS) {
+    const int g = i >> 1;
+    const float* src = (i & 1) ? pss : ps;
+    const int c_lo = max(g * cpg, ch0 * 8), c_hi = min((g + 1) * cpg, (ch0 + cpr) * 8);
+    float acc = 0.f;
+    for (int c = c_lo; c < c_hi; ++c)
+      for (int r = 0; r < rows_par; ++r) acc += src[r * cpr * 8 + (c - ch0 * 8)];
+    part[i] = acc;
+  }
+}
+
+extern "C" long nk_groupnorm_stats_parts(int N, int HW, int C) {
+  int nsplit;
+  gn_rows_per(N, HW, &nsplit);
+  return (long)nsplit * gn_nz(C);
+}
+
+extern "C" int nk_cat_channels_stats(const void* a, const void* b, void* out, float* part, int N, int HW, int Ca, int Cb, int G, void* stream) {
+  const int C = Ca + Cb;
+  NK_CHECK_ARG(a && b && out && part && N > 0 && HW > 0 && Ca > 0 && Cb > 0 && (Ca & 7) == 0 && (Cb & 7) == 0);
+  NK_CHECK_ARG(G > 0 && G <= 64 && C % G == 0 && C <= GN_MAXC);
+  int nsplit;
+  int rows_per = gn_rows_per(N, HW, &nsplit);
+  hipLaunchKernelGGL(gn_cat_stats_kernel, dim3(nsplit, N, gn_nz(C)), dim3(GN_THREADS), 0, (hipStream_t)stream, (const bf16_t*)a,
+                     (const bf16_t*)b, (bf16_t*)out, part, HW, Ca, Cb, G, rows_per);
+  return nk_check_launch("gn_cat_stats_kernel");
 }
 
 #define LN_MAXCH 4
diff --git a/neurosis_amd/lib.py b/neurosis_amd/lib.py
--- a/neurosis_amd/lib.py
+++ b/neurosis_amd/lib.py
@@ -67,6 +67,10 @@
     "nk_groupnorm_mod_fwd": [vp, vp, vp, vp, vp, vp, vp, vp, i32, i32, i32, i32, f32, i32, vp],
     "nk_groupnorm_mod_apply": [vp, vp, vp, vp, vp, vp, vp, vp, i32, i32, i32, i32, f32, i32, vp],
     "nk_groupnorm_mod_bwd": [vp, vp, vp, vp, vp, vp, vp, vp, vp, vp, vp, vp, vp, i32, i32, i32, i32, i32, i32, vp],
+    "nk_groupnorm_apply_parts": [vp, vp, i32, vp, vp, vp, vp, vp, vp, i32, i32, i32, i32, f32, i32, vp],
+    "nk_groupnorm_bwd_parts": [vp, vp, vp, vp, vp, vp, vp, vp, vp, vp, vp, vp, vp, vp, i32, i32, i32, i32, i32, i32, vp],
+    "nk_groupnorm_colpart_reduce_batch": [C.POINTER(NkColpartBatch), vp],
+    "nk_cat_channels_stats": [vp, vp, vp, vp, i32, i32, i32, i32, i32, vp],
     "nk_layernorm_fwd": [vp, vp, vp, vp, vp, vp, i32, i32, f32, vp],
     "nk_rmsnorm_fwd": [vp, vp, vp, i32, i32, f32, vp],
     "nk_layernorm_bwd": [vp, vp, vp, vp, vp, vp, vp, vp, vp, vp, i32, i32, i32, vp],
@@ -140,6 +144,10 @@
 SIZE_QUERIES: dict[str, list] = {
     "nk_groupnorm_ws_floats": [i32, i32, i32, i32],
     "nk_groupnorm_sums_ws_floats": [i32, i32, i32],
+    "nk_groupnorm_parts_max": [],
+    "nk_groupnorm_bwd_parts_max": [],
+    "nk_groupnorm_chan_rows": [i32, i32],
+    "nk_groupnorm_stats_parts": [i32, i32, i32],
     "nk_conv2d_stats_tiles": [cdp, i32],
     "nk_conv2d_dgrad_flipped_ok": [cdp],
     "nk_linear_fwd_geglu_ok": [i32, i32, i32],
diff --git a/neurosis_amd/modules/diffusion/openaimodel.py b/neurosis_amd/modules/diffusion/openaimodel.py
--- a/neurosis_amd/modules/diffusion/openaimodel.py
+++ b/neurosis_amd/modules/diffusion/openaimodel.py
@@ -506,7 +506,7 @@
         h, b_mid = self.middle_block.fwd(h, emb, context, sink_)
         out_tape = []
         for module in self.output_blocks:
-            h, b_cat = ops.cat_fwd(h, hs.pop())
+            h, b_cat = ops.cat_fwd(h, hs.pop(), stats_groups=32)
             h, b = module.fwd(h, emb, context, sink_)
             out_tape.append((module, b, b_cat))
         gn = self.out[0]
diff --git a/neurosis_amd/ops.py b/neurosis_amd/ops.py
--- a/neurosis_amd/ops.py
+++ b/neurosis_amd/ops.py
@@ -4,7 +4,6 @@
 import os
 import threading
 import weakref
-from dataclasses import dataclass
 from typing import Callable, Optional
 
 import torch
@@ -111,6 +110,7 @@
     def __init__(self, owner=None):
         self.items = []
         self.colparts = []
+        self.gn_colparts = []
         self.owner = owner
 
     MAX_ELEMS = 2 << 20
@@ -124,11 +124,17 @@
 
     def add_colpart(self, part: Tensor, dgamma: Tensor, dbeta: Tensor, nrows: int, Cc: int, accumulate: bool) -> None:
         self.colparts.append((part, dgamma, dbeta, nrows, Cc, accumulate))
+
+    def add_gn_colpart(self, chan: Tensor, dgamma: Tensor, dbeta: Tensor, nrows: int, Cc: int, accumulate: bool) -> None:
+        self.gn_colparts.append((chan, dgamma, dbeta, nrows, Cc, accumulate))
 
     def flush(self) -> None:
         colparts, self.colparts = self.colparts, []
         if colparts:
             on_wgrad_stream(lambda: colpart_reduce(colparts), *[c[0] for c in colparts], owner=self.owner)
+        gn_colparts, self.gn_colparts = self.gn_colparts, []
+        if gn_colparts:
+            on_wgrad_stream(lambda: gn_colpart_reduce(gn_colparts), *[c[0] for c in gn_colparts], owner=self.owner)
         items, self.items = self.items, []
         if not items:
             return
@@ -155,7 +161,16 @@
         on_wgrad_stream(run, *[t for it in items for t in it[:2]], owner=self.owner)
 
 
-def colpart_reduce(entries) -> None:
+def norm_params_deferred(p) -> bool:
+    st = state_of(p)
+    return st.norm_params_on_side_stream if st.norm_params_on_side_stream is not None else st.deferred is not None
+
+
+def gn_colpart_reduce(entries) -> None:
+    colpart_reduce(entries, entry_point="nk_groupnorm_colpart_reduce_batch")
+
+
+def colpart_reduce(entries, entry_point: str = "nk_colpart_reduce_batch") -> None:
     for i in range(0, len(entries), lib.NK_COLPART_MAX):
         chunk = entries[i:i + lib.NK_COLPART_MAX]
         b = lib.NkColpartBatch()
@@ -163,7 +178,7 @@
             b.part[z], b.dgamma[z], b.dbeta[z] = part.data_ptr(), dgamma.data_ptr(), dbeta.data_ptr()
             b.nrows[z], b.C[z], b.accumulate[z] = nrows, Cc, int(acc)
         b.n = len(chunk)
-        call("nk_colpart_reduce_batch", C.byref(b), _stream())
+        call(entry_point, C.byref(b), _stream())
 
 
 _wgrad_queue: Optional[WgradQueue] = None
@@ -220,14 +235,37 @@
         raise ValueError(f"{name}: expected a 2-D bf16 CUDA tensor with unit inner stride, got {tuple(t.shape)} {t.dtype} {t.stride()} {t.device}")
 
 
-@dataclass
 class Img:
 
-    t: Tensor
-    N: int
-    H: int
-    W: int
-    sums: Optional[Tensor] = None
+    def __init__(self, t: Tensor, N: int, H: int, W: int, sums: Optional[Tensor] = None, parts: Optional[Tensor] = None, stats_rows: bool = False):
+        self.t, self.N, self.H, self.W = t, N, H, W
+        self._sums, self.parts, self.stats_rows = sums, parts, stats_rows
+
+    def __repr__(self) -> str:
+        return f"Img(t={tuple(self.t.shape)}, N={self.N}, H={self.H}, W={self.W}, sums={self._sums is not None}, parts={self.parts is not None})"
+
+    @property
+    def sums(self) -> Optional[Tensor]:
+        if self._sums is None and self.parts is not None:
+            N, tiles, G2 = self.parts.shape
+            if self.stats_rows and tiles > query("nk_groupnorm_parts_max"):
+                self._sums = groupnorm_sums(Img(self.t, self.N, self.H, self.W), G2 // 2)
+                return self._sums
+            self._sums = torch.empty(N, G2, dtype=torch.float32, device=self.parts.device)
+            ws = _ws(query("nk_groupnorm_sums_ws_floats", N, tiles, G2 // 2), self.parts.device)
+            call("nk_groupnorm_sums_from_parts", self.parts.data_ptr(), self._sums.data_ptr(), ws.data_ptr(), N, tiles, G2 // 2, _stream())
+        return self._sums
+
+    @sums.setter
+    def sums(self, value: Optional[Tensor]) -> None:
+        self._sums = value
+
+    def parts_for(self, groups: int) -> Optional[Tensor]:
+        p = self.parts
+        if p is not None and self._sums is None and p.shape[0] == self.N and p.shape[2] == 2 * groups:
+            if p.shape[1] <= query("nk_groupnorm_bwd_parts_max" if self.stats_rows else "nk_groupnorm_parts_max"):
+                return p
+        return None
 
     @property
     def C(self) -> int:
@@ -520,21 +558,17 @@
     if not x.t.is_contiguous():
         raise ValueError("conv2d: x must be dense channels-last")
     tiles = query("nk_conv2d_stats_tiles", C.byref(d), stats_groups) if stats_groups else 0
-    sums_out = None
+    part = None
     if tiles:
-        dev = x.t.device
-        part = torch.empty(x.N, tiles, 2 * stats_groups, dtype=torch.float32, device=dev)
+        part = torch.empty(x.N, tiles, 2 * stats_groups, dtype=torch.float32, device=x.t.device)
         call("nk_conv2d_fwd_stats", C.byref(d), x.t.data_ptr(), w2d(weight).data_ptr(), _p(bias), _p(rowvec), _p(residual), y.data_ptr(),
              part.data_ptr(), stats_groups, _stream())
-        sums_out = torch.empty(x.N, 2 * stats_groups, dtype=torch.float32, device=dev)
-        ws = _ws(query("nk_groupnorm_sums_ws_floats", x.N, tiles, stats_groups), dev)
-        call("nk_groupnorm_sums_from_parts", part.data_ptr(), sums_out.data_ptr(), ws.data_ptr(), x.N, tiles, stats_groups, _stream())
     elif (cin_real in (3, 4) and Cin == 8 and KH == 3 and KW == 3 and stride == 1 and pad_t == 1 and not asym_pad and not upsample and rowvec is None
           and residual is None and Cout % 8 == 0):
         call("nk_conv3x3_few_channels_fwd", x.t.data_ptr(), w2d(weight).data_ptr(), _p(bias), y.data_ptr(), x.N, x.H, x.W, Cout, cin_real, _stream())
     else:
         call("nk_conv2d_fwd", C.byref(d), x.t.data_ptr(), w2d(weight).data_ptr(), _p(bias), _p(rowvec), _p(residual), y.data_ptr(), _stream())
-    out = Img(y, x.N, Ho, Wo, sums_out)
+    out = Img(y, x.N, Ho, Wo, parts=part)
 
     def bwd(dy: Tensor):
         _check2d(dy, "dy")
@@ -582,7 +616,11 @@
     mean = torch.empty(N, groups, dtype=torch.float32, device=x.t.device)
     rstd = torch.empty_like(mean)
     nws = query("nk_groupnorm_ws_floats", N, HW, Cc, groups)
-    if x.sums is not None and x.sums.shape == (N, 2 * groups):
+    parts = x.parts_for(groups)
+    if parts is not None:
+        call("nk_groupnorm_apply_parts", x.t.data_ptr(), parts.data_ptr(), parts.shape[1], weight.data_ptr(), bias.data_ptr(), None, y.data_ptr(),
+             mean.data_ptr(), rstd.data_ptr(), N, HW, Cc, groups, float(eps), int(silu), _stream())
+    elif x.sums is not None and x.sums.shape == (N, 2 * groups):
         call("nk_groupnorm_apply", x.t.data_ptr(), x.sums.data_ptr(), weight.data_ptr(), bias.data_ptr(), y.data_ptr(), mean.data_ptr(),
              rstd.data_ptr(), N, HW, Cc, groups, float(eps), int(silu), _stream())
     else:
@@ -593,9 +631,19 @@
     def bwd(dy: Tensor, dx_add: Optional[Tensor] = None):
         dx = torch.empty_like(x.t)
         ws2 = _ws(nws, dy.device)
-        call("nk_groupnorm_bwd", dy.data_ptr(), x.t.data_ptr(), weight.data_ptr(), bias.data_ptr(), mean.data_ptr(), rstd.data_ptr(),
-             _p(dx_add), dx.data_ptr(), grad_flat(weight).data_ptr(), grad_flat(bias).data_ptr(), ws2.data_ptr(), N, HW, Cc, groups,
-             int(silu), int(state_of(weight).grad_accumulate), _stream())
+        rows = query("nk_groupnorm_chan_rows", N, HW)
+        chan = torch.empty(rows * 2 * Cc, dtype=torch.float32, device=dy.device)
+        acc = bool(state_of(weight).grad_accumulate)
+        defer = norm_params_deferred(weight)
+        call("nk_groupnorm_bwd_parts", dy.data_ptr(), x.t.data_ptr(), weight.data_ptr(), bias.data_ptr(), None, mean.data_ptr(), rstd.data_ptr(),
+             _p(dx_add), dx.data_ptr(), None if defer else grad_flat(weight).data_ptr(), None if defer else grad_flat(bias).data_ptr(), None,
+             ws2.data_ptr(), chan.data_ptr(), N, HW, Cc, groups, int(silu), int(acc), _stream())
+        if defer:
+            entry = (chan, grad_flat(weight), grad_flat(bias), rows, Cc, acc)
+            if _wgrad_queue is not None:
+                _wgrad_queue.add_gn_colpart(*entry)
+            else:
+                on_wgrad_stream(lambda: gn_colpart_reduce([entry]), chan, owner=weight)
         return dx
 
     return Img(y, x.N, x.H, x.W), bwd
@@ -612,7 +660,11 @@
     mean = torch.empty(N, groups, dtype=torch.float32, device=x.t.device)
     rstd = torch.empty_like(mean)
     nws = query("nk_groupnorm_ws_floats", N, HW, Cc, groups)
-    if x.sums is not None and x.sums.shape == (N, 2 * groups):
+    parts = x.parts_for(groups)
+    if parts is not None:
+        call("nk_groupnorm_apply_parts", x.t.data_ptr(), parts.data_ptr(), parts.shape[1], weight.data_ptr(), bias.data_ptr(), mod.data_ptr(),
+             y.data_ptr(), mean.data_ptr(), rstd.data_ptr(), N, HW, Cc, groups, float(eps), int(silu), _stream())
+    elif x.sums is not None and x.sums.shape == (N, 2 * groups):
         call("nk_groupnorm_mod_apply", x.t.data_ptr(), x.sums.data_ptr(), weight.data_ptr(), bias.data_ptr(), mod.data_ptr(), y.data_ptr(),
              mean.data_ptr(), rstd.data_ptr(), N, HW, Cc, groups, float(eps), int(silu), _stream())
     else:
@@ -624,9 +676,10 @@
         dx = torch.empty_like(x.t)
         dmod = torch.empty_like(mod)
         ws2 = _ws(nws, dy.device)
-        call("nk_groupnorm_mod_bwd", dy.data_ptr(), x.t.data_ptr(), weight.data_ptr(), bias.data_ptr(), mod.data_ptr(), mean.data_ptr(),
+        chan = _ws(query("nk_groupnorm_chan_rows", N, HW) * 2 * Cc, dy.device)
+        call("nk_groupnorm_bwd_parts", dy.data_ptr(), x.t.data_ptr(), weight.data_ptr(), bias.data_ptr(), mod.data_ptr(), mean.data_ptr(),
              rstd.data_ptr(), _p(dx_add), dx.data_ptr(), grad_flat(weight).data_ptr(), grad_flat(bias).data_ptr(), dmod.data_ptr(),
-             ws2.data_ptr(), N, HW, Cc, groups, int(silu), int(state_of(weight).grad_accumulate), _stream())
+             ws2.data_ptr(), chan.data_ptr(), N, HW, Cc, groups, int(silu), int(state_of(weight).grad_accumulate), _stream())
         return dx, dmod
 
     return Img(y, x.N, x.H, x.W), bwd
@@ -1024,13 +1077,20 @@
     return y, bwd
 
 
-def cat_fwd(a: Img, b: Img):
+def cat_fwd(a: Img, b: Img, stats_groups: Optional[int] = None):
     if (a.N, a.H, a.W) != (b.N, b.H, b.W):
         raise ValueError("cat: spatial shapes differ")
     rows = a.t.shape[0]
-    out = torch.empty(rows, a.C + b.C, dtype=BF16, device=a.t.device)
-    call("nk_cat_channels", a.t.data_ptr(), b.t.data_ptr(), out.data_ptr(), rows, a.C, b.C, _stream())
     Ca, Cb = a.C, b.C
+    out = torch.empty(rows, Ca + Cb, dtype=BF16, device=a.t.device)
+    part = None
+    HW = a.H * a.W
+    nparts = query("nk_groupnorm_stats_parts", a.N, HW, Ca + Cb) if stats_groups and (Ca + Cb) % stats_groups == 0 else 0
+    if 0 < nparts <= query("nk_groupnorm_bwd_parts_max") and a.t.is_contiguous() and b.t.is_contiguous():
+        part = torch.empty(a.N, nparts, 2 * stats_groups, dtype=torch.float32, device=a.t.device)
+        call("nk_cat_channels_stats", a.t.data_ptr(), b.t.data_ptr(), out.data_ptr(), part.data_ptr(), a.N, HW, Ca, Cb, stats_groups, _stream())
+    else:
+        call("nk_cat_channels", a.t.data_ptr(), b.t.data_ptr(), out.data_ptr(), rows, Ca, Cb, _stream())
 
     def bwd(dout: Tensor):
         da = torch.empty(rows, Ca, dtype=BF16, device=dout.device)
@@ -1038,7 +1098,7 @@
         call("nk_split_channels", dout.data_ptr(), da.data_ptr(), db.data_ptr(), rows, Ca, Cb, _stream())
         return da, db
 
-    return Img(out, a.N, a.H, a.W), bwd
+    return Img(out, a.N, a.H, a.W, parts=part, stats_rows=True), bwd
 
 
 def attention_fwd(q: Tensor, k: Tensor, v: Tensor, B: int, heads: int, dim_head: int, causal: bool = False, need_lse: bool = True,
```

After: 26.53, median of 6. No clear change (+0.5%).
